# simonhmartin/genomics_general

Measured on NVIDIA H100. Metric: sites/sec popgenWindows (pi+Fst+Dxy), higher is better.
Workload: dtype u8

## Files before the change

genomics_general_b200/_lib.py:

```python
from __future__ import annotations

import ctypes as C
import os
import subprocess

import numpy as np

_HERE = os.path.dirname(os.path.abspath(__file__))
LIB_PATH = os.path.join(_HERE, "libpgwin.so")
CSRC = os.path.join(_HERE, "csrc")

_lib = None


class PgError(RuntimeError):
    pass


def build(force: bool = False, verbose: bool = False) -> str:
    srcs = [os.path.join(CSRC, f) for f in os.listdir(CSRC) if f.endswith((".cu", ".h", ".cpp"))]
    srcs.append(os.path.join(_HERE, "..", "include", "pgwin.h"))
    if not force and os.path.exists(LIB_PATH):
        newest = max(os.path.getmtime(s) for s in srcs)
        if os.path.getmtime(LIB_PATH) >= newest:
            return LIB_PATH
    cmd = ["make", "-C", CSRC, "-j4"]
    r = subprocess.run(cmd, stdout=subprocess.PIPE, stderr=subprocess.STDOUT, text=True)
    if verbose or r.returncode != 0:
        print(r.stdout)
    if r.returncode != 0:
        raise PgError("building libpgwin.so failed (nvcc for sm_90a)")
    return LIB_PATH


_SIGS = {
    "pg_version": (C.c_int, []),
    "pg_last_error": (C.c_char_p, []),
    "pg_device_count": (C.c_int, [C.POINTER(C.c_int)]),
    "pg_ctx_create": (C.c_int, [C.c_int, C.POINTER(C.c_void_p)]),
    "pg_ctx_destroy": (C.c_int, [C.c_void_p]),
    "pg_host_alloc": (C.c_int, [C.POINTER(C.c_void_p), C.c_size_t]),
    "pg_host_free": (C.c_int, [C.c_void_p]),
    "pg_upload": (C.c_int, [C.c_void_p, C.c_void_p, C.c_int64, C.c_int32, C.c_void_p]),
    "pg_alloc_sites": (C.c_int, [C.c_void_p, C.c_int64, C.c_int32]),
    "pg_upload_range": (C.c_int, [C.c_void_p, C.c_int64, C.c_int64, C.c_void_p, C.c_void_p]),
    "pg_append_sites": (C.c_int, [C.c_void_p, C.c_int64, C.c_void_p, C.c_void_p]),
    "pg_synth_fill": (C.c_int, [C.c_void_p, C.c_int64, C.c_int32, C.c_int32, C.c_int32, C.c_uint64, C.c_uint64,
                                C.c_uint64, C.c_uint64, C.c_uint64, C.c_int32]),
    "pg_download": (C.c_int, [C.c_void_p, C.c_int64, C.c_int64, C.c_void_p, C.c_void_p]),
    "pg_set_pops": (C.c_int, [C.c_void_p, C.c_int32, C.c_void_p]),
    "pg_set_windows": (C.c_int, [C.c_void_p, C.c_int64, C.c_void_p, C.c_void_p]),
    "pg_popgen": (C.c_int, [C.c_void_p, C.c_int32, C.c_double, C.c_int32, C.c_void_p, C.c_void_p, C.c_void_p,
                            C.c_void_p, C.c_void_p, C.c_void_p]),
    "pg_popgen_device": (C.c_int, [C.c_void_p, C.c_int32, C.c_double, C.c_int32, C.c_void_p, C.POINTER(C.c_int64)]),
    "pg_popgen_freqstats": (C.c_int, [C.c_void_p] * 6),
    "pg_set_freqstats": (C.c_int, [C.c_void_p, C.c_int32]),
    "pg_abbababa": (C.c_int, [C.c_void_p, C.c_int32, C.c_int32, C.c_int32, C.c_int32, C.c_double, C.c_void_p,
                              C.c_void_p, C.c_void_p, C.c_void_p]),
    "pg_fourpop": (C.c_int, [C.c_void_p, C.c_int32, C.c_int32, C.c_int32, C.c_int32, C.c_double, C.c_int32, C.c_void_p,
                             C.c_void_p, C.c_void_p, C.c_void_p]),
    "pg_site_counts": (C.c_int, [C.c_void_p, C.c_int64, C.c_int64, C.c_void_p]),
    "pg_site_target_freqs": (C.c_int, [C.c_void_p, C.c_int64, C.c_int64, C.c_int32, C.c_double, C.c_int32, C.c_void_p,
                                       C.c_void_p]),
    "pg_sfs": (C.c_int, [C.c_void_p, C.c_int32, C.c_int32, C.c_int32, C.c_void_p, C.c_void_p, C.c_void_p, C.c_void_p,
                         C.c_void_p, C.POINTER(C.c_int64)]),
    "pg_sfs_tables": (C.c_int, [C.c_void_p, C.c_int32, C.c_void_p, C.c_int64, C.c_int32, C.c_void_p, C.c_int32, C.c_int32,
                                C.c_int32, C.c_void_p, C.c_void_p, C.c_void_p, C.c_void_p, C.c_void_p, C.POINTER(C.c_int64)]),
    "pg_sfs_sparse": (C.c_int, [C.c_void_p, C.c_int32, C.c_int32, C.c_int32, C.c_void_p, C.c_void_p, C.c_void_p, C.c_void_p,
                                C.POINTER(C.c_int64)]),
    "pg_sfs_tables_sparse": (C.c_int, [C.c_void_p, C.c_int32, C.c_void_p, C.c_int64, C.c_int32, C.c_void_p, C.c_int32,
                                       C.c_int32, C.c_int32, C.c_void_p, C.c_void_p, C.c_void_p, C.c_void_p,
                                       C.POINTER(C.c_int64)]),
    "pg_sfs_sparse_fetch": (C.c_int, [C.c_void_p, C.c_int64, C.c_void_p, C.c_void_p, C.c_void_p]),
    "pg_pairdist": (C.c_int, [C.c_void_p, C.c_int32, C.c_void_p, C.c_int32, C.c_int32, C.c_void_p, C.c_void_p,
                              C.c_void_p]),
    "pg_distpaint": (C.c_int, [C.c_void_p, C.c_int32, C.c_void_p, C.c_int32, C.c_void_p, C.c_void_p, C.c_int32, C.c_int32,
                               C.c_double, C.c_int32, C.c_void_p, C.c_void_p, C.c_void_p]),
    "pg_pairdist_cat": (C.c_int, [C.c_void_p, C.c_int32, C.c_void_p, C.c_int32, C.c_void_p, C.POINTER(C.c_int64)]),
    "pg_seq_nonnan": (C.c_int, [C.c_void_p, C.c_void_p]),
    "pg_ind_het": (C.c_int, [C.c_void_p, C.c_int32, C.c_void_p, C.c_int32, C.c_void_p]),
    "pg_hapstats": (C.c_int, [C.c_void_p, C.c_double, C.c_int32, C.c_int32, C.c_void_p]),
    "pg_pair_counts": (C.c_int, [C.c_void_p, C.c_int64, C.c_void_p, C.c_void_p]),
    "pg_last_timings": (C.c_int, [C.c_void_p, C.c_int32, C.c_void_p, C.c_void_p, C.c_void_p, C.POINTER(C.c_int32)]),
    "pg_launch_count": (C.c_int, [C.c_void_p, C.POINTER(C.c_int64)]),
    "pg_debug_k1_plan": (C.c_int, [C.c_int64, C.c_int32] + [C.POINTER(C.c_int32)] * 5),
    "pg_debug_k1_plan_ex": (C.c_int, [C.c_int64, C.c_int32, C.c_int32, C.c_int32, C.c_int32, C.POINTER(C.c_int32)]),
    "pg_debug_packed": (C.c_int, [C.c_void_p, C.c_int64, C.c_int64, C.POINTER(C.c_int32), C.c_void_p]),
    "pg_debug_site_cls": (C.c_int, [C.c_void_p, C.c_int64, C.c_int64, C.POINTER(C.c_int32), C.c_void_p]),
    "pg_debug_uniform": (C.c_int, [C.c_void_p, C.POINTER(C.c_int32), C.POINTER(C.c_int64)]),
    "pg_debug_uniform_tile": (C.c_int, [C.c_void_p, C.POINTER(C.c_int32)]),
    "pg_debug_uniform_rows": (C.c_int, [C.c_void_p, C.POINTER(C.c_int64), C.POINTER(C.c_int64)]),
    "pg_debug_uniform_ring": (C.c_int, [C.c_void_p, C.POINTER(C.c_int32)]),
    "pg_debug_uniform_launch": (C.c_int, [C.c_void_p, C.POINTER(C.c_int32)]),
    "pg_debug_uniform_tiles": (C.c_int, [C.c_void_p, C.c_int64, C.c_void_p, C.c_void_p, C.POINTER(C.c_int64),
                                         C.POINTER(C.c_int32)]),
    "pg_nccl_unique_id": (C.c_int, [C.c_void_p]),
    "pg_nccl_init": (C.c_int, [C.c_void_p, C.c_int32, C.c_int32, C.c_void_p]),
    "pg_nccl_finalize": (C.c_int, [C.c_void_p]),
    "pg_popgen_gather_begin": (C.c_int, [C.c_void_p, C.c_int32, C.c_double, C.c_int64, C.c_int32]),
    "pg_popgen_gather_end": (C.c_int, [C.c_void_p, C.c_int32, C.POINTER(C.c_void_p), C.POINTER(C.c_int64)]),
    "pg_popgen_allgather": (C.c_int, [C.c_void_p, C.c_int32, C.c_double, C.c_int32, C.c_int64, C.c_void_p,
                                      C.POINTER(C.c_int64)]),
    "pg_ingest_file": (C.c_int, [C.c_void_p, C.c_char_p, C.c_int64, C.c_int32, C.c_int32, C.c_void_p, C.c_void_p, C.c_int32,
                                 C.POINTER(C.c_int64)]),
    "pg_ingest_file_range": (C.c_int, [C.c_void_p, C.c_char_p, C.c_int64, C.c_int64, C.c_int32, C.c_int32, C.c_void_p, C.c_void_p,
                                       C.c_int32, C.POINTER(C.c_int64)]),
    "pg_ingest_text": (C.c_int, [C.c_void_p, C.c_void_p, C.c_size_t, C.c_int32, C.c_int32, C.c_void_p, C.c_void_p, C.c_int32,
                                 C.POINTER(C.c_int64)]),
    "pg_ingest_meta": (C.c_int, [C.c_void_p, C.c_void_p, C.c_void_p, C.c_void_p]),
    "pg_ingest_release": (C.c_int, [C.c_void_p]),
    "pg_ingest_set_strict": (C.c_int, [C.c_void_p, C.c_int32]),
    "pg_debug_ingest": (C.c_int, [C.c_void_p, C.c_void_p]),
    "pg_filter": (C.c_int, [C.c_void_p, C.c_void_p, C.c_void_p, C.c_void_p, C.POINTER(C.c_int64), C.POINTER(C.c_uint8)]),
    "pg_filter_emit": (C.c_int, [C.c_void_p, C.c_int32, C.c_int32, C.c_int64, C.c_void_p, C.c_size_t, C.POINTER(C.c_int64),
                                 C.POINTER(C.c_size_t)]),
    "pg_filter_stats": (C.c_int, [C.c_void_p, C.c_int64, C.c_int64] + [C.c_void_p] * 8),
    "pg_format_freq_rows": (C.c_int, [C.c_int32, C.c_void_p, C.c_int64, C.c_int32, C.c_void_p, C.c_void_p, C.c_void_p,
                                      C.c_void_p, C.c_void_p, C.c_size_t, C.c_int32, C.c_void_p]),
    "pg_format_matrix_rows": (C.c_int, [C.c_void_p, C.c_int64, C.c_int32, C.c_int32, C.c_void_p, C.c_void_p, C.c_size_t,
                                        C.c_int32, C.c_void_p]),
    "pg_abbababa_allgather": (C.c_int, [C.c_void_p, C.c_int32, C.c_int32, C.c_int32, C.c_int32, C.c_double, C.c_int64,
                                        C.c_void_p]),
    "pg_fourpop_allgather": (C.c_int, [C.c_void_p, C.c_int32, C.c_int32, C.c_int32, C.c_int32, C.c_double, C.c_int32,
                                       C.c_int64, C.c_void_p]),
    "pg_vcf_set_spec": (C.c_int, [C.c_void_p, C.c_void_p]),
    "pg_vcf_load": (C.c_int, [C.c_void_p, C.c_char_p, C.c_size_t, C.c_char_p, C.c_int32, C.c_int32, C.POINTER(C.c_int64)]),
    "pg_vcf_lines": (C.c_int, [C.c_void_p, C.c_int64, C.c_int64, C.c_void_p]),
    "pg_vcf_genotypes": (C.c_int, [C.c_void_p, C.c_int64, C.c_void_p, C.c_void_p, C.POINTER(C.c_int64), C.POINTER(C.c_uint64)]),
    "pg_vcf_verdicts": (C.c_int, [C.c_void_p, C.c_void_p, C.c_void_p]),
    "pg_vcf_emit": (C.c_int, [C.c_void_p, C.c_int64, C.c_void_p, C.c_size_t, C.POINTER(C.c_int64), C.POINTER(C.c_size_t)]),
    "pg_seq_index": (C.c_int, [C.c_void_p, C.c_char_p, C.c_size_t, C.c_char_p, C.c_int64, C.c_int32, C.c_void_p, C.c_int32,
                               C.c_void_p, C.c_int32, C.POINTER(C.c_int64), C.c_void_p]),
    "pg_seq_meta": (C.c_int, [C.c_void_p, C.c_void_p, C.c_void_p, C.c_void_p]),
    "pg_seq_plan": (C.c_int, [C.c_void_p, C.c_int32, C.c_int32, C.c_int32, C.c_char_p, C.c_void_p, C.c_void_p, C.c_void_p,
                              C.c_void_p, C.c_int64, C.c_void_p, C.c_void_p, C.POINTER(C.c_int64), C.c_void_p]),
    "pg_seq_emit": (C.c_int, [C.c_void_p, C.c_int64, C.c_int64, C.c_void_p, C.c_size_t, C.POINTER(C.c_int64),
                              C.POINTER(C.c_int64), C.POINTER(C.c_size_t)]),
    "pg_g2v_ref_load": (C.c_int, [C.c_void_p, C.c_char_p, C.c_size_t, C.POINTER(C.c_int64)]),
    "pg_g2v_ref_starts": (C.c_int, [C.c_void_p, C.c_void_p]),
    "pg_g2v_ref_index": (C.c_int, [C.c_void_p, C.c_int64, C.c_void_p, C.c_void_p, C.c_void_p]),
    "pg_g2v_spec": (C.c_int, [C.c_void_p, C.c_int32, C.c_int32, C.c_void_p, C.c_void_p, C.c_int32, C.c_void_p, C.c_int32]),
    "pg_g2v_chunk": (C.c_int, [C.c_void_p, C.c_char_p, C.c_size_t, C.POINTER(C.c_int64), C.POINTER(C.c_int64)]),
    "pg_g2v_runs": (C.c_int, [C.c_void_p, C.c_void_p, C.c_void_p]),
    "pg_g2v_sites": (C.c_int, [C.c_void_p, C.c_void_p, C.POINTER(C.c_int64), C.POINTER(C.c_int64), C.c_void_p]),
    "pg_g2v_emit": (C.c_int, [C.c_void_p, C.c_int64, C.c_void_p, C.c_size_t, C.POINTER(C.c_size_t)]),
    "pg_s2g_fasta_load": (C.c_int, [C.c_void_p, C.c_char_p, C.c_size_t, C.POINTER(C.c_int64)]),
    "pg_s2g_fasta_starts": (C.c_int, [C.c_void_p, C.c_void_p]),
    "pg_s2g_fasta_index": (C.c_int, [C.c_void_p, C.c_int64, C.c_void_p, C.c_void_p, C.c_void_p]),
    "pg_s2g_phylip_load": (C.c_int, [C.c_void_p, C.c_char_p, C.c_size_t, C.POINTER(C.c_int64)]),
    "pg_s2g_phylip_lines": (C.c_int, [C.c_void_p, C.c_void_p]),
    "pg_s2g_phylip_pack": (C.c_int, [C.c_void_p, C.c_int64, C.c_void_p, C.c_int64, C.c_void_p]),
    "pg_s2g_plan": (C.c_int, [C.c_void_p, C.c_int64, C.c_void_p, C.c_char_p, C.c_int64, C.c_int64, C.c_void_p, C.c_void_p,
                              C.POINTER(C.c_int64)]),
    "pg_s2g_emit": (C.c_int, [C.c_void_p, C.c_int64, C.c_void_p, C.c_size_t, C.POINTER(C.c_size_t)]),
    "pg_ws_spec": (C.c_int, [C.c_void_p, C.c_int32, C.c_void_p, C.c_int32, C.c_int32]),
    "pg_ws_chunk": (C.c_int, [C.c_void_p, C.c_char_p, C.c_size_t, C.POINTER(C.c_int64), C.POINTER(C.c_int64),
                              C.POINTER(C.c_int64), C.c_void_p]),
    "pg_ws_chunk_info": (C.c_int, [C.c_void_p, C.c_void_p, C.c_void_p, C.c_void_p, C.c_void_p]),
    "pg_ws_set_values": (C.c_int, [C.c_void_p, C.c_int64, C.c_void_p, C.c_void_p, C.c_void_p]),
    "pg_ws_meta": (C.c_int, [C.c_void_p, C.POINTER(C.c_int64), C.c_void_p]),
    "pg_ws_stats": (C.c_int, [C.c_void_p, C.c_int64, C.c_void_p, C.c_void_p, C.c_int32, C.c_void_p, C.c_void_p, C.c_int64,
                              C.c_void_p, C.c_void_p]),
    "pg_geno_count_lines": (C.c_int, [C.c_char_p, C.c_size_t, C.POINTER(C.c_int64)]),
    "pg_geno_parse": (C.c_int, [C.c_char_p, C.c_size_t, C.c_int32, C.c_int32, C.c_void_p, C.c_void_p, C.c_int32,
                                C.c_int64, C.c_void_p, C.c_void_p, C.c_void_p, C.c_void_p, C.c_int32]),
}

EXPORTS = tuple(_SIGS)


class FilterSpec(C.Structure):
    _fields_ = [("n_samp", C.c_int32), ("samp_hap0", C.c_void_p), ("samp_ploidy", C.c_void_p), ("P", C.c_int32),
                ("pop_off", C.c_void_p), ("pop_members", C.c_void_p), ("min_calls", C.c_int32), ("min_alleles", C.c_int32), ("max_alleles", C.c_double),
                ("min_var_count", C.c_int32), ("has_max_het", C.c_int32), ("max_het", C.c_double),
                ("min_freq", C.c_double), ("max_freq", C.c_double), ("min_pop_calls", C.c_void_p),
                ("min_pop_alleles", C.c_void_p), ("max_pop_alleles", C.c_void_p), ("fixed_diffs", C.c_int32),
                ("has_nearly_fixed", C.c_int32), ("nearly_fixed_diff", C.c_double), ("partial_to_missing", C.c_int32),
                ("no_test", C.c_int32), ("thin_dist", C.c_int32), ("pod_size", C.c_int32)]
# ... 42 lines not shown
```

genomics_general_b200/csrc/ctx.cu:

```cuda
#include <stdarg.h>
#include <stdlib.h>

#include <algorithm>
#include <thread>

#include "pgwin_internal.h"

static thread_local char g_err[1024] = "";

void pg_set_error(const char* fmt, ...) {
    va_list ap;
    va_start(ap, fmt);
    vsnprintf(g_err, sizeof(g_err), fmt, ap);
    va_end(ap);
}

extern "C" const char* pg_last_error(void) { return g_err; }
extern "C" int pg_version(void) { return 110; }

extern "C" int pg_device_count(int* n) {
    PG_CHECK(n != nullptr, "pg_device_count: null argument");
    *n = 0;
    PG_CUDA(cudaGetDeviceCount(n));
    return PG_OK;
// ... 86 lines not shown
            cudaEventDestroy(ctx->h_text_free[k]);
        }
    cudaStreamDestroy(ctx->stream);
    delete ctx;
    return PG_OK;
}

extern "C" int pg_host_alloc(void** ptr, size_t bytes) {
    PG_CHECK(ptr != nullptr, "pg_host_alloc: null pointer");
    PG_CUDA(cudaHostAlloc(ptr, bytes, cudaHostAllocDefault));
    return PG_OK;
}
extern "C" int pg_host_free(void* ptr) {
    if (ptr) PG_CUDA(cudaFreeHost(ptr));
    return PG_OK;
}

int pg_pinned(pg_ctx* ctx, size_t bytes, void** out) {
    if (bytes > ctx->h_pinned_cap) {
        if (ctx->h_pinned) cudaFreeHost(ctx->h_pinned);
        ctx->h_pinned = nullptr;
        ctx->h_pinned_cap = 0;
        size_t want = bytes + bytes / 4 + 4096;
        PG_CUDA(cudaHostAlloc(&ctx->h_pinned, want, cudaHostAllocDefault));
        ctx->h_pinned_cap = want;
    }
    *out = ctx->h_pinned;
    return PG_OK;
}

int pg_d2h_staged(pg_ctx* ctx, void* dst, const void* src, size_t bytes) {
    if (bytes == 0) return PG_OK;
    const size_t slab = (size_t)64 << 20;
    bool pinned = false;
    {
        cudaPointerAttributes at;
        if (cudaPointerGetAttributes(&at, dst) == cudaSuccess) pinned = (at.type == cudaMemoryTypeHost);
        else cudaGetLastError();
    }
    if (pinned || bytes < ((size_t)8 << 20)) {
        PG_CUDA(cudaMemcpyAsync(dst, src, bytes, cudaMemcpyDeviceToHost, ctx->stream));
        PG_CUDA(cudaStreamSynchronize(ctx->stream));
        return PG_OK;
    }
    if (!ctx->h_text[0]) {
        for (int k = 0; k < 2; ++k) {
            PG_CUDA(cudaHostAlloc(&ctx->h_text[k], slab, cudaHostAllocDefault));
            PG_CUDA(cudaEventCreateWithFlags(&ctx->h_text_free[k], cudaEventDisableTiming));
        }
    }
    const int n_threads = std::max(1, std::min(16, (int)std::thread::hardware_concurrency() / 2));
    auto drain = [&](int b, size_t off, size_t n) {
        std::vector<std::thread> th;
        auto work = [&](int t) {
            const size_t a = n * (size_t)t / (size_t)n_threads, e = n * (size_t)(t + 1) / (size_t)n_threads;
            memcpy((char*)dst + off + a, (const char*)ctx->h_text[b] + a, e - a);
        };
        for (int t = 1; t < n_threads; ++t) th.emplace_back(work, t);
        work(0);
        for (auto& x : th) x.join();
    };
    size_t prev_off = 0, prev_n = 0;
    int k = 0;
    for (size_t off = 0; off < bytes; off += slab, ++k) {
        const size_t n = std::min(slab, bytes - off);
        const int b = k & 1;
        PG_CUDA(cudaMemcpyAsync(ctx->h_text[b], (const char*)src + off, n, cudaMemcpyDeviceToHost, ctx->stream));
        PG_CUDA(cudaEventRecord(ctx->h_text_free[b], ctx->stream));
        if (k > 0) {
            PG_CUDA(cudaEventSynchronize(ctx->h_text_free[b ^ 1]));
            drain(b ^ 1, prev_off, prev_n);
        }
        prev_off = off;
        prev_n = n;
    }
    PG_CUDA(cudaEventSynchronize(ctx->h_text_free[(k - 1) & 1]));
    drain((k - 1) & 1, prev_off, prev_n);
    return PG_OK;
}

void pg_timings_reset(pg_ctx* ctx) {
    ctx->timings.clear();
    ctx->events_used = 0;
}
static cudaEvent_t next_event(pg_ctx* ctx) {
    if (ctx->events_used == ctx->event_pool.size()) {
        cudaEvent_t ev;
        cudaEventCreate(&ev);
        ctx->event_pool.push_back(ev);
    }
    return ctx->event_pool[ctx->events_used++];
}
int pg_time_begin(pg_ctx* ctx, const char* name) {
    PgTiming t;
    memset(&t, 0, sizeof(t));
    strncpy(t.name, name, sizeof(t.name) - 1);
    t.start = next_event(ctx);
    t.stop = next_event(ctx);
    t.launches = 1;
    cudaEventRecord(t.start, ctx->stream);
    ctx->timings.push_back(t);
    ctx->launches += 1;
    return (int)ctx->timings.size() - 1;
}
void pg_time_end(pg_ctx* ctx, int idx) { cudaEventRecord(ctx->timings[idx].stop, ctx->stream); }

extern "C" int pg_last_timings(pg_ctx* ctx, int32_t cap, char (*names)[32], float* ms, int32_t* launches,
                               int32_t* count) {
    PG_CHECK(ctx && count, "pg_last_timings: null argument");
    PG_CUDA(cudaSetDevice(ctx->device));
    PG_CUDA(cudaStreamSynchronize(ctx->stream));
    std::vector<std::string> order;
    std::vector<float> tot;
    std::vector<int> cnt;
    for (const PgTiming& t : ctx->timings) {
        float m = 0.f;
        PG_CUDA(cudaEventElapsedTime(&m, t.start, t.stop));
        size_t k = 0;
        for (; k < order.size(); ++k)
            if (order[k] == t.name) break;
        if (k == order.size()) {
            order.push_back(t.name);
            tot.push_back(0.f);
            cnt.push_back(0);
        }
        tot[k] += m;
        cnt[k] += t.launches;
    }
    int n = (int)std::min<size_t>(order.size(), (size_t)std::max(cap, 0));
    for (int k = 0; k < n; ++k) {
        if (names) {
            memset(names[k], 0, 32);
            strncpy(names[k], order[k].c_str(), 31);
        }
        if (ms) ms[k] = tot[k];
        if (launches) launches[k] = cnt[k];
    }
    *count = n;
    return PG_OK;
}

extern "C" int pg_launch_count(pg_ctx* ctx, int64_t* n) {
    PG_CHECK(ctx && n, "pg_launch_count: null argument");
    *n = ctx->launches;
    return PG_OK;
}

int pg_pitch_for(int H) {
    int chunks = (H + 15) / 16;
    if (chunks < 1) chunks = 1;
    if ((chunks & 1) == 0) chunks += 1;
    return chunks * 16;
}

static int env_int(const char* name, int dflt) {
    const char* e = getenv(name);
    return (e && *e) ? atoi(e) : dflt;
}

K1Plan pg_make_k1_plan(int64_t S, int H, int sm_count, int table_bytes, int nw, int force_G) {
    return pg_make_k1_plan_rows(S, pg_pitch_for(H), sm_count, table_bytes, nw, force_G);
}

int pg_k1_ring_stages(int tile_bytes, int table_bytes) {
    const int smem_cap = 227 * 1024 - 2048 - table_bytes;
    int stages = smem_cap / tile_bytes;
// ... 573 lines not shown
```

genomics_general_b200/csrc/k1.cu:

```cuda
#include <stdlib.h>

#include <algorithm>
#include <climits>
#include <cmath>
#include <type_traits>
#include <cub/cub.cuh>

#include "pgwin_internal.h"

namespace {

constexpr int K1_MAX_WARPS = 12;

enum { MODE_POPGEN = 0, MODE_ABBA = 1, MODE_COUNTS = 2, MODE_POPGEN_FREQ = 3, MODE_FOURPOP = 4 };

struct K1Params {
    const uint8_t* geno;
    const int32_t* pos;
    int64_t site_begin, site_end;
    int64_t num_tiles;
    int pitch, G, I, T, wpt, stages, tile_bytes, nw;
    const int32_t* ent_chunk;
    const uint4* ent_mask;
    int n_ent;
// ... 1262 lines not shown
                            gseg = next_seg(prm.brk, prm.nseg, gseg + 1, first);
                            gseg_end = __ldg(prm.brk + gseg + 1);
                        }
                        const uint32_t in = pending & __ballot_sync(0xffffffffu, site < gseg_end);
                        gram_add(k0, k1, in);
                        pending &= ~in;
                    }
                }
            } else if constexpr (P < 8) {
                for (int r = ((lw - rot + wpt) % wpt) * 32; r < n1; r += wpt * 32) {
                    const int rw = r + mma_row(lane);
                    BitCounts<P> ct;
                    ct.N = prm.popN;
                    varied_mma<P>(s_bf, reinterpret_cast<const uint32_t*>(tile), n1, prm.wd, r, lane, ct);
                    add_row(tile_site0 + (rw < n1 ? s_slot[rw] : 0), rw < n1, ct, false);
                }
            }

            const uint32_t* rows3 = reinterpret_cast<const uint32_t*>(tile) + ((n1 * prm.wd + 3) & ~3);
            for (int r = ((lw - rot - nb1 % wpt + 2 * wpt) % wpt) * spv; r < n3; r += wpt * spv) {
                const int rw = r + sl;
                const bool valid = rw < n3;
                const bool owner = valid && (gsub == 0);
                const uint32_t* row = rows3 + (valid ? rw : r);
                std::conditional_t<P == 8, ArrCounts<P>, PkCounts<P>> ct;
                if (P < 8 && Gv == 1) varied_counts<P, true>(prm, s_ent, row, n3, 1, 0, 32, ct);
                else varied_counts<P, false>(prm, s_ent, row, n3, Gv, gsub, spv, ct);
                add_row(tile_site0 + (valid ? s_slot[n1 + rw] : 0), owner, ct, true);
            }

            __syncwarp();
            if (lane == 0) mbar_arrive(&empty[stage]);
        }
        if constexpr (GRAM) gram_flush();
    }
    warp_flush<QI, QU, 0>(acc, cur_seg, prm.part, slot_base, seg_first, warp, lane, NW);
}

struct FinParams {
    const unsigned long long* part;
    const int32_t* seg_cta_lo;
    const int32_t* seg_cta_hi;
    const int32_t* cta_seg_first;
    const int64_t* cta_slot_off;
    const int32_t* win_seg_lo;
    const int32_t* win_seg_hi;
    const int64_t* win_lo;
    const int64_t* win_hi;
    int64_t W;
    int Q, QI, nw;
    int P;
    int Ppad;
    int popN[PG_MAX_K1_POPS];
    double harm_a[PG_MAX_K1_POPS], harm_a2[PG_MAX_K1_POPS];
    int min_sites;
    double min_data;
    int force_path;
    int with_freq;
    int bookkeeping_only;
    const int64_t* pre_pos;
    const int64_t* pre_uni;
    int64_t S;
    unsigned long long* rec;
    int RC;
    int32_t* path;
    int* n_pairwise;
};

__device__ __forceinline__ unsigned long long d2u(double x) { return (unsigned long long)__double_as_longlong(x); }

__device__ __forceinline__ double nan_d() { return __longlong_as_double(0x7ff8000000000000ll); }

__device__ __forceinline__ double cf_pi(long long N, long long Lp, long long sumsq, bool all_nan, double min_data) {
    if (N <= 0) return nan_d();
    const double size = (double)(N * N);
    const double nan_cnt = all_nan ? size : (double)N;
    if (1.0 - (1.0 * nan_cnt / size) < min_data) return nan_d();
    if (all_nan) return nan_d();
    const double num = (double)(N * N * Lp - sumsq);
    const double den = (double)((N * N - N) * Lp);
    return num / den;
}

template <int MODE>
__global__ void __launch_bounds__(64) k1_finalize(const __grid_constant__ FinParams fp) {
    __shared__ unsigned long long sums[64];
    const int q = threadIdx.x;
    for (int64_t w = blockIdx.x; w < fp.W; w += gridDim.x) {
        __syncthreads();
        if (q < fp.Q) {
            long long si = 0;
            double sd = 0.0;
            for (int g = fp.win_seg_lo[w]; g < fp.win_seg_hi[w]; ++g) {
                for (int b = fp.seg_cta_lo[g]; b <= fp.seg_cta_hi[g]; ++b) {
                    const unsigned long long* src =
                        fp.part + fp.cta_slot_off[b] + (int64_t)(g - fp.cta_seg_first[b]) * fp.nw * fp.Q;
                    for (int wp = 0; wp < fp.nw; ++wp) {
                        const unsigned long long v = src[wp * fp.Q + q];
                        if (q < fp.QI) si += (long long)v; else sd += __longlong_as_double((long long)v);
                    }
                }
            }
            if (MODE == MODE_POPGEN && fp.pre_uni) {
                const int64_t lo = min(max(fp.win_lo[w], (int64_t)0), fp.S), hi = min(max(fp.win_hi[w], lo), fp.S);
                const long long u = fp.pre_uni[hi] - fp.pre_uni[lo];
                const int Pp = fp.Ppad;
                if (q == 0) si += u;
                else if (q == 2) si += fp.pre_pos[hi] - fp.pre_pos[lo];
                else if (q >= 3 && q < 3 + Pp + Pp * (Pp - 1) / 2) {
                    int X = q - 3, Y = X;
                    if (X >= Pp) {
                        int k = X - Pp, left = Pp - 1;
                        for (X = 0; k >= left; ++X, --left) k -= left;
                        Y = X + 1 + k;
                    }
                    si += u * (long long)fp.popN[X] * (long long)fp.popN[Y];
                }
            }
            sums[q] = (q < fp.QI) ? (unsigned long long)si : (unsigned long long)__double_as_longlong(sd);
        }
        __syncthreads();
        if (q != 0) continue;
        const long long sites = fp.win_hi[w] - fp.win_lo[w];
        unsigned long long* rec = fp.rec + (size_t)w * fp.RC;
        rec[0] = (unsigned long long)sites;
        rec[1] = sums[2];
        if (MODE == MODE_POPGEN) {
            const int P = fp.P, Pp = fp.Ppad;
            const int npairs = P * (P - 1) / 2;
            double* pi_o = reinterpret_cast<double*>(rec + 3);
            double* dxy_o = pi_o + P;
            double* fst_o = dxy_o + npairs;
            const long long Lp = (long long)sums[0];
            const bool ragged = (long long)sums[1] > 0;
            if (fp.bookkeeping_only) {
                const int path = sites < fp.min_sites ? 0 : 2;
                fp.path[w] = path;
                rec[2] = (unsigned long long)path;
                if (path == 2) atomicAdd(fp.n_pairwise, 1);
                for (int k = 3; k < fp.RC; ++k) rec[k] = d2u(nan_d());
                continue;
            }
            {
                double* fq = fst_o + npairs;
                fq[0] = fp.with_freq ? (double)Lp : nan_d();
                const int npp = Pp * (Pp - 1) / 2;
                for (int x = 0; x < P; ++x) {
                    double Sx = nan_d(), tpi = nan_d(), tw = nan_d(), tD = nan_d();
                    if (Lp >= 1 && fp.with_freq) {
                        const long long N = fp.popN[x];
                        const long long seg = N == 1 ? (long long)Lp : (long long)sums[3 + Pp + npp + x];
                        const long long pairs = (N * N * Lp - (long long)sums[3 + x]) / 2;
                        Sx = (double)seg;
                        tpi = (double)pairs / (.5 * (double)N * (double)(N - 1));
                        const double a = fp.harm_a[x], a2 = fp.harm_a2[x];
                        tw = (double)seg / a;
                        const double n_ = (double)N;
                        const double b1 = (n_ + 1.) / (3 * (n_ - 1));
                        const double b2 = (2. * (n_ * n_ + n_ + 3)) / (9 * n_ * (n_ - 1));
                        const double c1 = b1 - (1. / a);
                        const double c2 = b2 - ((n_ + 2) / (a * n_)) + a2 / (a * a);
                        const double e1 = c1 / a;
                        const double e2 = c2 / (a * a + a2);
                        const double d = tpi - tw;
                        tD = d / sqrt(e1 * Sx + e2 * Sx * (Sx - 1));
                    }
                    fq[1 + x] = Sx;
                    fq[1 + P + x] = tpi;
                    fq[1 + 2 * P + x] = tw;
                    fq[1 + 3 * P + x] = tD;
                }
            }
            int path = 1;
            if (sites < fp.min_sites) path = 0;
            else if (ragged || fp.force_path == 2) path = 2;
            fp.path[w] = path;
            rec[2] = (unsigned long long)path;
            if (path == 2) atomicAdd(fp.n_pairwise, 1);
            if (path != 1) {
                for (int x = 0; x < P; ++x) pi_o[x] = nan_d();
                for (int k = 0; k < npairs; ++k) dxy_o[k] = fst_o[k] = nan_d();
                continue;
            }
            const bool all_nan = (Lp == 0) || (fp.min_sites > 0 && Lp < fp.min_sites);
            double piv[PG_MAX_K1_POPS];
            for (int x = 0; x < P; ++x) {
                piv[x] = cf_pi(fp.popN[x], Lp, (long long)sums[3 + x], all_nan, fp.min_data);
                pi_o[x] = piv[x];
            }
            int k = 0;
            for (int x = 0; x < P; ++x)
                for (int y = x + 1; y < P; ++y) {
                    int kp = 0;
                    for (int xx = 0; xx < x; ++xx) kp += Pp - 1 - xx;
                    kp += y - x - 1;
                    const long long cross = (long long)sums[3 + Pp + kp];
                    const long long Nx = fp.popN[x], Ny = fp.popN[y];
                    double dxy = nan_d();
                    {
                        const double size = (double)(Nx * Ny);
                        const double nan_cnt = all_nan ? size : 0.0;
                        const bool frac_bad = (1.0 - (1.0 * nan_cnt / size) < fp.min_data);
                        if (!frac_bad && !all_nan) dxy = (double)(Nx * Ny * Lp - cross) / (double)(Nx * Ny * Lp);
                    }
// ... 456 lines not shown
    p.pitch = pl.pitch;
    p.G = pl.G;
    p.I = pl.I;
    p.T = pl.T;
    p.wpt = pl.wpt;
    p.nw = pl.nw;
    p.stages = pl.stages;
    p.tile_bytes = pl.tile_bytes;
    p.ent_chunk = dt.ent_chunk;
    p.ent_mask = dt.ent_mask;
    p.word_ent = dt.word_ent;
    p.bit_frag = dt.bit_frag;
    p.wd = (ctx->H + 31) / 32;
    p.n_ent = packed ? (int)pt.word_ent.size() / 2 : (int)pt.ent_chunk.size();
    for (int X = 0; X < PG_MAX_K1_POPS; ++X) {
        p.ent_lo[X] = pt.ent_lo[X];
        p.ent_hi[X] = pt.ent_hi[X];
        p.full_lo[X] = pt.full_lo[X];
        p.full_hi[X] = pt.full_hi[X];
        p.popN[X] = pt.popN[X];
    }
}

int prepare_windowed(pg_ctx* ctx, K1Cache& c, const std::vector<int32_t>& hap_pop_local, int Ppad, int Q, int nw, int force_G,
                     bool packed) {
    K1Launch& L = c.L;
    DevTables& dt = c.dt;
    PopTables& pt = c.pt;
    PG_TRY(pg_build_segments(ctx));
    if (packed) {
        build_word_tables(hap_pop_local, ctx->H, Ppad, pt);
        const int table_bytes = table_bytes_of(pt);
        PG_CHECK(table_bytes <= 48 * 1024, "population layout needs %d bytes of mask tables (limit 48 KiB)", table_bytes);
        L.plan = pg_make_k1_plan_rows(ctx->S, ctx->packed_pitch, ctx->sm_count, table_bytes, nw, force_G);
        PG_CHECK(L.plan.stages >= 2, "rows of %d haplotypes are too long for the packed site pass (%d bytes)", ctx->H,
                 L.plan.pitch);
        PG_TRY(check_plan(L.plan));
    } else {
        PG_TRY(byte_plan(ctx, hap_pop_local, Ppad, nw, force_G, pt, L.plan));
    }
    for (int X = 0; X < Ppad; ++X) PG_CHECK(pt.popN[X] <= 65535, "a population has more than 65535 haplotypes");
    const K1Plan& pl = L.plan;
    const int B = pl.ctas;
    std::vector<int64_t> bound(B + 1);
    for (int b = 0; b <= B; ++b) bound[b] = std::min<int64_t>((int64_t)b * pl.num_tiles / B * pl.T, ctx->S);
    HostSlots hs;
    slot_tables(ctx->brk, bound, nw, Q, hs);
    size_t bytes = 4096 + pt.ent_mask.size() * 4 + pt.ent_chunk.size() * 4 + pt.word_ent.size() * 4 + pt.bit_frag.size() * 4 +
                   ctx->brk.size() * 8 + hs.bytes() + (size_t)ctx->W * 24 + 14 * 16;
    PG_TRY(c.tables.ensure(bytes));
    uint8_t* base = (uint8_t*)c.tables.p;
    size_t o = 0;
    uint32_t* d_mask_words = nullptr;
    PG_TRY(push(ctx, base, o, pt.ent_mask.data(), pt.ent_mask.size(), &d_mask_words));
    dt.ent_mask = reinterpret_cast<uint4*>(d_mask_words);
    PG_TRY(push(ctx, base, o, pt.ent_chunk.data(), pt.ent_chunk.size(), &dt.ent_chunk));
    uint32_t* d_word_ent = nullptr;
    PG_TRY(push(ctx, base, o, pt.word_ent.data(), pt.word_ent.size(), &d_word_ent));
    dt.word_ent = reinterpret_cast<uint2*>(d_word_ent);
    uint32_t* d_bit_frag = nullptr;
    PG_TRY(push(ctx, base, o, pt.bit_frag.data(), pt.bit_frag.size(), &d_bit_frag));
    dt.bit_frag = reinterpret_cast<uint2*>(d_bit_frag);
    PG_TRY(push(ctx, base, o, ctx->brk.data(), ctx->brk.size(), &dt.brk));
    PG_TRY(push_slots(ctx, base, o, hs, L.slots));
    PG_TRY(push(ctx, base, o, ctx->win_seg_lo.data(), ctx->win_seg_lo.size(), &dt.win_seg_lo));
    PG_TRY(push(ctx, base, o, ctx->win_seg_hi.data(), ctx->win_seg_hi.size(), &dt.win_seg_hi));
    PG_TRY(push(ctx, base, o, ctx->win_lo.data(), ctx->win_lo.size(), &dt.win_lo));
    PG_TRY(push(ctx, base, o, ctx->win_hi.data(), ctx->win_hi.size(), &dt.win_hi));
    PG_CHECK(o <= c.tables.cap, "internal: table buffer overflow");
    PG_CUDA(cudaStreamSynchronize(ctx->stream));

    K1Params& p = L.prm;
    fill_params(p, ctx, pl, pt, dt, packed);
    p.site_begin = 0;
    p.site_end = ctx->S;
    p.brk = dt.brk;
    p.nseg = (int)ctx->brk.size() - 1;
    p.cta_seg_first = L.slots.cta_seg_first;
    p.cta_slot_off = L.slots.cta_slot_off;
    return PG_OK;
}

int arm_slots(pg_ctx* ctx, K1Launch& L, const void* rows) {
    const size_t bytes = (size_t)std::max<int64_t>(L.slots.words, 1) * 8;
    PG_TRY(ctx->part.ensure(bytes));
    PG_CUDA(cudaMemsetAsync(ctx->part.p, 0, bytes, ctx->stream));
    L.prm.part = (unsigned long long*)ctx->part.p;
    L.prm.geno = (const uint8_t*)rows;
    L.prm.pos = ctx->d_pos;
    return PG_OK;
}

template <auto Kern, int NW>
int launch_kernel(pg_ctx* ctx, const K1Launch& L, const char* name) {
    PG_TRY(pg_smem_limit<Kern>(ctx, 227 * 1024));
    const int ti = pg_time_begin(ctx, name);
    Kern<<<L.plan.ctas, (NW + 1) * 32, L.plan.smem_bytes, ctx->stream>>>(L.prm);
    pg_time_end(ctx, ti);
    PG_CUDA(cudaGetLastError());
    return PG_OK;
}

template <int MODE, int P>
int launch_site_pass(pg_ctx* ctx, const K1Launch& L, const char* name) {
    constexpr bool POPGEN_MODE = (MODE == MODE_POPGEN || MODE == MODE_POPGEN_FREQ);
    const bool w12 = L.prm.nw == 12;
    if constexpr ((POPGEN_MODE || MODE == MODE_COUNTS) && (P == 4 || P == 8)) {
        if (L.prm.lanepop)
            return w12 ? launch_kernel<k1_site_pass_lp<MODE, P, 12>, 12>(ctx, L, name)
                       : launch_kernel<k1_site_pass_lp<MODE, P, 8>, 8>(ctx, L, name);
    }
    if constexpr (POPGEN_MODE) {
        if (L.prm.bytes)
            return w12 ? launch_kernel<k1_site_pass<MODE, P, 12, true>, 12>(ctx, L, name)
                       : launch_kernel<k1_site_pass<MODE, P, 8, true>, 8>(ctx, L, name);
    }
    return w12 ? launch_kernel<k1_site_pass<MODE, P, 12, false>, 12>(ctx, L, name)
               : launch_kernel<k1_site_pass<MODE, P, 8, false>, 8>(ctx, L, name);
}

template <int MODE, int P, bool UNI>
int launch_site_pass_packed(pg_ctx* ctx, const K1Launch& L, const char* name, int32_t* launched = nullptr) {
    if (launched) {
        launched[0] = L.plan.ctas;
        launched[1] = L.prm.nw;
        launched[2] = UNI && P < 8 && L.prm.bytes ? 1 : 0;
    }
    if constexpr (UNI && P < 8) {
        if (L.prm.bytes)
            return L.prm.nw == 12 ? launch_kernel<k1_site_pass_packed<MODE, P, 12, true, true>, 12>(ctx, L, name)
                                  : launch_kernel<k1_site_pass_packed<MODE, P, 8, true, true>, 8>(ctx, L, name);
    }
    return L.prm.nw == 12 ? launch_kernel<k1_site_pass_packed<MODE, P, 12, UNI>, 12>(ctx, L, name)
                          : launch_kernel<k1_site_pass_packed<MODE, P, 8, UNI>, 8>(ctx, L, name);
}

template <typename F>
int with_pops(int Pp, F&& f) {
    if (Pp == 2) return f(std::integral_constant<int, 2>());
    if (Pp == 4) return f(std::integral_constant<int, 4>());
    return f(std::integral_constant<int, 8>());
}

template <typename F>
int with_popgen_mode(bool with_freq, int Pp, F&& f) {
    return with_pops(Pp, [&](auto P) {
        return with_freq ? f(std::integral_constant<int, MODE_POPGEN_FREQ>(), P) : f(std::integral_constant<int, MODE_POPGEN>(), P);
    });
}

constexpr double UNI_MIN_FRACTION = 0.125;

int uni_word_rows(int R, int pitch, int wd) { return (R * (pitch / 4) - 3) / wd; }

int uni_stage_bytes(int row_cap, int cap_rows, int pitch) {
    return (int)align_up((size_t)row_cap * pitch + align_up((size_t)cap_rows * 2, 16), 128);
}

void uni_geometry(UniformPass& u) {
    const K1Plan& pl = u.plan;
    const char* eb = getenv("PG_K1_UNI_BITS");
    u.bits = u.one_plane && !(eb && *eb && atoi(eb) == 0);
    const char* er = getenv("PG_K1_UNI_R");
    u.words = u.bits && !(er && *er);
    int Tmax = u.words ? 2048 : 512;
    if (const char* e = getenv("PG_K1_UNI_TMAX")) Tmax = std::max(8, std::min(32768, (atoi(e) + 7) / 8 * 8));
    const int lanes = 32 / std::max(1, pl.G);
    int R = lanes * pl.wpt;
    auto stage = [&](int r) {
        const bool w = u.words && r >= 2;
        u.row_cap = w ? r + 1 : r;
        u.cap_rows = w ? uni_word_rows(r, pl.pitch, u.wd) : r;
        return uni_stage_bytes(u.row_cap, u.cap_rows, pl.pitch);
// ... 135 lines not shown
    PG_CUDA(cudaStreamSynchronize(ctx->stream));
    us.nt = info[0];
    const int B = (int)std::max<int64_t>(1, std::min<int64_t>(ctas, us.nt));
    us.bound.assign(info.begin() + 1, info.begin() + 2 + B);
    us.in_use = true;
    return PG_OK;
}

int uniform_slots(pg_ctx* ctx, UniformPass& u, const K1Launch& L, int Q) {
    if (u.slots_epoch == ctx->epoch && u.slots_serial == u.us.serial && u.slots_Q == Q && u.L.plan.stages == u.stages)
        return PG_OK;
    HostSlots hs;
    slot_tables(ctx->brk, u.us.bound, L.prm.nw, Q, hs);
    PG_TRY(u.slot_buf.ensure(hs.bytes()));
    size_t o = 0;
    PG_TRY(push_slots(ctx, (uint8_t*)u.slot_buf.p, o, hs, u.L.slots));
    PG_CHECK(o <= u.slot_buf.cap, "internal: slot table buffer overflow");
    PG_CUDA(cudaStreamSynchronize(ctx->stream));
    K1Plan& pl = u.L.plan;
    pl = u.plan;
    pl.T = u.Tmax;
    pl.num_tiles = u.us.nt;
    pl.ctas = (int)u.us.bound.size() - 1;
    pl.tile_bytes = u.stage_bytes;
    pl.stages = u.stages;
    pl.smem_bytes = pl.stages * pl.tile_bytes + 256 + u.table_bytes;
    K1Params& p = u.L.prm;
    p = L.prm;
    p.T = pl.T;
    p.num_tiles = pl.num_tiles;
    p.stages = pl.stages;
    p.tile_bytes = pl.tile_bytes;
    p.row_cap = u.row_cap;
    p.cta_seg_first = u.L.slots.cta_seg_first;
    p.cta_slot_off = u.L.slots.cta_slot_off;
    p.row0 = (const int64_t*)u.us.row0.p;
    p.site_lo = (const int64_t*)u.us.site_lo.p;
    p.woff = u.us.woff;
    p.n1 = (const int32_t*)u.us.n1.p;
    p.slots = (const uint16_t*)u.us.slots.p;
    u.slots_epoch = ctx->epoch;
    u.slots_serial = u.us.serial;
    u.slots_Q = Q;
    return PG_OK;
}

int pad_pops(int P) { return P <= 2 ? 2 : (P <= 4 ? 4 : 8); }

K1Cache* cache_of(pg_ctx* ctx, int slot) {
    if (!ctx->k1_cache[slot]) ctx->k1_cache[slot] = new K1Cache();
    return static_cast<K1Cache*>(ctx->k1_cache[slot]);
}

void fill_fin(FinParams& fp, pg_ctx* ctx, const K1Cache& c, const SlotTables& slots, int Q, int QI) {
    memset(&fp, 0, sizeof(fp));
    fp.part = (const unsigned long long*)ctx->part.p;
    fp.seg_cta_lo = slots.seg_cta_lo;
    fp.seg_cta_hi = slots.seg_cta_hi;
    fp.cta_seg_first = slots.cta_seg_first;
    fp.cta_slot_off = slots.cta_slot_off;
    fp.win_seg_lo = c.dt.win_seg_lo;
    fp.win_seg_hi = c.dt.win_seg_hi;
    fp.win_lo = c.dt.win_lo;
    fp.win_hi = c.dt.win_hi;
    fp.W = ctx->W;
    fp.Q = Q;
    fp.QI = QI;
    fp.nw = c.L.prm.nw;
    for (int X = 0; X < PG_MAX_K1_POPS; ++X) {
        fp.popN[X] = c.pt.popN[X];
        double a = 0.0, a2 = 0.0;
        for (int i = 1; i < c.pt.popN[X]; ++i) {
            a += 1. / (double)i;
            a2 += 1. / ((double)i * (double)i);
        }
        fp.harm_a[X] = a;
        fp.harm_a2[X] = a2;
    }
}

template <int MODE>
int launch_finalize(pg_ctx* ctx, const FinParams& fp) {
    const int ti = pg_time_begin(ctx, "k1_finalize");
    k1_finalize<MODE><<<(unsigned)std::min<int64_t>(fp.W, 65535), 64, 0, ctx->stream>>>(fp);
    pg_time_end(ctx, ti);
    PG_CUDA(cudaGetLastError());
    return PG_OK;
}

unsigned long long nan_bits() {
    const double qn = NAN;
    unsigned long long u;
    memcpy(&u, &qn, 8);
    return u;
}

int put_empty_records(pg_ctx* ctx, const std::vector<unsigned long long>& one, void* d_rec) {
    std::vector<unsigned long long> h;
    h.reserve((size_t)ctx->W * one.size());
    for (int64_t w = 0; w < ctx->W; ++w) h.insert(h.end(), one.begin(), one.end());
    PG_CUDA(cudaMemcpyAsync(d_rec, h.data(), h.size() * 8, cudaMemcpyHostToDevice, ctx->stream));
    PG_CUDA(cudaStreamSynchronize(ctx->stream));
    return PG_OK;
}

int min_count(int N, double min_data) {
    for (int n = 0; n <= N; ++n)
        if ((double)n * 1.0 / (double)N >= min_data) return n;
    return N + 1;
}

template <int FIN_MODE, typename Launch>
int fourpop_enqueue(pg_ctx* ctx, const char* who, int slot, int Q, int RC, int nan_end, const int* sel, double min_data,
                    int variant, void* d_rec, Launch launch) {
    PG_CHECK(ctx->P >= 1, "%s: call pg_set_pops first", who);
    for (int k = 0; k < 4; ++k) {
        PG_CHECK(sel[k] >= 0 && sel[k] < ctx->P, "%s: population index %d out of range", who, sel[k]);
        for (int j = 0; j < k; ++j) PG_CHECK(sel[j] != sel[k], "%s: populations must be distinct", who);
    }
    PG_CUDA(cudaSetDevice(ctx->device));
    pg_timings_reset(ctx);
    if (ctx->W == 0) return PG_OK;
    if (ctx->S == 0) {
        std::vector<unsigned long long> one(RC, 0ull);
        std::fill(one.begin() + 2, one.begin() + nan_end, nan_bits());
        return put_empty_records(ctx, one, d_rec);
    }
    K1Cache& c = *cache_of(ctx, slot);
    if (!c.valid || c.epoch != ctx->epoch || memcmp(c.sel, sel, 4 * sizeof(int)) != 0) {
        c.valid = false;
        std::vector<int32_t> local(ctx->H, -1);
        for (int h = 0; h < ctx->H; ++h)
            for (int k = 0; k < 4; ++k)
                if (ctx->hap_pop[h] == sel[k]) local[h] = k;
        PG_TRY(prepare_windowed(ctx, c, local, 4, Q, k1_nw_for(ctx->pitch, false), 0, false));
        for (int k = 0; k < 4; ++k) PG_CHECK(c.pt.popN[k] >= 1, "%s: population %d has no haplotypes", who, sel[k]);
        memcpy(c.sel, sel, 4 * sizeof(int));
        c.epoch = ctx->epoch;
        c.valid = true;
    }
    for (int k = 0; k < 4; ++k) c.L.prm.thr[k] = min_count(c.pt.popN[k], min_data);
    c.L.prm.variant = variant;
    PG_TRY(arm_slots(ctx, c.L, ctx->d_geno));
    PG_TRY(launch(c.L));
    FinParams fp;
    fill_fin(fp, ctx, c, c.L.slots, Q, 3);
    fp.P = 4;
    fp.Ppad = 4;
    fp.rec = (unsigned long long*)d_rec;
    fp.RC = RC;
    return launch_finalize<FIN_MODE>(ctx, fp);
}

template <typename Enqueue>
int fourpop_read(pg_ctx* ctx, int RC, Enqueue enqueue, double* out, double* sites_used, int64_t* n_sites, int64_t* pos_sum) {
    const int64_t W = ctx->W;
    PG_CUDA(cudaSetDevice(ctx->device));
    PG_TRY(ctx->out_d.ensure((size_t)std::max<int64_t>(W, 1) * RC * 8 + 64));
    PG_TRY(enqueue(ctx->out_d.p));
    if (W == 0) return PG_OK;
    void* hp = nullptr;
    PG_TRY(pg_pinned(ctx, (size_t)W * RC * 8 + 64, &hp));
    const unsigned long long* hrec = (const unsigned long long*)hp;
    PG_CUDA(cudaMemcpyAsync(hp, ctx->out_d.p, (size_t)W * RC * 8, cudaMemcpyDeviceToHost, ctx->stream));
    PG_CUDA(cudaStreamSynchronize(ctx->stream));
    const int n = RC - 3;
    for (int64_t w = 0; w < W; ++w) {
// ... 29 lines not shown
    pg_timings_reset(ctx);
    const int P = ctx->P;
    const bool many = P > PG_MAX_K1_POPS;
    const int npairs = P * (P - 1) / 2;
    const int RC = 3 + P + 2 * npairs + 1 + 4 * P;
    const int64_t W = ctx->W;
    if (W == 0) return PG_OK;
    if (ctx->S == 0) {
        std::vector<unsigned long long> one(RC, nan_bits());
        one[0] = one[1] = 0;
        one[2] = (0 < min_sites) ? 0 : 1;
        return put_empty_records(ctx, one, d_rec);
    }
    const int Pp = many ? 2 : pad_pops(P);
    const bool wf = ctx->want_freq && !many;
    const int Q = 3 + Pp + Pp * (Pp - 1) / 2 + (wf ? Pp : 0);
    const bool packed = ctx->d_packed != nullptr && !getenv("PG_K1_BYTE_PASS");
    K1Cache& c = *cache_of(ctx, 0);
    UniformPass& u = c.up;
    if (!c.valid || c.epoch != ctx->epoch || c.packed != packed) {
        c.valid = false;
        int maxN = 0;
        for (int x = 0; x < P; ++x) {
            int N = 0;
            for (int h = 0; h < ctx->H; ++h) N += ctx->hap_pop[h] == x;
            PG_CHECK(N >= 1, "pg_popgen: population %d has no haplotypes", x);
            maxN = std::max(maxN, N);
        }
        std::vector<int32_t> collapsed;
        if (many) {
            collapsed.assign(ctx->hap_pop.begin(), ctx->hap_pop.end());
            for (int32_t& v : collapsed) v = v >= 0 ? 0 : -1;
        }
        const std::vector<int32_t>& pop_map = many ? collapsed : ctx->hap_pop;
        PopTables pt;
        if (packed) {
            K1Plan bp;
            PG_TRY(byte_plan(ctx, pop_map, Pp, k1_nw_for(ctx->pitch, false), 0, pt, bp));
            c.lanepop = false;
            const int nw = k1_nw_for(ctx->packed_pitch, false);
            PG_TRY(prepare_windowed(ctx, c, pop_map, Pp, Q, nw, 0, true));
            u.one_plane = Pp < 8;
            u.table_bytes = table_bytes_of(c.pt) + (u.one_plane ? (int)c.pt.bit_frag.size() * 4 : 0);
            u.plan = c.L.plan;
            u.wd = (ctx->H + 31) / 32;
            u.slots_epoch = 0;
        } else {
            build_tables(pop_map, ctx->H, ctx->pitch / 16, Pp, pt);
            const WarpChoice wc = choose_warps(ctx, ctx->S, Pp, Pp == P, table_bytes_of(pt), byte_counts(maxN));
            c.lanepop = wc.lanepop;
            PG_TRY(prepare_windowed(ctx, c, pop_map, Pp, Q, wc.nw, wc.lanepop ? Pp : 0, false));
        }
        c.packed = packed;
        c.epoch = ctx->epoch;
        c.valid = true;
    }
    const bool uni = c.packed && ctx->d_site_cls && !getenv("PG_K1_NO_UNIFORM");
    if (c.packed) uni_geometry(u);
    if (uni) PG_TRY(uniform_prepare(ctx, u));
    u.last = uni && u.us.in_use;
    if (u.last) PG_TRY(uniform_slots(ctx, u, c.L, Q));
    K1Launch& L = u.last ? u.L : c.L;
    {
        long long maxN = 1;
        for (int X = 0; X < Pp; ++X) maxN = std::max<long long>(maxN, c.pt.popN[X]);
        L.prm.acc_limit = (int)std::max<long long>(1, std::min<long long>(0xffffffffll / (maxN * maxN), 1 << 30));
        if (const char* e = getenv("PG_K1_ACC_LIMIT")) L.prm.acc_limit = std::max(1, atoi(e));
        L.prm.bytes = byte_counts((int)maxN) ? 1 : 0;
        L.prm.lanepop = c.lanepop ? 1 : 0;
        const char* gv = getenv("PG_K1_UNI_GV");
        L.prm.uni_gv = u.last && gv && *gv ? atoi(gv) : 0;
        PG_CHECK(L.prm.uni_gv >= 0 && L.prm.uni_gv <= 32 && (L.prm.uni_gv & (L.prm.uni_gv - 1)) == 0,
                 "PG_K1_UNI_GV must be a power of two up to 32");
    }
    PG_TRY(arm_slots(ctx, L, u.last ? u.us.rows.p : c.packed ? (const void*)ctx->d_packed : ctx->d_geno));
    PG_TRY(with_popgen_mode(wf, Pp, [&](auto M, auto PP) {
        constexpr int MODE = decltype(M)::value, PT = decltype(PP)::value;
        if (u.last) return launch_site_pass_packed<MODE, PT, true>(ctx, L, "k1_popgen", u.launched);
        if (c.packed) return launch_site_pass_packed<MODE, PT, false>(ctx, L, "k1_popgen");
        return launch_site_pass<MODE, PT>(ctx, L, "k1_popgen");
    }));

    PG_TRY(ctx->out_i.ensure((size_t)W * 4 + 128));
    int* d_cnt = (int*)ctx->out_i.p;
    int32_t* d_path = (int32_t*)ctx->out_i.p + 16;
    PG_CUDA(cudaMemsetAsync(d_cnt, 0, 4, ctx->stream));
    FinParams fp;
    fill_fin(fp, ctx, c, L.slots, Q, Q);
    fp.P = P;
    fp.Ppad = Pp;
    fp.min_sites = min_sites;
    fp.min_data = min_data;
    fp.force_path = many ? 2 : force_path;
    fp.bookkeeping_only = many ? 1 : 0;
    fp.with_freq = wf ? 1 : 0;
    if (u.last) {
        fp.pre_uni = (const int64_t*)u.us.pre.p;
        fp.pre_pos = fp.pre_uni + ctx->S + 1;
        fp.S = ctx->S;
    }
    fp.rec = (unsigned long long*)d_rec;
    fp.RC = RC;
    fp.path = d_path;
    fp.n_pairwise = d_cnt;
    PG_TRY(launch_finalize<MODE_POPGEN>(ctx, fp));
    if (!h_count) return PG_OK;
    void* hp = nullptr;
    PG_TRY(pg_pinned(ctx, (size_t)W * 4 + 256, &hp));
    int* h_cnt = (int*)hp;
    *h_cnt = 0;
    PG_CUDA(cudaMemcpyAsync(h_cnt, d_cnt, 4, cudaMemcpyDeviceToHost, ctx->stream));
    *h_count = h_cnt;
    return PG_OK;
}

extern "C" int pg_debug_uniform(pg_ctx* ctx, int32_t* in_use, int64_t* varied_sites) {
    PG_CHECK(ctx && in_use && varied_sites, "pg_debug_uniform: null argument");
    const K1Cache* c = static_cast<const K1Cache*>(ctx->k1_cache[0]);
    const bool read = c && c->up.last;
    *in_use = read ? 1 : 0;
    *varied_sites = (c && c->up.us.gen == ctx->data_gen) ? c->up.us.varied : ctx->S;
    return PG_OK;
}

extern "C" int pg_debug_uniform_tile(pg_ctx* ctx, int32_t* out) {
    PG_CHECK(ctx && out, "pg_debug_uniform_tile: null argument");
    const K1Cache* c = static_cast<const K1Cache*>(ctx->k1_cache[0]);
    const bool planned = c && c->valid && c->packed;
    out[0] = planned ? c->up.Tmax : 0;
    out[1] = planned ? c->up.plan.wpt : 0;
    return PG_OK;
}

extern "C" int pg_debug_uniform_ring(pg_ctx* ctx, int32_t* out) {
    PG_CHECK(ctx && out, "pg_debug_uniform_ring: null argument");
    const K1Cache* c = static_cast<const K1Cache*>(ctx->k1_cache[0]);
    const bool read = c && c->up.last;
    out[0] = read ? c->up.cap_rows : 0;
    out[1] = read ? c->up.stages : 0;
    out[2] = read ? c->up.stage_bytes : 0;
    return PG_OK;
}

extern "C" int pg_debug_uniform_launch(pg_ctx* ctx, int32_t* out) {
    PG_CHECK(ctx && out, "pg_debug_uniform_launch: null argument");
    const K1Cache* c = static_cast<const K1Cache*>(ctx->k1_cache[0]);
    const bool read = c && c->up.last;
    for (int k = 0; k < 3; ++k) out[k] = read ? c->up.launched[k] : 0;
    return PG_OK;
}

extern "C" int pg_debug_uniform_tiles(pg_ctx* ctx, int64_t cap, int64_t* site_lo, int64_t* row0, int64_t* ntiles,
                                      int32_t* geometry) {
    PG_CHECK(ctx && ntiles && geometry, "pg_debug_uniform_tiles: null argument");
    const K1Cache* c = static_cast<const K1Cache*>(ctx->k1_cache[0]);
    const bool read = c && c->up.last;
    const UniformStream* us = read ? &c->up.us : nullptr;
    *ntiles = read ? us->nt : 0;
    geometry[0] = read ? c->up.cap_rows : 0;
    geometry[1] = read ? c->up.Tmax : 0;
    if (!read || cap < us->nt + 1) return PG_OK;
    PG_CHECK(site_lo && row0, "pg_debug_uniform_tiles: null table");
    PG_CUDA(cudaSetDevice(ctx->device));
    PG_CUDA(cudaStreamSynchronize(ctx->stream));
    PG_CUDA(cudaMemcpy(site_lo, us->site_lo.p, (size_t)(us->nt + 1) * 8, cudaMemcpyDeviceToHost));
    PG_CUDA(cudaMemcpy(row0, us->row0.p, (size_t)(us->nt + 1) * 8, cudaMemcpyDeviceToHost));
    return PG_OK;
}

// ... 908 lines not shown
```

genomics_general_b200/csrc/k2.cu:

```cuda
#include <stdlib.h>

#include <algorithm>
#include <cmath>

#include "pgwin_internal.h"

namespace {

constexpr int TS = 64;
constexpr int TSP = TS + 1;
constexpr int KW = 16;
constexpr int K4 = KW / 4;
constexpr int NST = 3;
enum { PAIR_DIFF = 0, PAIR_N = 1 };
template <int WHAT>
struct PairGeom {
    static constexpr int NP = (WHAT == PAIR_DIFF) ? 3 : 1;
    static constexpr int OPND_BYTES = NP * K4 * TSP * 16;
    static constexpr int STAGE_BYTES = 2 * OPND_BYTES;
    static constexpr int SMEM = NST * STAGE_BYTES;
};

__device__ __forceinline__ uint32_t smem_u32(const void* p) { return (uint32_t)__cvta_generic_to_shared(p); }
__device__ __forceinline__ void cp_async16(void* dst, const void* src, bool valid) {
// ... 320 lines not shown
    const int32_t* n;
    const int32_t* mid;
    int Hm;
    int Hk, P;
    const int32_t* pop_start;
    int min_sites;
    double min_data;
    unsigned long long* rec;
    int RC;
    const int64_t* win_idx;
    double* blk_s;
    long long* blk_c;
};

__device__ __forceinline__ double nanmean_min_dev(double sum, double nonnan, double size, double min_data) {
    if (size <= 0) return nan_d();
    const double nan_cnt = size - nonnan;
    if (1.0 - (1.0 * nan_cnt / size) < min_data) return nan_d();
    if (nonnan <= 0) return nan_d();
    return sum / nonnan;
}

__global__ void __launch_bounds__(256) k2_popgen_epi_blocks(const __grid_constant__ PopEpiParams ep) {
    __shared__ double sh_s[8];
    __shared__ long long sh_c[8];
    const int P = ep.P;
    const int wb = blockIdx.y;
    int bi = blockIdx.x, X = 0;
    while (bi >= P - X) {
        bi -= P - X;
        ++X;
    }
    const int Y = X + bi;
    const size_t HH = (size_t)ep.Hk * ep.Hk;
    const int32_t* D = ep.diff + (size_t)wb * HH;
    const int32_t* N = ep.n + (size_t)wb * ep.Hm * ep.Hm;
    const int r0 = ep.pop_start[X], r1 = ep.pop_start[X + 1];
    const int c0 = ep.pop_start[Y], c1 = ep.pop_start[Y + 1];
    const int nr = r1 - r0, nc = c1 - c0;
    double s = 0.0;
    long long c = 0;
    double s1 = 0.0;
    long long cnt1 = 0;
    for (int i = r0 + (threadIdx.x >> 5); i < r1; i += 8) {
        const int mi = ep.mid[i];
        const int32_t* Drow = D + (size_t)i * ep.Hk;
        for (int j = ((X == Y) ? i + 1 : c0) + (threadIdx.x & 31); j < c1; j += 64) {
            const int j2 = j + 32;
            const int nij = N[upper_idx(mi, ep.mid[j], ep.Hm)];
            const int nij2 = (j2 < c1) ? N[upper_idx(mi, ep.mid[j2], ep.Hm)] : 0;
            const bool ok = !(nij == 0 || (ep.min_sites > 0 && nij < ep.min_sites));
            const bool ok2 = !(nij2 == 0 || (ep.min_sites > 0 && nij2 < ep.min_sites));
            const double d0 = ok ? (double)Drow[j] / (double)nij : 0.0;
            const double d1 = ok2 ? (double)Drow[j2] / (double)nij2 : 0.0;
            if (ok) {
                s += d0;
                c += 1;
            }
            if (ok2) {
                s1 += d1;
                cnt1 += 1;
            }
        }
    }
    s += s1;
    c += cnt1;
    (void)nr;
    (void)nc;
    block_sum(s, c, sh_s, sh_c);
    if (threadIdx.x == 0) {
        const int nblk = P * (P + 1) / 2;
        ep.blk_s[(size_t)wb * nblk + blockIdx.x] = s;
        ep.blk_c[(size_t)wb * nblk + blockIdx.x] = c;
    }
}

__global__ void __launch_bounds__(128) k2_popgen_epi_pairs(const __grid_constant__ PopEpiParams ep) {
    extern __shared__ __align__(16) double epi_sh[];
    const int P = ep.P, nblk = P * (P + 1) / 2;
    double* sh_s = epi_sh;
    long long* sh_c = reinterpret_cast<long long*>(epi_sh + (size_t)nblk * 4);
    const int wb = blockIdx.x;
    const int lane = threadIdx.x & 31, warp = threadIdx.x >> 5;
    const int32_t* D = ep.diff + (size_t)wb * ep.Hk * ep.Hk;
    const int32_t* N = ep.n + (size_t)wb * ep.Hm * ep.Hm;
    int blk = 0;
    for (int X = 0; X < P; ++X) {
        const int a0 = ep.pop_start[X] >> 1, a1 = ep.pop_start[X + 1] >> 1;
        for (int Y = X; Y < P; ++Y, ++blk) {
            if (blk % (int)gridDim.y != (int)blockIdx.y) continue;
            const int b0 = ep.pop_start[Y] >> 1, b1 = ep.pop_start[Y + 1] >> 1;
            double s = 0.0;
            int c = 0;
            const int n = a1 - a0;
            const bool diag = (X == Y);
            const uint32_t width = diag ? (uint32_t)(n + 1) : (uint32_t)(b1 - b0);
            const uint32_t units = diag ? (uint32_t)((n + 1) / 2) * width : (uint32_t)n * width;
            const uint32_t magic = width > 1 ? (uint32_t)(((1ull << 32) + width - 1) / width) : 0u;
#pragma unroll 2
            for (uint32_t idx = threadIdx.x; idx < units; idx += 128) {
                uint32_t r = width > 1 ? __umulhi(idx, magic) : idx;
                int k = (int)(idx - r * width);
                if (k < 0) {
                    r -= 1;
                    k += (int)width;
                }
                int a = a0 + (int)r, b = b0 + k;
                bool use = true;
                if (diag) {
                    if (k < n - (int)r) b = a + k;
                    else {
                        const int a2 = n - 1 - (int)r;
                        use = (a2 != (int)r);
                        a = a0 + a2;
                        b = a + (k - (n - (int)r));
                    }
                }
                const int nab = N[(size_t)a * ep.Hm + b];
                const int2 u = *reinterpret_cast<const int2*>(D + (size_t)(2 * a) * ep.Hk + 2 * b);
                const int2 v = *reinterpret_cast<const int2*>(D + (size_t)(2 * a + 1) * ep.Hk + 2 * b);
                const bool ok = use && nab != 0 && !(ep.min_sites > 0 && nab < ep.min_sites);
                const int num = (a == b) ? u.y : (u.x + u.y + v.x + v.y);
                const double q = (double)num / (double)(ok ? nab : 1);
                if (ok) {
                    s += q;
                    c += (a == b) ? 1 : 4;
                }
            }
#pragma unroll
            for (int d = 16; d >= 1; d >>= 1) {
                s += __shfl_xor_sync(0xffffffffu, s, d);
                c += __shfl_xor_sync(0xffffffffu, c, d);
            }
            if (lane == 0) {
                sh_s[blk * 4 + warp] = s;
                sh_c[blk * 4 + warp] = c;
            }
        }
    }
    __syncthreads();
    for (int b = threadIdx.x; b < nblk; b += 128) {
        if (b % (int)gridDim.y != (int)blockIdx.y) continue;
        ep.blk_s[(size_t)wb * nblk + b] = ((sh_s[b * 4] + sh_s[b * 4 + 1]) + sh_s[b * 4 + 2]) + sh_s[b * 4 + 3];
        ep.blk_c[(size_t)wb * nblk + b] = sh_c[b * 4] + sh_c[b * 4 + 1] + sh_c[b * 4 + 2] + sh_c[b * 4 + 3];
    }
}

__global__ void __launch_bounds__(128) k2_popgen_epi_final(const __grid_constant__ PopEpiParams ep, int nb) {
    const int wb = blockIdx.x * 128 + threadIdx.x;
    if (wb >= nb) return;
    const int P = ep.P;
    const int nblk = P * (P + 1) / 2;
    const double* blk_s = ep.blk_s + (size_t)wb * nblk;
    const long long* blk_c = ep.blk_c + (size_t)wb * nblk;
    const int npairs = P * (P - 1) / 2;
    double* pi_o = reinterpret_cast<double*>(ep.rec + (size_t)ep.win_idx[wb] * ep.RC + 3);
    double* dxy_o = pi_o + P;
    double* fst_o = dxy_o + npairs;
    auto bidx = [&](int X, int Y) { return X * P - X * (X - 1) / 2 + (Y - X); };
    for (int X = 0; X < P; ++X) {
        const double Nx = ep.pop_start[X + 1] - ep.pop_start[X];
        const int b = bidx(X, X);
        pi_o[X] = nanmean_min_dev(2.0 * blk_s[b], 2.0 * (double)blk_c[b], Nx * Nx, ep.min_data);
    }
    int k = 0;
    for (int X = 0; X < P; ++X)
        for (int Y = X + 1; Y < P; ++Y, ++k) {
            const double Nx = ep.pop_start[X + 1] - ep.pop_start[X], Ny = ep.pop_start[Y + 1] - ep.pop_start[Y];
            const int bxx = bidx(X, X), byy = bidx(Y, Y), bxy = bidx(X, Y);
            const double dxy = nanmean_min_dev(blk_s[bxy], (double)blk_c[bxy], Nx * Ny, ep.min_data);
            const double st = blk_s[bxx] + blk_s[byy] + blk_s[bxy];
            const double ct = (double)(blk_c[bxx] + blk_c[byy] + blk_c[bxy]);
            const double pi_t = nanmean_min_dev(2.0 * st, 2.0 * ct, (Nx + Ny) * (Nx + Ny), ep.min_data);
            const double w = 1.0 * Nx / (Nx + Ny);
            const double pi_s = w * pi_o[X] + (1 - w) * pi_o[Y];
            dxy_o[k] = dxy;
            fst_o[k] = 1 - pi_s / pi_t;
        }
}

struct IndEpiParams {
    const int32_t* diff;
    const int32_t* n;
    const int32_t* mid;
    int Hm;
    int Hk, n_ind;
    const int32_t* ind_start;
    int include_same;
    int min_sites;
    double* out;
};

__global__ void __launch_bounds__(256) k2_ind_epi(const __grid_constant__ IndEpiParams ep) {
    const int wb = blockIdx.y;
    const size_t HH = (size_t)ep.Hk * ep.Hk;
    const int32_t* D = ep.diff + (size_t)wb * HH;
    const int32_t* N = ep.n + (size_t)wb * ep.Hm * ep.Hm;
    const int64_t total = (int64_t)ep.n_ind * ep.n_ind;
    double* o = ep.out + (size_t)wb * total;
    const int lane = threadIdx.x & 31;
    for (int a = blockIdx.x * 8 + (threadIdx.x >> 5); a < ep.n_ind; a += gridDim.x * 8) {
        const int i0 = ep.ind_start[a], i1 = ep.ind_start[a + 1];
        for (int b = lane; b < ep.n_ind; b += 32) {
            const int j0 = ep.ind_start[b], j1 = ep.ind_start[b + 1];
            double s = 0.0;
// ... 454 lines not shown
    std::vector<int32_t> c2r(ctx->pitch, -1);
    for (int r = 0; r < Hk; ++r) c2r[order[r]] = r;
    PG_TRY(ctx->misc2.ensure((size_t)ctx->pitch * 4 + 64));
    PG_CUDA(cudaMemcpyAsync(ctx->misc2.p, c2r.data(), (size_t)ctx->pitch * 4, cudaMemcpyHostToDevice, ctx->stream));
    PG_TRY(pg_smem_limit<k2_build_planes>(ctx, BP_SMEM));
    const int colblocks = (ctx->pitch + BP_COLS - 1) / BP_COLS;
    for (int64_t y0 = 0; y0 < nblk; y0 += 65535) {
        const int64_t ny = std::min<int64_t>(65535, nblk - y0);
        PG_TRY(pg_timed(ctx, "k2_planes", [&] {
            k2_build_planes<<<dim3((unsigned)colblocks, (unsigned)ny), 256, BP_SMEM, ctx->stream>>>(
                (const uint8_t*)ctx->d_geno, ctx->pitch, ctx->S, sb + y0 * BP_SITES, (const int32_t*)ctx->misc2.p,
                (uint32_t*)ctx->planes.p + y0 * 8, Hk, NWp);
        }));
    }
    ps.Hk = Hk;
    ps.site_base = sb;
    ps.NWp = NWp;
    ps.planes = (uint32_t*)ctx->planes.p;
    int32_t* d_mid = (int32_t*)(ps.planes + bytes / 4);
    int32_t* d_rowmap = d_mid + Hk;
    PG_TRY(ctx->misc4.ensure((size_t)Hk * 12 + 256));
    unsigned long long* d_hash = (unsigned long long*)ctx->misc4.p;
    int32_t* d_rep = (int32_t*)(d_hash + Hk);
    int* d_flag = (int*)(d_rep + Hk);
    const uint32_t* mplane = ps.planes + (size_t)2 * Hk * NWp;
    PG_TRY(pg_timed(ctx, "k2_mask_groups", [&] { k2_hash_rows<<<Hk, 256, 0, ctx->stream>>>(mplane, NWp, d_hash); }));
    std::vector<unsigned long long> hh(Hk);
    PG_CUDA(cudaMemcpyAsync(hh.data(), d_hash, (size_t)Hk * 8, cudaMemcpyDeviceToHost, ctx->stream));
    PG_CUDA(cudaStreamSynchronize(ctx->stream));
    std::vector<int32_t> rep(Hk), mid(Hk), rowmap;
    {
        std::vector<std::pair<unsigned long long, int>> first;
        for (int r = 0; r < Hk; ++r) {
            int q = -1;
            for (size_t k = 0; k < first.size(); ++k)
                if (first[k].first == hh[r]) {
                    q = (int)k;
                    break;
                }
            if (q < 0) {
                first.push_back({hh[r], r});
                q = (int)first.size() - 1;
                rowmap.push_back(r);
            }
            mid[r] = q;
            rep[r] = first[q].second;
        }
    }
    PG_CUDA(cudaMemcpyAsync(d_rep, rep.data(), (size_t)Hk * 4, cudaMemcpyHostToDevice, ctx->stream));
    PG_CUDA(cudaMemsetAsync(d_flag, 0, 4, ctx->stream));
    PG_TRY(pg_timed(ctx, "k2_mask_groups", [&] { k2_verify_rows<<<Hk, 256, 0, ctx->stream>>>(mplane, NWp, d_rep, d_flag); }));
    int flag = 0;
    PG_CUDA(cudaMemcpyAsync(&flag, d_flag, 4, cudaMemcpyDeviceToHost, ctx->stream));
    PG_CUDA(cudaStreamSynchronize(ctx->stream));
    if (flag || getenv("PG_K2_NO_MASK_SHARING")) {
        rowmap.resize(Hk);
        for (int r = 0; r < Hk; ++r) mid[r] = rowmap[r] = r;
    }
    ps.Hm = (int)rowmap.size();
    ps.mid = mid;
    PG_CUDA(cudaMemcpyAsync(d_mid, mid.data(), (size_t)Hk * 4, cudaMemcpyHostToDevice, ctx->stream));
    PG_CUDA(cudaMemcpyAsync(d_rowmap, rowmap.data(), (size_t)ps.Hm * 4, cudaMemcpyHostToDevice, ctx->stream));
    PG_CUDA(cudaStreamSynchronize(ctx->stream));
    ps.d_mid = d_mid;
    ps.d_rowmap = d_rowmap;
    return PG_OK;
}

int build_planes(pg_ctx* ctx, const std::vector<int32_t>& order, int64_t lo, int64_t hi, PlaneSet& ps) {
    const int Hk = (int)order.size();
    PG_CHECK(Hk >= 1, "pairwise path: no haplotypes selected");
    ps.tensor = pg_k2_use_tensor() && pg_k2t_fits(ctx->pitch, Hk);
    if (!ps.tensor) return build_popc_planes(ctx, order, lo, hi, ps);
    PG_TRY(pg_k2t_build(ctx, order, lo, hi, ps.t));
    ps.Hk = Hk;
    ps.Hm = ps.t.Hm;
    ps.mid.resize(Hk);
    for (int r = 0; r < Hk; ++r) ps.mid[r] = (ps.t.Hm == Hk) ? r : r / 2;
    ps.d_mid = ps.t.d_mid;
    return PG_OK;
}

int run_pair_batch(pg_ctx* ctx, const PlaneSet& ps, const int64_t* d_lo, const int64_t* d_hi, int nb, int32_t** d_diff,
                   int32_t** d_n) {
    const size_t HH = (size_t)ps.Hk * ps.Hk, MM = (size_t)ps.Hm * ps.Hm;
    PG_TRY(ctx->pairs.ensure((size_t)nb * (HH + MM) * 4 + 64));
    *d_diff = (int32_t*)ctx->pairs.p;
    *d_n = *d_diff + (size_t)nb * HH;
    if (ps.tensor) return pg_k2t_pairs(ctx, ps.t, d_lo, d_hi, nb, *d_diff, *d_n);
    PG_TRY(pg_smem_limit<k2_pair<PAIR_DIFF>>(ctx, PairGeom<PAIR_DIFF>::SMEM));
    PG_TRY(pg_smem_limit<k2_pair<PAIR_N>>(ctx, PairGeom<PAIR_N>::SMEM));
    PairParams pp;
    pp.planes = ps.planes;
    pp.Hk = ps.Hk;
    pp.NWp = ps.NWp;
    pp.site_base = ps.site_base;
    pp.win_lo = d_lo;
    pp.win_hi = d_hi;
    pp.n_rows = ps.Hk;
    pp.row_map = nullptr;
    pp.ntile = (ps.Hk + TS - 1) / TS;
    pp.out = *d_diff;
    PG_TRY(pg_timed(ctx, "k2_pair_diff", [&] {
        k2_pair<PAIR_DIFF><<<dim3((unsigned)(pp.ntile * (pp.ntile + 1) / 2), (unsigned)nb), 256, PairGeom<PAIR_DIFF>::SMEM,
                             ctx->stream>>>(pp);
    }));
    pp.n_rows = ps.Hm;
    pp.row_map = ps.d_rowmap;
    pp.ntile = (ps.Hm + TS - 1) / TS;
    pp.out = *d_n;
    return pg_timed(ctx, "k2_pair_n", [&] {
        k2_pair<PAIR_N><<<dim3((unsigned)(pp.ntile * (pp.ntile + 1) / 2), (unsigned)nb), 256, PairGeom<PAIR_N>::SMEM,
                          ctx->stream>>>(pp);
    });
}

int run_het(pg_ctx* ctx, const PlaneSet& ps, const int64_t* d_lo, const int64_t* d_hi, int nb, const int32_t* d_ind_start,
            int n_ind, int min_sites, double* d_out) {
    if (ps.tensor) return pg_k2t_het(ctx, ps.t, d_lo, d_hi, nb, d_ind_start, n_ind, min_sites, d_out);
    HetParams hp;
    hp.planes = ps.planes;
    hp.Hk = ps.Hk;
    hp.NWp = ps.NWp;
    hp.site_base = ps.site_base;
    hp.win_lo = d_lo;
    hp.win_hi = d_hi;
    hp.ind_start = d_ind_start;
    hp.n_ind = n_ind;
    hp.min_sites = min_sites;
    hp.out = d_out;
    return pg_timed(ctx, "k2_het", [&] { k2_het<<<dim3((unsigned)n_ind, (unsigned)nb), 128, 0, ctx->stream>>>(hp); });
}

int run_seq_nonnan(pg_ctx* ctx, const PlaneSet& ps, const int64_t* d_lo, const int64_t* d_hi, int nb, long long* d_out) {
    if (ps.tensor) return pg_k2t_seq_nonnan(ctx, ps.t, d_lo, d_hi, nb, d_out);
    return pg_timed(ctx, "k2_seq_nonnan", [&] {
        k2_seq_nonnan<<<dim3((unsigned)ps.Hk, (unsigned)nb), 128, 0, ctx->stream>>>(ps.planes + (size_t)2 * ps.Hk * ps.NWp,
                                                                                   ps.NWp, ps.site_base, d_lo, d_hi, ps.Hk,
                                                                                   d_out);
    });
}

int group_rows(const pg_ctx* ctx, const int32_t* group, int G, const char* what, std::vector<int32_t>& order,
               std::vector<int32_t>& start) {
    for (int h = 0; what && h < ctx->H; ++h)
        PG_CHECK(group[h] >= -1 && group[h] < G, "%s[%d]=%d out of range", what, h, group[h]);
    start.assign(G + 1, 0);
    for (int g = 0; g < G; ++g) {
        start[g] = (int32_t)order.size();
        for (int h = 0; h < ctx->H; ++h)
            if (group[h] == g) order.push_back(h);
    }
    start[G] = (int32_t)order.size();
    return PG_OK;
}

std::vector<int32_t> all_rows(int H) {
    std::vector<int32_t> order(H);
    for (int h = 0; h < H; ++h) order[h] = h;
    return order;
}

void nonempty_windows(const pg_ctx* ctx, std::vector<int64_t>& idx, int64_t& lo, int64_t& hi) {
    lo = ctx->S;
    hi = 0;
    for (int64_t w = 0; w < ctx->W; ++w)
        if (ctx->win_hi[w] > ctx->win_lo[w]) {
            idx.push_back(w);
            lo = std::min(lo, ctx->win_lo[w]);
            hi = std::max(hi, ctx->win_hi[w]);
        }
}

size_t pair_batch_size(int Hk, size_t extra) {
    const char* e = getenv("PG_PAIR_SCRATCH_MB");
    size_t mb = e ? (size_t)atoll(e) : 3072;
    if (mb < 1) mb = 1;
    return std::max<size_t>(1, std::min<size_t>((mb << 20) / ((size_t)Hk * Hk * 8 + extra), 65535));
}

template <class Body>
int for_each_batch(pg_ctx* ctx, const std::vector<int64_t>& wins, const int64_t* lo, const int64_t* hi, size_t per_batch,
                   Body&& body) {
    for (size_t b0 = 0; b0 < wins.size(); b0 += per_batch) {
        const size_t nb = std::min(per_batch, wins.size() - b0);
        std::vector<int64_t> blo(nb), bhi(nb);
        for (size_t k = 0; k < nb; ++k) {
            blo[k] = lo[wins[b0 + k]];
            bhi[k] = hi[wins[b0 + k]];
        }
        PG_TRY(ctx->misc3.ensure(nb * 16 + 64));
        int64_t* d_lo = (int64_t*)ctx->misc3.p;
        int64_t* d_hi = d_lo + nb;
        PG_CUDA(cudaMemcpyAsync(d_lo, blo.data(), nb * 8, cudaMemcpyHostToDevice, ctx->stream));
        PG_CUDA(cudaMemcpyAsync(d_hi, bhi.data(), nb * 8, cudaMemcpyHostToDevice, ctx->stream));
        PG_TRY(body(b0, nb, (const int64_t*)d_lo, (const int64_t*)d_hi));
    }
    return PG_OK;
}

int copy_rows_back(pg_ctx* ctx, const std::vector<int64_t>& wins, size_t b0, size_t nb, const void* d_src, void* h_dst,
                   size_t row_bytes, bool staged = false) {
    size_t k = 0;
    while (k < nb) {
        size_t e = k + 1;
        while (e < nb && wins[b0 + e] == wins[b0 + e - 1] + 1) ++e;
        uint8_t* dst = (uint8_t*)h_dst + (size_t)wins[b0 + k] * row_bytes;
        const uint8_t* src = (const uint8_t*)d_src + k * row_bytes;
        if (staged) PG_TRY(pg_d2h_staged(ctx, dst, src, (e - k) * row_bytes));
        else PG_CUDA(cudaMemcpyAsync(dst, src, (e - k) * row_bytes, cudaMemcpyDeviceToHost, ctx->stream));
        k = e;
    }
    PG_CUDA(cudaStreamSynchronize(ctx->stream));
    return PG_OK;
}

}

int pg_k2_popgen_windows(pg_ctx* ctx, const std::vector<int64_t>& wins, const int64_t* win_lo, const int64_t* win_hi,
                         int32_t min_sites, double min_data, void* d_rec, int RC) {
    const int P = ctx->P;
    std::vector<int32_t> order, pop_start;
    PG_TRY(group_rows(ctx, ctx->hap_pop.data(), P, nullptr, order, pop_start));
    int64_t lo = ctx->S, hi = 0;
    for (int64_t w : wins) {
        lo = std::min(lo, win_lo[w]);
        hi = std::max(hi, win_hi[w]);
    }
    PlaneSet ps;
    PG_TRY(build_planes(ctx, order, lo, hi, ps));
    const size_t per_batch = pair_batch_size(ps.Hk, 0);
    PG_TRY(ctx->misc.ensure((size_t)(P + 1) * 4 + per_batch * 8 + 128));
    PG_CUDA(cudaMemcpyAsync(ctx->misc.p, pop_start.data(), (size_t)(P + 1) * 4, cudaMemcpyHostToDevice, ctx->stream));
    int64_t* d_widx = reinterpret_cast<int64_t*>((uint8_t*)ctx->misc.p + (((size_t)(P + 1) * 4 + 63) / 64) * 64);
    return for_each_batch(ctx, wins, win_lo, win_hi, per_batch, [&](size_t b0, size_t nb, const int64_t* d_lo, const int64_t* d_hi) {
        int32_t *d_diff = nullptr, *d_n = nullptr;
        PG_TRY(run_pair_batch(ctx, ps, d_lo, d_hi, (int)nb, &d_diff, &d_n));
        PG_CUDA(cudaMemcpyAsync(d_widx, wins.data() + b0, nb * 8, cudaMemcpyHostToDevice, ctx->stream));
        PopEpiParams ep;
        ep.diff = d_diff;
        ep.n = d_n;
        ep.mid = ps.d_mid;
        ep.Hm = ps.Hm;
        ep.Hk = ps.Hk;
        ep.P = P;
        ep.pop_start = (const int32_t*)ctx->misc.p;
        ep.min_sites = min_sites;
        ep.min_data = min_data;
        ep.rec = (unsigned long long*)d_rec;
        ep.RC = RC;
        ep.win_idx = d_widx;
        const int nblk = P * (P + 1) / 2;
        PG_TRY(ctx->misc5.ensure(nb * (size_t)nblk * 16 + 64));
        ep.blk_s = (double*)ctx->misc5.p;
        ep.blk_c = (long long*)(ep.blk_s + nb * (size_t)nblk);
        bool by_pairs = ps.tensor && ps.Hm * 2 == ps.Hk && (size_t)nblk * 64 <= 48 * 1024;
        for (int X = 0; X <= P; ++X) by_pairs = by_pairs && (pop_start[X] % 2 == 0);
        const unsigned nsplit = (unsigned)std::max<int64_t>(1, std::min<int64_t>(nblk, (8 * (int64_t)ctx->sm_count + (int64_t)nb - 1) / (int64_t)nb));
        PG_TRY(pg_timed(ctx, by_pairs ? "k2_popgen_epi_pairs" : "k2_popgen_epi_blocks", [&] {
            if (by_pairs) k2_popgen_epi_pairs<<<dim3((unsigned)nb, nsplit), 128, (size_t)nblk * 64, ctx->stream>>>(ep);
            else k2_popgen_epi_blocks<<<dim3((unsigned)nblk, (unsigned)nb), 256, 0, ctx->stream>>>(ep);
            k2_popgen_epi_final<<<(unsigned)((nb + 127) / 128), 128, 0, ctx->stream>>>(ep, (int)nb);
        }));
        ctx->launches += 1;
        PG_CUDA(cudaStreamSynchronize(ctx->stream));
        return PG_OK;
    });
}

extern "C" int pg_pairdist(pg_ctx* ctx, int32_t n_ind, const int32_t* hap_ind, int32_t include_same_with_same,
                           int32_t min_sites, double* dist, int64_t* n_sites, int64_t* pos_sum) {
    PG_CHECK(ctx && hap_ind && dist, "pg_pairdist: null argument");
    PG_CHECK(n_ind >= 1, "pg_pairdist: n_ind must be >= 1");
    PG_CHECK(ctx->H > 0, "pg_pairdist: upload genotypes first");
    PG_CUDA(cudaSetDevice(ctx->device));
    pg_timings_reset(ctx);
    const int64_t W = ctx->W;
    if (W == 0) return PG_OK;
    std::vector<int32_t> order, ind_start;
    PG_TRY(group_rows(ctx, hap_ind, n_ind, "pg_pairdist: hap_ind", order, ind_start));
    const size_t nn = (size_t)n_ind * n_ind;
    std::vector<int64_t> wins;
    int64_t lo, hi;
    nonempty_windows(ctx, wins, lo, hi);
    for (int64_t w = 0; w < W; ++w) {
        if (n_sites) n_sites[w] = ctx->win_hi[w] - ctx->win_lo[w];
        if (ctx->win_hi[w] <= ctx->win_lo[w])
            for (size_t k = 0; k < nn; ++k) dist[(size_t)w * nn + k] = NAN;
    }
    if (pos_sum) {
        std::vector<int32_t> hp((size_t)std::max<int64_t>(ctx->S, 1));
        if (ctx->S > 0)
            PG_CUDA(cudaMemcpy(hp.data(), ctx->d_pos, (size_t)ctx->S * 4, cudaMemcpyDeviceToHost));
        std::vector<int64_t> pre((size_t)ctx->S + 1, 0);
        for (int64_t s = 0; s < ctx->S; ++s) pre[s + 1] = pre[s] + hp[s];
        for (int64_t w = 0; w < W; ++w) pos_sum[w] = pre[ctx->win_hi[w]] - pre[ctx->win_lo[w]];
    }
    if (wins.empty()) return PG_OK;
    PlaneSet ps;
    PG_TRY(build_planes(ctx, order, lo, hi, ps));
    const size_t per_batch = pair_batch_size(ps.Hk, nn * 8);
    PG_TRY(ctx->misc.ensure((size_t)(n_ind + 1) * 4 + 64));
    PG_CUDA(cudaMemcpyAsync(ctx->misc.p, ind_start.data(), (size_t)(n_ind + 1) * 4, cudaMemcpyHostToDevice, ctx->stream));
    PG_TRY(ctx->out_d.ensure(per_batch * nn * 8 + 64));
    return for_each_batch(ctx, wins, ctx->win_lo.data(), ctx->win_hi.data(), per_batch,
                          [&](size_t b0, size_t nb, const int64_t* d_lo, const int64_t* d_hi) {
        int32_t *d_diff = nullptr, *d_n = nullptr;
        PG_TRY(run_pair_batch(ctx, ps, d_lo, d_hi, (int)nb, &d_diff, &d_n));
        IndEpiParams ep;
        ep.diff = d_diff;
        ep.n = d_n;
        ep.mid = ps.d_mid;
        ep.Hm = ps.Hm;
        ep.Hk = ps.Hk;
        ep.n_ind = n_ind;
        ep.ind_start = (const int32_t*)ctx->misc.p;
        ep.include_same = include_same_with_same ? 1 : 0;
        ep.min_sites = min_sites;
        ep.out = (double*)ctx->out_d.p;
        PG_TRY(pg_timed(ctx, "k2_ind_epi", [&] {
            k2_ind_epi<<<dim3((unsigned)std::min<int>((n_ind + 7) / 8, 64), (unsigned)nb), 256, 0, ctx->stream>>>(ep);
        }));
        return copy_rows_back(ctx, wins, b0, nb, ctx->out_d.p, dist, nn * 8, true);
    });
}

extern "C" int pg_distpaint(pg_ctx* ctx, int32_t n_query, const int32_t* query_hap, int32_t P, const int32_t* ref_off,
                            const int32_t* ref_hap, int32_t min_sites, int32_t mode, double threshold, int32_t noresult,
                            int32_t* out, double* means, double* pvals) {
    PG_CHECK(ctx && query_hap && ref_off && ref_hap && out, "pg_distpaint: null argument");
    PG_CHECK(ctx->H > 0, "pg_distpaint: upload genotypes first");
    PG_CHECK(n_query >= 1, "pg_distpaint: n_query must be >= 1");
    PG_CHECK(P >= 1 && P <= PAINT_MAX_POPS, "pg_distpaint: P=%d populations; the epilogue takes 1 to %d (one lane each)", P,
             PAINT_MAX_POPS);
    PG_CHECK(mode == 0 || mode == 1, "pg_distpaint: mode %d is neither 0 (rank-sum rule) nor 1 (delta rule)", mode);
    PG_CHECK(mode == 0 || P >= 2, "pg_distpaint: the delta rule compares the two lowest means and needs two populations");
    PG_CHECK(min_sites >= 1, "pg_distpaint: min_sites must be >= 1");
    PG_CHECK(ref_off[0] == 0, "pg_distpaint: ref_off[0] must be 0");
    for (int p = 0; p < P; ++p)
        PG_CHECK(ref_off[p + 1] > ref_off[p], "pg_distpaint: reference population %d has no member entries", p);
// ... 13 lines not shown
    nonempty_windows(ctx, wins, lo, hi);
    if (wins.empty()) return PG_OK;
    PlaneSet ps;
    PG_TRY(build_planes(ctx, all_rows(H), lo, hi, ps));
    PG_TRY(ctx->misc.ensure((size_t)(n_query + P + 1 + M) * 4 + 64));
    int32_t* d_query = (int32_t*)ctx->misc.p;
    int32_t* d_off = d_query + n_query;
    int32_t* d_ref = d_off + P + 1;
    PG_CUDA(cudaMemcpyAsync(d_query, query_hap, (size_t)n_query * 4, cudaMemcpyHostToDevice, ctx->stream));
    PG_CUDA(cudaMemcpyAsync(d_off, ref_off, (size_t)(P + 1) * 4, cudaMemcpyHostToDevice, ctx->stream));
    PG_CUDA(cudaMemcpyAsync(d_ref, ref_hap, (size_t)M * 4, cudaMemcpyHostToDevice, ctx->stream));
    const size_t qp = (size_t)n_query * P;
    const int n_dbl = (means ? 1 : 0) + (pvals ? 1 : 0);
    const size_t per_batch = pair_batch_size(ps.Hk, (size_t)n_query * 4 + qp * 8 * n_dbl);
    PG_TRY(ctx->out_i.ensure(per_batch * n_query * 4 + 64));
    PG_TRY(ctx->out_d.ensure(per_batch * qp * 8 * std::max(n_dbl, 1) + 64));
    const size_t smem = (size_t)PAINT_WARPS * M * 8;
    return for_each_batch(ctx, wins, ctx->win_lo.data(), ctx->win_hi.data(), per_batch,
                          [&](size_t b0, size_t nb, const int64_t* d_lo, const int64_t* d_hi) {
        int32_t *d_diff = nullptr, *d_n = nullptr;
        PG_TRY(run_pair_batch(ctx, ps, d_lo, d_hi, (int)nb, &d_diff, &d_n));
        PaintEpiParams ep;
        ep.diff = d_diff;
        ep.n = d_n;
        ep.mid = ps.d_mid;
        ep.Hm = ps.Hm;
        ep.Hk = ps.Hk;
        ep.n_query = n_query;
        ep.query_row = d_query;
        ep.P = P;
        ep.M = M;
        ep.ref_off = d_off;
        ep.ref_row = d_ref;
        ep.min_sites = min_sites;
        ep.mode = mode;
        ep.threshold = threshold;
        ep.noresult = noresult;
        ep.out = (int32_t*)ctx->out_i.p;
        ep.means = means ? (double*)ctx->out_d.p : nullptr;
        ep.pvals = pvals ? (double*)ctx->out_d.p + (means ? nb * qp : 0) : nullptr;
        PG_TRY(pg_timed(ctx, "k2_paint_epi", [&] {
            k2_paint_epi<<<dim3((unsigned)((n_query + PAINT_WARPS - 1) / PAINT_WARPS), (unsigned)nb), PAINT_WARPS * 32, smem,
                           ctx->stream>>>(ep);
        }));
        if (means) PG_TRY(copy_rows_back(ctx, wins, b0, nb, ep.means, means, qp * 8));
        if (pvals) PG_TRY(copy_rows_back(ctx, wins, b0, nb, ep.pvals, pvals, qp * 8));
        return copy_rows_back(ctx, wins, b0, nb, ep.out, out, (size_t)n_query * 4);
    });
}

extern "C" int pg_pair_counts(pg_ctx* ctx, int64_t window, int32_t* diff, int32_t* n) {
    PG_CHECK(ctx && diff && n, "pg_pair_counts: null argument");
    PG_CHECK(window >= 0 && window < ctx->W, "pg_pair_counts: window %lld out of range", (long long)window);
    PG_CUDA(cudaSetDevice(ctx->device));
    pg_timings_reset(ctx);
    const int H = ctx->H;
    const size_t HH = (size_t)H * H;
    const int64_t lo = ctx->win_lo[window], hi = ctx->win_hi[window];
    if (hi <= lo) {
        memset(diff, 0, HH * 4);
        memset(n, 0, HH * 4);
        return PG_OK;
    }
    PlaneSet ps;
    PG_TRY(build_planes(ctx, all_rows(H), lo, hi, ps));
    int32_t *d_diff = nullptr, *d_n = nullptr;
    PG_TRY(for_each_batch(ctx, std::vector<int64_t>(1, window), ctx->win_lo.data(), ctx->win_hi.data(), 1,
                          [&](size_t, size_t, const int64_t* d_lo, const int64_t* d_hi) {
        return run_pair_batch(ctx, ps, d_lo, d_hi, 1, &d_diff, &d_n);
    }));
    std::vector<int32_t> nu((size_t)ps.Hm * ps.Hm);
    PG_CUDA(cudaMemcpyAsync(diff, d_diff, HH * 4, cudaMemcpyDeviceToHost, ctx->stream));
    PG_CUDA(cudaMemcpyAsync(nu.data(), d_n, nu.size() * 4, cudaMemcpyDeviceToHost, ctx->stream));
    PG_CUDA(cudaStreamSynchronize(ctx->stream));
    for (int i = 0; i < H; ++i)
        for (int j = 0; j < H; ++j) {
            const int a = std::min(ps.mid[i], ps.mid[j]), b = std::max(ps.mid[i], ps.mid[j]);
            n[(size_t)i * H + j] = nu[(size_t)a * ps.Hm + b];
            if (j < i) diff[(size_t)i * H + j] = diff[(size_t)j * H + i];
        }
    return PG_OK;
}

extern "C" int pg_ind_het(pg_ctx* ctx, int32_t n_ind, const int32_t* hap_ind, int32_t min_sites, double* het) {
    PG_CHECK(ctx && hap_ind && het, "pg_ind_het: null argument");
    PG_CHECK(n_ind >= 1, "pg_ind_het: n_ind must be >= 1");
    PG_CHECK(ctx->H > 0, "pg_ind_het: upload genotypes first");
    PG_CUDA(cudaSetDevice(ctx->device));
    pg_timings_reset(ctx);
    const int64_t W = ctx->W;
    if (W == 0) return PG_OK;
    std::vector<int32_t> order, ind_start;
    PG_TRY(group_rows(ctx, hap_ind, n_ind, "pg_ind_het: hap_ind", order, ind_start));
    for (size_t k = 0; k < (size_t)W * n_ind; ++k) het[k] = NAN;
    std::vector<int64_t> wins;
    int64_t lo, hi;
    nonempty_windows(ctx, wins, lo, hi);
    if (wins.empty() || order.empty()) return PG_OK;
    PlaneSet ps;
    PG_TRY(build_planes(ctx, order, lo, hi, ps));
    PG_TRY(ctx->misc.ensure((size_t)(n_ind + 1) * 4 + 64));
    PG_CUDA(cudaMemcpyAsync(ctx->misc.p, ind_start.data(), (size_t)(n_ind + 1) * 4, cudaMemcpyHostToDevice, ctx->stream));
    return for_each_batch(ctx, wins, ctx->win_lo.data(), ctx->win_hi.data(), 65535,
                          [&](size_t b0, size_t nb, const int64_t* d_lo, const int64_t* d_hi) {
        PG_TRY(ctx->out_d.ensure(nb * (size_t)n_ind * 8 + 64));
        PG_TRY(run_het(ctx, ps, d_lo, d_hi, (int)nb, (const int32_t*)ctx->misc.p, n_ind, min_sites, (double*)ctx->out_d.p));
        return copy_rows_back(ctx, wins, b0, nb, ctx->out_d.p, het, (size_t)n_ind * 8);
    });
}

extern "C" int pg_hapstats(pg_ctx* ctx, double max_dist, int32_t min_sites, int32_t diag_nan, double* out) {
    PG_CHECK(ctx && out, "pg_hapstats: null argument");
    PG_CHECK(ctx->P >= 1, "pg_hapstats: call pg_set_pops first");
    PG_CHECK(ctx->P <= PG_MAX_POPS, "pg_hapstats: P=%d > %d populations", ctx->P, PG_MAX_POPS);
    PG_CUDA(cudaSetDevice(ctx->device));
    pg_timings_reset(ctx);
    const int64_t W = ctx->W;
    const int P = ctx->P;
    if (W == 0) return PG_OK;
    std::vector<int32_t> order, pop_start;
    PG_TRY(group_rows(ctx, ctx->hap_pop.data(), P, nullptr, order, pop_start));
    int maxN = 0;
    for (int X = 0; X < P; ++X) {
        PG_CHECK(pop_start[X + 1] > pop_start[X], "pg_hapstats: population %d has no haplotypes", X);
        maxN = std::max(maxN, pop_start[X + 1] - pop_start[X]);
    }
    const size_t smem = (size_t)maxN * ((maxN + 31) / 32) * 4 + (size_t)((maxN + 31) / 32) * 4 + (size_t)maxN * 4 + 64;
    PG_CHECK(smem <= 200 * 1024, "pg_hapstats: a population of %d haplotypes is too large for the clustering kernel", maxN);
    for (size_t k = 0; k < (size_t)W * P * 3; ++k) out[k] = NAN;
    std::vector<int64_t> wins;
    int64_t lo, hi;
    nonempty_windows(ctx, wins, lo, hi);
    if (wins.empty()) return PG_OK;
    PlaneSet ps;
    PG_TRY(build_planes(ctx, order, lo, hi, ps));
    PG_TRY(ctx->misc.ensure((size_t)(P + 1) * 4 + 64));
    PG_CUDA(cudaMemcpyAsync(ctx->misc.p, pop_start.data(), (size_t)(P + 1) * 4, cudaMemcpyHostToDevice, ctx->stream));
    PG_CUDA(cudaFuncSetAttribute(k2_hap_epi, cudaFuncAttributeMaxDynamicSharedMemorySize, (int)smem));
    return for_each_batch(ctx, wins, ctx->win_lo.data(), ctx->win_hi.data(), pair_batch_size(ps.Hk, 0),
                          [&](size_t b0, size_t nb, const int64_t* d_lo, const int64_t* d_hi) {
        int32_t *d_diff = nullptr, *d_n = nullptr;
        PG_TRY(run_pair_batch(ctx, ps, d_lo, d_hi, (int)nb, &d_diff, &d_n));
        PG_TRY(ctx->out_d.ensure(nb * (size_t)P * 24 + 64));
        HapEpiParams ep;
        ep.diff = d_diff;
        ep.n = d_n;
        ep.mid = ps.d_mid;
        ep.Hm = ps.Hm;
        ep.Hk = ps.Hk;
        ep.P = P;
        ep.pop_start = (const int32_t*)ctx->misc.p;
        ep.min_sites = min_sites;
        ep.diag_nan = diag_nan ? 1 : 0;
        ep.max_dist = max_dist;
        ep.out = (double*)ctx->out_d.p;
        PG_TRY(pg_timed(ctx, "k2_hap_epi", [&] {
            k2_hap_epi<<<dim3((unsigned)P, (unsigned)nb), 256, smem, ctx->stream>>>(ep);
        }));
        return copy_rows_back(ctx, wins, b0, nb, ctx->out_d.p, out, (size_t)P * 24);
    });
}

extern "C" int pg_pairdist_cat(pg_ctx* ctx, int32_t n_ind, const int32_t* hap_ind, int32_t include_same_with_same,
                               double* dist, int64_t* total_sites) {
    PG_CHECK(ctx && hap_ind && dist, "pg_pairdist_cat: null argument");
    PG_CHECK(n_ind >= 1, "pg_pairdist_cat: n_ind must be >= 1");
// ... 82 lines not shown
```

genomics_general_b200/csrc/k2t.cu:

```cuda
#include <stdlib.h>

#include <algorithm>

#include "pgwin_internal.h"

namespace {

__device__ __forceinline__ uint32_t smem_u32(const void* p) { return (uint32_t)__cvta_generic_to_shared(p); }
__device__ __forceinline__ void mbar_init(uint64_t* bar, uint32_t count) {
    asm volatile("mbarrier.init.shared::cta.b64 [%0], %1;" ::"r"(smem_u32(bar)), "r"(count) : "memory");
}
__device__ __forceinline__ void mbar_arrive(uint64_t* bar) {
    asm volatile("mbarrier.arrive.shared::cta.b64 _, [%0];" ::"r"(smem_u32(bar)) : "memory");
}
__device__ __forceinline__ void mbar_expect_tx(uint64_t* bar, uint32_t bytes) {
    asm volatile("mbarrier.arrive.expect_tx.shared::cta.b64 _, [%0], %1;" ::"r"(smem_u32(bar)), "r"(bytes) : "memory");
}
__device__ __forceinline__ void bulk_g2s(void* dst, const void* src, uint32_t bytes, uint64_t* bar) {
    asm volatile("cp.async.bulk.shared::cluster.global.mbarrier::complete_tx::bytes [%0], [%1], %2, [%3];" ::"r"(smem_u32(dst)),
                 "l"(src), "r"(bytes), "r"(smem_u32(bar))
                 : "memory");
}
__device__ __forceinline__ void mbar_wait(uint64_t* bar, uint32_t parity) {
    uint32_t ok;
// ... 272 lines not shown
#pragma unroll
            for (int k = 0; k < 8; ++k) {
#define PQ_WORD(C)                                         \
    {                                                      \
        op.C |= ((w[k].C >> psh[k]) & 0x01010101u) << k;   \
        uint32_t t = w[k].C & qm[k];                       \
        t |= t >> 4;                                       \
        t |= t >> 2;                                       \
        oq.C |= (t & 0x01010101u) << k;                    \
    }
                PQ_WORD(x)
                PQ_WORD(y)
                PQ_WORD(z)
                PQ_WORD(w)
#undef PQ_WORD
            }
            reinterpret_cast<uint4*>(pq_st + (0 * 8 + o) * p.pw)[q] = op;
            reinterpret_cast<uint4*>(pq_st + (1 * 8 + o) * p.pw)[q] = oq;
        }
        __syncthreads();
        for (int cw = tid; cw < p.pw; cw += 256) {
            uint32_t a[8], plo[4], phi[4], qlo[4], qhi[4];
#pragma unroll
            for (int q = 0; q < 8; ++q) a[q] = pq_st[q * p.pw + cw];
            octets_to_words(a, plo, phi);
#pragma unroll
            for (int q = 0; q < 8; ++q) a[q] = pq_st[(8 + q) * p.pw + cw];
            octets_to_words(a, qlo, qhi);
            const int4 r4 = *reinterpret_cast<const int4*>(p.c2r + 4 * cw);
            const int rr[4] = {r4.x, r4.y, r4.z, r4.w};
#pragma unroll
            for (int j = 0; j < 4; ++j) {
                if (rr[j] < 0) continue;
                p.pq[(chunk * 2 + 0) * p.R + rr[j]] = (uint64_t)plo[j] | ((uint64_t)phi[j] << 32);
                p.pq[(chunk * 2 + 1) * p.R + rr[j]] = (uint64_t)qlo[j] | ((uint64_t)qhi[j] << 32);
            }
        }
        for (int r = p.Hk + tid; r < p.R; r += 256) {
            p.pq[(chunk * 2 + 0) * p.R + r] = 0ull;
            p.pq[(chunk * 2 + 1) * p.R + r] = 0ull;
        }
        __syncthreads();
    }
}

struct GramGroup {
    int a_row0;
    int b_row0;
    int nb_rows;
    int pad;
};
struct GramParams {
    const uint64_t* plane;
    int R, Hk;
    int64_t site_base;
    const int64_t* win_lo;
    const int64_t* win_hi;
    const int32_t* cps;
    const GramGroup* groups;
    int ngroups;
    int nb;
    int brows;
    int a_sep;
    int nstages;
    int nraw;
    int64_t nchunks;
    int32_t* out;
};

constexpr int GRAM_CTHREADS = 256;
constexpr int GRAM_THREADS = GRAM_CTHREADS + 32;
constexpr int GRAM_MAX_RAW = 48;
constexpr int GRAM_BMAX = 256;
constexpr int GRAM_ACC = GRAM_BMAX / 2;

__device__ __forceinline__ uint4 expand16(uint32_t x) {
    uint4 r;
    r.x = ((x & 0xfu) * 0x00204081u) & 0x01010101u;
    r.y = (((x >> 4) & 0xfu) * 0x00204081u) & 0x01010101u;
    r.z = (((x >> 8) & 0xfu) * 0x00204081u) & 0x01010101u;
    r.w = (((x >> 12) & 0xfu) * 0x00204081u) & 0x01010101u;
    return r;
}

__device__ __forceinline__ uint64_t gmma_desc(uint32_t saddr) {
    return (uint64_t)((saddr & 0x3ffffu) >> 4) | ((uint64_t)(128u >> 4) << 16) | ((uint64_t)(256u >> 4) << 32);
}

template <int N>
__device__ __forceinline__ void wgmma_u8(uint32_t (&d)[GRAM_ACC], uint64_t a, uint64_t b);
template <>
__device__ __forceinline__ void wgmma_u8<64>(uint32_t (&d)[GRAM_ACC], uint64_t a, uint64_t b) {
    asm volatile(
        "{\n\t.reg .pred p;\n\tsetp.ne.b32 p, 1, 0;\n\twgmma.mma_async.sync.aligned.m64n64k32.s32.u8.u8 {"
        "%0,%1,%2,%3,%4,%5,%6,%7,%8,%9,%10,%11,%12,%13,%14,%15,"
        "%16,%17,%18,%19,%20,%21,%22,%23,%24,%25,%26,%27,%28,%29,%30,%31"
        "}, %32, %33, p;\n\t}"
        : "+r"(d[0]), "+r"(d[1]), "+r"(d[2]), "+r"(d[3]), "+r"(d[4]), "+r"(d[5]), "+r"(d[6]), "+r"(d[7]),
          "+r"(d[8]), "+r"(d[9]), "+r"(d[10]), "+r"(d[11]), "+r"(d[12]), "+r"(d[13]), "+r"(d[14]), "+r"(d[15]),
          "+r"(d[16]), "+r"(d[17]), "+r"(d[18]), "+r"(d[19]), "+r"(d[20]), "+r"(d[21]), "+r"(d[22]), "+r"(d[23]),
          "+r"(d[24]), "+r"(d[25]), "+r"(d[26]), "+r"(d[27]), "+r"(d[28]), "+r"(d[29]), "+r"(d[30]), "+r"(d[31])
        : "l"(a), "l"(b));
}
template <>
__device__ __forceinline__ void wgmma_u8<128>(uint32_t (&d)[GRAM_ACC], uint64_t a, uint64_t b) {
    asm volatile(
        "{\n\t.reg .pred p;\n\tsetp.ne.b32 p, 1, 0;\n\twgmma.mma_async.sync.aligned.m64n128k32.s32.u8.u8 {"
        "%0,%1,%2,%3,%4,%5,%6,%7,%8,%9,%10,%11,%12,%13,%14,%15,"
        "%16,%17,%18,%19,%20,%21,%22,%23,%24,%25,%26,%27,%28,%29,%30,%31,"
        "%32,%33,%34,%35,%36,%37,%38,%39,%40,%41,%42,%43,%44,%45,%46,%47,"
        "%48,%49,%50,%51,%52,%53,%54,%55,%56,%57,%58,%59,%60,%61,%62,%63"
        "}, %64, %65, p;\n\t}"
        : "+r"(d[0]), "+r"(d[1]), "+r"(d[2]), "+r"(d[3]), "+r"(d[4]), "+r"(d[5]), "+r"(d[6]), "+r"(d[7]),
          "+r"(d[8]), "+r"(d[9]), "+r"(d[10]), "+r"(d[11]), "+r"(d[12]), "+r"(d[13]), "+r"(d[14]), "+r"(d[15]),
          "+r"(d[16]), "+r"(d[17]), "+r"(d[18]), "+r"(d[19]), "+r"(d[20]), "+r"(d[21]), "+r"(d[22]), "+r"(d[23]),
          "+r"(d[24]), "+r"(d[25]), "+r"(d[26]), "+r"(d[27]), "+r"(d[28]), "+r"(d[29]), "+r"(d[30]), "+r"(d[31]),
          "+r"(d[32]), "+r"(d[33]), "+r"(d[34]), "+r"(d[35]), "+r"(d[36]), "+r"(d[37]), "+r"(d[38]), "+r"(d[39]),
          "+r"(d[40]), "+r"(d[41]), "+r"(d[42]), "+r"(d[43]), "+r"(d[44]), "+r"(d[45]), "+r"(d[46]), "+r"(d[47]),
          "+r"(d[48]), "+r"(d[49]), "+r"(d[50]), "+r"(d[51]), "+r"(d[52]), "+r"(d[53]), "+r"(d[54]), "+r"(d[55]),
          "+r"(d[56]), "+r"(d[57]), "+r"(d[58]), "+r"(d[59]), "+r"(d[60]), "+r"(d[61]), "+r"(d[62]), "+r"(d[63])
        : "l"(a), "l"(b));
}
template <>
__device__ __forceinline__ void wgmma_u8<192>(uint32_t (&d)[GRAM_ACC], uint64_t a, uint64_t b) {
    asm volatile(
        "{\n\t.reg .pred p;\n\tsetp.ne.b32 p, 1, 0;\n\twgmma.mma_async.sync.aligned.m64n192k32.s32.u8.u8 {"
        "%0,%1,%2,%3,%4,%5,%6,%7,%8,%9,%10,%11,%12,%13,%14,%15,"
        "%16,%17,%18,%19,%20,%21,%22,%23,%24,%25,%26,%27,%28,%29,%30,%31,"
        "%32,%33,%34,%35,%36,%37,%38,%39,%40,%41,%42,%43,%44,%45,%46,%47,"
        "%48,%49,%50,%51,%52,%53,%54,%55,%56,%57,%58,%59,%60,%61,%62,%63,"
        "%64,%65,%66,%67,%68,%69,%70,%71,%72,%73,%74,%75,%76,%77,%78,%79,"
        "%80,%81,%82,%83,%84,%85,%86,%87,%88,%89,%90,%91,%92,%93,%94,%95"
        "}, %96, %97, p;\n\t}"
        : "+r"(d[0]), "+r"(d[1]), "+r"(d[2]), "+r"(d[3]), "+r"(d[4]), "+r"(d[5]), "+r"(d[6]), "+r"(d[7]),
          "+r"(d[8]), "+r"(d[9]), "+r"(d[10]), "+r"(d[11]), "+r"(d[12]), "+r"(d[13]), "+r"(d[14]), "+r"(d[15]),
          "+r"(d[16]), "+r"(d[17]), "+r"(d[18]), "+r"(d[19]), "+r"(d[20]), "+r"(d[21]), "+r"(d[22]), "+r"(d[23]),
          "+r"(d[24]), "+r"(d[25]), "+r"(d[26]), "+r"(d[27]), "+r"(d[28]), "+r"(d[29]), "+r"(d[30]), "+r"(d[31]),
          "+r"(d[32]), "+r"(d[33]), "+r"(d[34]), "+r"(d[35]), "+r"(d[36]), "+r"(d[37]), "+r"(d[38]), "+r"(d[39]),
          "+r"(d[40]), "+r"(d[41]), "+r"(d[42]), "+r"(d[43]), "+r"(d[44]), "+r"(d[45]), "+r"(d[46]), "+r"(d[47]),
          "+r"(d[48]), "+r"(d[49]), "+r"(d[50]), "+r"(d[51]), "+r"(d[52]), "+r"(d[53]), "+r"(d[54]), "+r"(d[55]),
          "+r"(d[56]), "+r"(d[57]), "+r"(d[58]), "+r"(d[59]), "+r"(d[60]), "+r"(d[61]), "+r"(d[62]), "+r"(d[63]),
          "+r"(d[64]), "+r"(d[65]), "+r"(d[66]), "+r"(d[67]), "+r"(d[68]), "+r"(d[69]), "+r"(d[70]), "+r"(d[71]),
          "+r"(d[72]), "+r"(d[73]), "+r"(d[74]), "+r"(d[75]), "+r"(d[76]), "+r"(d[77]), "+r"(d[78]), "+r"(d[79]),
          "+r"(d[80]), "+r"(d[81]), "+r"(d[82]), "+r"(d[83]), "+r"(d[84]), "+r"(d[85]), "+r"(d[86]), "+r"(d[87]),
          "+r"(d[88]), "+r"(d[89]), "+r"(d[90]), "+r"(d[91]), "+r"(d[92]), "+r"(d[93]), "+r"(d[94]), "+r"(d[95])
        : "l"(a), "l"(b));
}
template <>
__device__ __forceinline__ void wgmma_u8<256>(uint32_t (&d)[GRAM_ACC], uint64_t a, uint64_t b) {
    asm volatile(
        "{\n\t.reg .pred p;\n\tsetp.ne.b32 p, 1, 0;\n\twgmma.mma_async.sync.aligned.m64n256k32.s32.u8.u8 {"
        "%0,%1,%2,%3,%4,%5,%6,%7,%8,%9,%10,%11,%12,%13,%14,%15,"
        "%16,%17,%18,%19,%20,%21,%22,%23,%24,%25,%26,%27,%28,%29,%30,%31,"
        "%32,%33,%34,%35,%36,%37,%38,%39,%40,%41,%42,%43,%44,%45,%46,%47,"
        "%48,%49,%50,%51,%52,%53,%54,%55,%56,%57,%58,%59,%60,%61,%62,%63,"
        "%64,%65,%66,%67,%68,%69,%70,%71,%72,%73,%74,%75,%76,%77,%78,%79,"
        "%80,%81,%82,%83,%84,%85,%86,%87,%88,%89,%90,%91,%92,%93,%94,%95,"
        "%96,%97,%98,%99,%100,%101,%102,%103,%104,%105,%106,%107,%108,%109,%110,%111,"
        "%112,%113,%114,%115,%116,%117,%118,%119,%120,%121,%122,%123,%124,%125,%126,%127"
        "}, %128, %129, p;\n\t}"
        : "+r"(d[0]), "+r"(d[1]), "+r"(d[2]), "+r"(d[3]), "+r"(d[4]), "+r"(d[5]), "+r"(d[6]), "+r"(d[7]),
          "+r"(d[8]), "+r"(d[9]), "+r"(d[10]), "+r"(d[11]), "+r"(d[12]), "+r"(d[13]), "+r"(d[14]), "+r"(d[15]),
          "+r"(d[16]), "+r"(d[17]), "+r"(d[18]), "+r"(d[19]), "+r"(d[20]), "+r"(d[21]), "+r"(d[22]), "+r"(d[23]),
          "+r"(d[24]), "+r"(d[25]), "+r"(d[26]), "+r"(d[27]), "+r"(d[28]), "+r"(d[29]), "+r"(d[30]), "+r"(d[31]),
          "+r"(d[32]), "+r"(d[33]), "+r"(d[34]), "+r"(d[35]), "+r"(d[36]), "+r"(d[37]), "+r"(d[38]), "+r"(d[39]),
          "+r"(d[40]), "+r"(d[41]), "+r"(d[42]), "+r"(d[43]), "+r"(d[44]), "+r"(d[45]), "+r"(d[46]), "+r"(d[47]),
          "+r"(d[48]), "+r"(d[49]), "+r"(d[50]), "+r"(d[51]), "+r"(d[52]), "+r"(d[53]), "+r"(d[54]), "+r"(d[55]),
          "+r"(d[56]), "+r"(d[57]), "+r"(d[58]), "+r"(d[59]), "+r"(d[60]), "+r"(d[61]), "+r"(d[62]), "+r"(d[63]),
          "+r"(d[64]), "+r"(d[65]), "+r"(d[66]), "+r"(d[67]), "+r"(d[68]), "+r"(d[69]), "+r"(d[70]), "+r"(d[71]),
          "+r"(d[72]), "+r"(d[73]), "+r"(d[74]), "+r"(d[75]), "+r"(d[76]), "+r"(d[77]), "+r"(d[78]), "+r"(d[79]),
          "+r"(d[80]), "+r"(d[81]), "+r"(d[82]), "+r"(d[83]), "+r"(d[84]), "+r"(d[85]), "+r"(d[86]), "+r"(d[87]),
          "+r"(d[88]), "+r"(d[89]), "+r"(d[90]), "+r"(d[91]), "+r"(d[92]), "+r"(d[93]), "+r"(d[94]), "+r"(d[95]),
          "+r"(d[96]), "+r"(d[97]), "+r"(d[98]), "+r"(d[99]), "+r"(d[100]), "+r"(d[101]), "+r"(d[102]), "+r"(d[103]),
          "+r"(d[104]), "+r"(d[105]), "+r"(d[106]), "+r"(d[107]), "+r"(d[108]), "+r"(d[109]), "+r"(d[110]), "+r"(d[111]),
          "+r"(d[112]), "+r"(d[113]), "+r"(d[114]), "+r"(d[115]), "+r"(d[116]), "+r"(d[117]), "+r"(d[118]), "+r"(d[119]),
          "+r"(d[120]), "+r"(d[121]), "+r"(d[122]), "+r"(d[123]), "+r"(d[124]), "+r"(d[125]), "+r"(d[126]), "+r"(d[127])
        : "l"(a), "l"(b));
}
__device__ __forceinline__ void wgmma_fence() { asm volatile("wgmma.fence.sync.aligned;" ::: "memory"); }
__device__ __forceinline__ void wgmma_commit() { asm volatile("wgmma.commit_group.sync.aligned;" ::: "memory"); }
__device__ __forceinline__ void wgmma_wait_all() { asm volatile("wgmma.wait_group.sync.aligned 0;" ::: "memory"); }
__device__ __forceinline__ void consumers_sync() { asm volatile("bar.sync 1, %0;" ::"n"(GRAM_CTHREADS) : "memory"); }

__device__ __forceinline__ bool elect_one() {
    uint32_t pred;
    asm volatile("{\n\t.reg .pred p;\n\telect.sync _|p, 0xffffffff;\n\tselp.u32 %0, 1, 0, p;\n\t}" : "=r"(pred));
    return pred != 0;
}

struct GramItem {
    GramGroup g;
    int wb;
    int64_t lo, hi, c_first;
    int nst;
};
template <int NPL, int CH>
__device__ __forceinline__ GramItem gram_item(const GramParams& gp, int64_t j) {
    constexpr int SH = 6 + (CH == 4 ? 2 : (CH == 2 ? 1 : 0));
    GramItem it;
    it.wb = (int)(j / gp.ngroups);
    it.g = gp.groups[j - (int64_t)it.wb * gp.ngroups];
    it.lo = gp.win_lo[it.wb] - gp.site_base;
    it.hi = gp.win_hi[it.wb] - gp.site_base;
    if (NPL == 2) {
        it.lo = gp.cps[it.lo];
        it.hi = gp.cps[it.hi];
    }
    it.c_first = it.lo >> SH;
    it.nst = (it.hi > it.lo) ? (int)(((it.hi - 1) >> SH) - it.c_first + 1) : 0;
    return it;
}

template <int NPL, int CH, int N>
__device__ __forceinline__ void gram_stage_mma(uint32_t (&acc)[GRAM_ACC], uint32_t st, uint32_t a_off, uint32_t b_off,
                                               uint32_t blk) {
#pragma unroll
    for (int ks = 0; ks < 2 * CH; ++ks) {
        if (NPL == 1) {
            const uint32_t bk = st + ks * blk;
            wgmma_u8<N>(acc, gmma_desc(bk + a_off), gmma_desc(bk + b_off));
        } else {
            const uint32_t bp = st + (ks * 2) * blk, bq = bp + blk;
            wgmma_u8<N>(acc, gmma_desc(bp + a_off), gmma_desc(bq + b_off));
            wgmma_u8<N>(acc, gmma_desc(bq + a_off), gmma_desc(bp + b_off));
        }
    }
}

template <int NPL, int CH>
__global__ void __launch_bounds__(GRAM_THREADS, 1) k2t_gram(const __grid_constant__ GramParams gp) {
    static_assert(CH == 1 || CH == 2 || CH == 4, "chunks per stage");
    constexpr int GRAM_MAX_ITEMS = ((128 + GRAM_BMAX) * NPL + GRAM_CTHREADS - 1) / GRAM_CTHREADS;
    extern __shared__ __align__(128) uint8_t gsm[];
    __shared__ __align__(8) uint64_t raw_full[GRAM_MAX_RAW], raw_empty[GRAM_MAX_RAW];
    const int tid = threadIdx.x, warp = tid >> 5;
    const int NS = gp.nstages, RD = gp.nraw;
    const int AOFF = gp.a_sep ? 128 : 0;
    const int RROWS = AOFF + gp.brows;
    const int RAW1 = NPL * RROWS * 8;
    const int RAW = CH * RAW1;
    const int BLK = RROWS * 32;
    const int STAGE = CH * 2 * NPL * BLK;
    uint8_t* const raw_base = gsm;
    uint8_t* const op_base = gsm + (size_t)RD * RAW;

    const int64_t n_items = (int64_t)gp.nb * gp.ngroups;
    const int64_t j0 = n_items * blockIdx.x / gridDim.x, j1 = n_items * (blockIdx.x + 1) / gridDim.x;

    if (tid == 0) {
        for (int s = 0; s < RD; ++s) {
            mbar_init(&raw_full[s], 1);
            mbar_init(&raw_empty[s], 1);
        }
        asm volatile("fence.mbarrier_init.release.cluster;" ::: "memory");
    }
    __syncthreads();

    if (__shfl_sync(0xffffffffu, warp, 0) == GRAM_CTHREADS / 32) {
        int n_done = 0, rs = 0;
        uint32_t rph = 0;
        for (int64_t j = j0; j < j1; ++j) {
            const GramItem im = gram_item<NPL, CH>(gp, j);
            const bool a_in_b = (im.g.a_row0 == im.g.b_row0);
            const int a_rows = a_in_b ? 0 : min(128, gp.R - im.g.a_row0);
            const uint32_t bytes_a = (uint32_t)a_rows * 8u, bytes_b = (uint32_t)im.g.nb_rows * 8u;
            for (int it = 0; it < im.nst; ++it) {
                if (n_done >= RD) mbar_wait(&raw_empty[rs], rph ^ 1u);
                if (elect_one()) {
                    mbar_expect_tx(&raw_full[rs], CH * NPL * (bytes_a + bytes_b));
#pragma unroll
                    for (int h = 0; h < CH; ++h) {
                        const int64_t chunk = min((im.c_first + it) * CH + h, gp.nchunks - 1);
#pragma unroll
                        for (int pl = 0; pl < NPL; ++pl) {
                            const uint64_t* src = gp.plane + (chunk * NPL + pl) * gp.R;
                            uint8_t* dst = raw_base + (size_t)rs * RAW + (size_t)h * RAW1 + (size_t)pl * RROWS * 8;
                            if (bytes_a) bulk_g2s(dst, src + im.g.a_row0, bytes_a, &raw_full[rs]);
                            bulk_g2s(dst + AOFF * 8, src + im.g.b_row0, bytes_b, &raw_full[rs]);
                        }
                    }
                }
                __syncwarp();
                ++n_done;
                if (++rs == RD) {
                    rs = 0;
                    rph ^= 1u;
                }
            }
        }
        return;
    }

    const int wg = warp >> 2, lane = tid & 31, wq = warp & 3;
    const uint32_t op16 = smem_u32(op_base);
    int rs = 0, os = 0;
    uint32_t rph = 0;
    uint32_t acc[GRAM_ACC];
    for (int64_t j = j0; j < j1; ++j) {
        const GramItem im = gram_item<NPL, CH>(gp, j);
        const bool a_in_b = (im.g.a_row0 == im.g.b_row0);
        const int skip_a = a_in_b ? 128 : 0;
        const int rows_tot = 128 + im.g.nb_rows - skip_a;
        const int nitems = rows_tot * NPL;
        int r_idx[GRAM_MAX_ITEMS], d_off[GRAM_MAX_ITEMS];
#pragma unroll
        for (int q = 0; q < GRAM_MAX_ITEMS; ++q) {
            const int item = tid + q * GRAM_CTHREADS;
            r_idx[q] = -1;
            d_off[q] = 0;
            if (item < nitems) {
                const int pl = (NPL == 2 && item >= rows_tot) ? 1 : 0;
                const int rr = item - pl * rows_tot + skip_a;
                const int x = (rr < 128) ? rr : rr - 128;
                const int row = (rr < 128) ? x : AOFF + x;
                r_idx[q] = (rr < 128 && im.g.a_row0 + x >= gp.R) ? -2 : pl * RROWS + row;
                d_off[q] = pl * BLK + (row >> 3) * 256 + (row & 7) * 16;
            }
        }
        const uint32_t a_off = (uint32_t)((a_in_b ? AOFF : 0) + 64 * wg) * 32u, b_off = (uint32_t)AOFF * 32u;
        const int nsel = __shfl_sync(0xffffffffu, (min(im.g.nb_rows, GRAM_BMAX) + 63) / 64, 0);
#pragma unroll
        for (int e = 0; e < GRAM_ACC; ++e) acc[e] = 0u;
        for (int it = 0; it < im.nst; ++it) {
            uint64_t mask[CH];
#pragma unroll
            for (int h = 0; h < CH; ++h) {
                const int64_t b0 = ((im.c_first + it) * CH + h) << 6;
                uint64_t m = 0ull;
                if (b0 < im.hi && b0 + 64 > im.lo) {
                    m = ~0ull;
                    if (im.lo > b0) m &= ~0ull << (int)(im.lo - b0);
                    if (im.hi < b0 + 64) m &= ~0ull >> (int)(b0 + 64 - im.hi);
                }
                mask[h] = m;
            }
            mbar_wait(&raw_full[rs], rph);
            const uint64_t* rw = reinterpret_cast<const uint64_t*>(raw_base + (size_t)rs * RAW);
            uint64_t v[GRAM_MAX_ITEMS][CH];
#pragma unroll
            for (int q = 0; q < GRAM_MAX_ITEMS; ++q)
#pragma unroll
                for (int h = 0; h < CH; ++h) v[q][h] = (r_idx[q] >= 0) ? (rw[h * (RAW1 / 8) + r_idx[q]] & mask[h]) : 0ull;
            if (NS == 1) {
                wgmma_wait_all();
                consumers_sync();
            }
            uint8_t* sb = op_base + (size_t)os * STAGE;
#pragma unroll
            for (int q = 0; q < GRAM_MAX_ITEMS; ++q) {
                if (q * GRAM_CTHREADS < nitems && r_idx[q] != -1) {
#pragma unroll
                    for (int h = 0; h < CH; ++h) {
                        const uint32_t wlo = (uint32_t)v[q][h], whi = (uint32_t)(v[q][h] >> 32);
                        uint8_t* d0 = sb + (size_t)h * 2 * NPL * BLK + d_off[q];
                        uint8_t* d1 = d0 + NPL * BLK;
                        *reinterpret_cast<uint4*>(d0) = expand16(wlo & 0xffffu);
                        *reinterpret_cast<uint4*>(d0 + 128) = expand16(wlo >> 16);
                        *reinterpret_cast<uint4*>(d1) = expand16(whi & 0xffffu);
                        *reinterpret_cast<uint4*>(d1 + 128) = expand16(whi >> 16);
                    }
                }
            }
            asm volatile("fence.proxy.async.shared::cta;" ::: "memory");
            wgmma_wait_all();
            consumers_sync();
            if (tid == 0) mbar_arrive(&raw_empty[rs]);
            wgmma_fence();
            const uint32_t st = op16 + (uint32_t)os * (uint32_t)STAGE;
            switch (nsel) {
                case 1: gram_stage_mma<NPL, CH, 64>(acc, st, a_off, b_off, (uint32_t)BLK); break;
                case 2: gram_stage_mma<NPL, CH, 128>(acc, st, a_off, b_off, (uint32_t)BLK); break;
                case 3: gram_stage_mma<NPL, CH, 192>(acc, st, a_off, b_off, (uint32_t)BLK); break;
                default: gram_stage_mma<NPL, CH, 256>(acc, st, a_off, b_off, (uint32_t)BLK); break;
            }
            wgmma_commit();
            if (++rs == RD) {
                rs = 0;
                rph ^= 1u;
            }
            if (++os == NS) os = 0;
        }
        wgmma_wait_all();
        const int i0 = im.g.a_row0 + 64 * wg + 16 * wq + (lane >> 2);
        const bool pair_ok = (gp.Hk & 1) == 0;
#pragma unroll
        for (int e = 0; e < GRAM_ACC; e += 2) {
            const int c = 8 * (e >> 2) + 2 * (lane & 3);
            const int i = i0 + 8 * ((e >> 1) & 1), jc = im.g.b_row0 + c;
            if (c < im.g.nb_rows && i < gp.Hk && jc < gp.Hk) {
                int32_t* o = gp.out + (size_t)im.wb * gp.Hk * gp.Hk + (size_t)i * gp.Hk + jc;
                if (pair_ok) {
                    *reinterpret_cast<int2*>(o) = make_int2((int32_t)acc[e], (int32_t)acc[e + 1]);
                } else {
                    o[0] = (int32_t)acc[e];
                    if (jc + 1 < gp.Hk) o[1] = (int32_t)acc[e + 1];
                }
            }
        }
    }
}

__device__ __forceinline__ uint64_t chunk_mask(int64_t chunk, int64_t lo, int64_t hi) {
    uint64_t m = ~0ull;
    const int64_t b0 = chunk << 6;
    if (lo > b0) m &= ~0ull << (int)(lo - b0);
    if (hi < b0 + 64) m &= ~0ull >> (int)(b0 + 64 - hi);
    return m;
}

__global__ void __launch_bounds__(128) k2t_seq_nonnan(const uint64_t* __restrict__ vplane, int R, int Hk, int64_t site_base,
                                                      const int64_t* __restrict__ win_lo, const int64_t* __restrict__ win_hi,
                                                      long long* __restrict__ out) {
    const int r = blockIdx.x * 128 + threadIdx.x, wb = blockIdx.y;
    if (r >= Hk) return;
    const int64_t lo = win_lo[wb] - site_base, hi = win_hi[wb] - site_base;
    long long n = 0;
    if (hi > lo)
        for (int64_t c = lo >> 6; c <= (hi - 1) >> 6; ++c) n += __popcll(vplane[c * R + r] & chunk_mask(c, lo, hi));
    out[(size_t)wb * Hk + r] = n;
}

__global__ void __launch_bounds__(128) k2t_het(const uint64_t* __restrict__ vplane, const uint64_t* __restrict__ pq,
                                               const int32_t* __restrict__ cps, int R, int64_t site_base,
                                               const int64_t* __restrict__ win_lo, const int64_t* __restrict__ win_hi,
                                               const int32_t* __restrict__ ind_start, int n_ind, int min_sites,
                                               double* __restrict__ out) {
    const int a = blockIdx.x * 128 + threadIdx.x, wb = blockIdx.y;
    if (a >= n_ind) return;
    const double nan = __longlong_as_double(0x7ff8000000000000ll);
    const int r0 = ind_start[a], r1 = ind_start[a + 1];
    double v = nan;
    if (r1 - r0 == 2) {
        const int64_t lo = win_lo[wb] - site_base, hi = win_hi[wb] - site_base;
        long long n = 0, diff = 0;
        if (hi > lo) {
            for (int64_t c = lo >> 6; c <= (hi - 1) >> 6; ++c)
                n += __popcll(vplane[c * R + r0] & vplane[c * R + r0 + 1] & chunk_mask(c, lo, hi));
            const int64_t plo = cps[lo], phi = cps[hi];
            if (phi > plo)
                for (int64_t c = plo >> 6; c <= (phi - 1) >> 6; ++c) {
                    const uint64_t p0 = pq[(c * 2) * R + r0], p1 = pq[(c * 2) * R + r0 + 1];
                    const uint64_t q0 = pq[(c * 2 + 1) * R + r0], q1 = pq[(c * 2 + 1) * R + r0 + 1];
// ... 78 lines not shown
    vp.pair_flag = d_off + nchunk + 1;
    PG_CUDA(cudaMemsetAsync(vp.pair_flag, 0, 4, ctx->stream));
    const int grid1 = (int)std::min<int64_t>(nchunk, (int64_t)ctx->sm_count * 8);
    bool all_used = true;
    for (int c = 0; c < ctx->H; ++c) all_used = all_used && c2r[c] >= 0;
    PG_TRY(pg_timed(ctx, "k2t_valid_class", [&] {
        if (all_used) k2t_valid_class<true><<<grid1, 256, (size_t)8 * pw * 4 + (size_t)R * 8, ctx->stream>>>(vp);
        else k2t_valid_class<false><<<grid1, 256, (size_t)8 * pw * 4 + (size_t)R * 8, ctx->stream>>>(vp);
    }));
    PG_TRY(pg_timed(ctx, "k2t_scan", [&] { k2t_scan<<<1, 1024, 0, ctx->stream>>>(vp.chunk_tot, d_off, nchunk); }));
    int32_t tf[2] = {0, 0};
    PG_CUDA(cudaMemcpyAsync(tf, d_off + nchunk, 8, cudaMemcpyDeviceToHost, ctx->stream));
    PG_CUDA(cudaStreamSynchronize(ctx->stream));
    const int32_t total = tf[0];
    const bool pairs_ok = want_pairs && tf[1] == 0;
    const int64_t nchunk_d = ((int64_t)total + 63) / 64;
    off = 0;
    const size_t o_inv = carve((size_t)std::max<int64_t>(total, 1) * 8), o_pq = carve((size_t)std::max<int64_t>(nchunk_d, 1) * 2 * R * 8);
    PG_TRY(ctx->planes2.ensure(off));
    uint8_t* base2 = (uint8_t*)ctx->planes2.p;
    const int gridi = (int)std::min<int64_t>((nchunk + 7) / 8, (int64_t)ctx->sm_count * 16);
    PG_TRY(pg_timed(ctx, "k2t_inv", [&] {
        k2t_inv<<<gridi, 256, 0, ctx->stream>>>(vp.cls, d_off, nchunk, d_cps, (uint2*)(base2 + o_inv));
    }));
    if (nchunk_d > 0) {
        PqParams pp;
        pp.geno32 = vp.geno32;
        pp.pw = pw;
        pp.pitch = pitch;
        pp.site_base = sb;
        pp.total = total;
        pp.nchunk = nchunk_d;
        pp.inv = (const uint2*)(base2 + o_inv);
        pp.c2r = d_c2r;
        pp.pq = (uint64_t*)(base2 + o_pq);
        pp.R = R;
        pp.Hk = Hk;
        const size_t smem = (size_t)16 * pw * 4;
        const int grid2 = (int)std::min<int64_t>(nchunk_d, (int64_t)ctx->sm_count * 8);
        PG_TRY(pg_timed(ctx, "k2t_build_pq", [&] { k2t_build_pq<<<grid2, 256, smem, ctx->stream>>>(pp); }));
    }
    ps.Hk = Hk;
    ps.R = R;
    ps.site_base = sb;
    ps.nchunk_v = nchunk;
    ps.vplane = vp.vplane;
    ps.cps = d_cps;
    ps.npseudo = total;
    ps.pq = (uint64_t*)(base2 + o_pq);
    ps.Hm = pairs_ok ? Hk / 2 : Hk;
    ps.R2 = R2;
    ps.vpair = pairs_ok ? vp.vpair : nullptr;
    if (pairs_ok) {
        int32_t* d_mid = (int32_t*)(base + o_mid);
        k2t_half<<<(Hk + 255) / 256, 256, 0, ctx->stream>>>(d_mid, Hk);
        ps.d_mid = d_mid;
    } else {
        ps.d_mid = d_iota;
    }
    return PG_OK;
}

namespace {
void gram_groups(int R, std::vector<GramGroup>& groups, int& brows, int& a_sep) {
    groups.clear();
    int nbmax = 16;
    a_sep = 0;
    for (int a0 = 0; a0 < R; a0 += 128)
        for (int c = a0; c < R; c += GRAM_BMAX) {
            GramGroup g;
            g.a_row0 = a0;
            g.b_row0 = c;
            g.nb_rows = std::min(GRAM_BMAX, R - c);
            g.pad = 0;
            nbmax = std::max(nbmax, g.nb_rows);
            if (c != a0) a_sep = 1;
            groups.push_back(g);
        }
    brows = std::max(128, (nbmax + 63) / 64 * 64);
}
}

int pg_k2t_pairs(pg_ctx* ctx, const K2TPlanes& ps, const int64_t* d_lo, const int64_t* d_hi, int nb, int32_t* d_diff,
                 int32_t* d_n) {
    const int budget = 227 * 1024 - 1024;
    PG_TRY((pg_smem_limit<k2t_gram<1, 1>>(ctx, budget)));
    PG_TRY((pg_smem_limit<k2t_gram<1, 2>>(ctx, budget)));
    PG_TRY((pg_smem_limit<k2t_gram<1, 4>>(ctx, budget)));
    PG_TRY((pg_smem_limit<k2t_gram<2, 1>>(ctx, budget)));
    const int Rn = ps.vpair ? ps.R2 : ps.R;
    std::vector<GramGroup> gn, gd;
    int brows_n, asep_n, brows_d, asep_d;
    gram_groups(Rn, gn, brows_n, asep_n);
    gram_groups(ps.R, gd, brows_d, asep_d);
    PG_TRY(ctx->misc4.ensure((gn.size() + gd.size()) * sizeof(GramGroup) + 64));
    GramGroup* d_gn = (GramGroup*)ctx->misc4.p;
    GramGroup* d_gd = d_gn + gn.size();
    PG_CUDA(cudaMemcpyAsync(d_gn, gn.data(), gn.size() * sizeof(GramGroup), cudaMemcpyHostToDevice, ctx->stream));
    PG_CUDA(cudaMemcpyAsync(d_gd, gd.data(), gd.size() * sizeof(GramGroup), cudaMemcpyHostToDevice, ctx->stream));
    GramParams gp;
    gp.site_base = ps.site_base;
    gp.win_lo = d_lo;
    gp.win_hi = d_hi;
    gp.nb = nb;
    auto geometry = [&](int npl, int brows, int a_sep, int ch, int& nstages, int& nraw) {
        const int rrows = (a_sep ? 128 : 0) + brows;
        const int stage = ch * 2 * npl * rrows * 32, raw = ch * npl * rrows * 8;
        nstages = 2;
        if (const char* e = getenv("PG_K2T_NSTAGES")) nstages = std::max(1, std::min(nstages, atoi(e)));
        nraw = std::min(GRAM_MAX_RAW, (budget - nstages * stage) / raw);
        if (const char* e = getenv("PG_K2T_NRAW")) nraw = std::min(nraw, atoi(e));
        nraw = std::max(1, nraw);
        return (size_t)nstages * stage + (size_t)nraw * raw;
    };
    {
        gp.R = Rn;
        gp.Hk = ps.Hm;
        gp.groups = d_gn;
        gp.ngroups = (int)gn.size();
        gp.brows = brows_n;
        gp.a_sep = asep_n;
        int ch_n = 4;
        if (const char* e = getenv("PG_K2T_CH")) ch_n = std::min(ch_n, std::max(1, atoi(e)));
        size_t smem = geometry(1, brows_n, asep_n, ch_n, gp.nstages, gp.nraw);
        while (ch_n > 1 && (smem > (size_t)budget || gp.nraw < 2)) {
            ch_n /= 2;
            smem = geometry(1, brows_n, asep_n, ch_n, gp.nstages, gp.nraw);
        }
        PG_CHECK(smem <= (size_t)budget, "pairwise path: %d mask rows do not fit the Gram kernel's shared memory", Rn);
        gp.plane = ps.vpair ? ps.vpair : ps.vplane;
        gp.nchunks = ps.nchunk_v;
        gp.cps = nullptr;
        gp.out = d_n;
        const unsigned grid = (unsigned)std::min<int64_t>((int64_t)nb * gp.ngroups, ctx->sm_count);
        PG_TRY(pg_timed(ctx, "k2t_gram_n", [&] {
            if (ch_n == 4) k2t_gram<1, 4><<<grid, GRAM_THREADS, smem, ctx->stream>>>(gp);
            else if (ch_n == 2) k2t_gram<1, 2><<<grid, GRAM_THREADS, smem, ctx->stream>>>(gp);
            else k2t_gram<1, 1><<<grid, GRAM_THREADS, smem, ctx->stream>>>(gp);
        }));
    }
    {
        gp.R = ps.R;
        gp.Hk = ps.Hk;
        gp.groups = d_gd;
        gp.ngroups = (int)gd.size();
        gp.brows = brows_d;
        gp.a_sep = asep_d;
        const size_t smem = geometry(2, brows_d, asep_d, 1, gp.nstages, gp.nraw);
        PG_CHECK(smem <= (size_t)budget, "pairwise path: %d haplotype rows do not fit the Gram kernel's shared memory", ps.R);
        gp.plane = ps.pq;
        gp.nchunks = (ps.npseudo + 63) / 64;
        gp.cps = ps.cps;
        gp.out = d_diff;
        const unsigned grid = (unsigned)std::min<int64_t>((int64_t)nb * gp.ngroups, ctx->sm_count);
        PG_TRY(pg_timed(ctx, "k2t_gram_diff", [&] { k2t_gram<2, 1><<<grid, GRAM_THREADS, smem, ctx->stream>>>(gp); }));
    }
    return PG_OK;
}

int pg_k2t_seq_nonnan(pg_ctx* ctx, const K2TPlanes& ps, const int64_t* d_lo, const int64_t* d_hi, int nb, long long* d_out) {
    return pg_timed(ctx, "k2_seq_nonnan", [&] {
        k2t_seq_nonnan<<<dim3((unsigned)((ps.Hk + 127) / 128), (unsigned)nb), 128, 0, ctx->stream>>>(ps.vplane, ps.R, ps.Hk,
                                                                                                    ps.site_base, d_lo, d_hi, d_out);
    });
}

int pg_k2t_het(pg_ctx* ctx, const K2TPlanes& ps, const int64_t* d_lo, const int64_t* d_hi, int nb, const int32_t* d_ind_start,
               int n_ind, int min_sites, double* d_out) {
    return pg_timed(ctx, "k2_het", [&] {
        k2t_het<<<dim3((unsigned)((n_ind + 127) / 128), (unsigned)nb), 128, 0, ctx->stream>>>(
            ps.vplane, ps.pq, ps.cps, ps.R, ps.site_base, d_lo, d_hi, d_ind_start, n_ind, min_sites, d_out);
    });
}
```

genomics_general_b200/csrc/pgwin_internal.h:

```cpp
#pragma once

#include <cuda_runtime.h>
#include <stdint.h>
#include <stdio.h>
#include <string.h>

#include <string>
#include <vector>

#include "../../include/pgwin.h"

#define PG_OK 0
#define PG_ERR 1

void pg_set_error(const char* fmt, ...);

#define PG_CUDA(call)                                                                                  \
    do {                                                                                               \
        cudaError_t _e = (call);                                                                       \
        if (_e != cudaSuccess) {                                                                       \
            pg_set_error("%s:%d: %s failed: %s", __FILE__, __LINE__, #call, cudaGetErrorString(_e));  \
            return PG_ERR;                                                                             \
        }                                                                                              \
    } while (0)

#define PG_CHECK(cond, ...)                 \
    do {                                    \
        if (!(cond)) {                      \
            pg_set_error(__VA_ARGS__);      \
            return PG_ERR;                  \
        }                                   \
    } while (0)

#define PG_TRY(expr)                 \
    do {                             \
        int _r = (expr);             \
        if (_r != PG_OK) return _r;  \
    } while (0)

struct PgTiming {
    char name[32];
    cudaEvent_t start, stop;
    int launches;
};

struct PgBuf {
    void* p = nullptr;
    size_t cap = 0;
    int ensure(size_t bytes);
    void release();
};

static constexpr int PG_MAX_K1_POPS = 8;
static constexpr int PG_MAX_POPS = 64;

struct K1Plan {
    int pitch;
    int chunks;
    int G;
    int I;
    int wpt;
    int nw;
    int T;
    int stages;
    int tile_bytes;
    int smem_bytes;
    int64_t num_tiles;
    int ctas;
};
K1Plan pg_make_k1_plan(int64_t S, int H, int sm_count, int table_bytes, int nw = 8, int force_G = 0);
K1Plan pg_make_k1_plan_rows(int64_t S, int pitch, int sm_count, int table_bytes, int nw, int force_G);
int pg_k1_ring_stages(int tile_bytes, int table_bytes);
int pg_k1_plan_ok(const K1Plan& p);
int pg_pitch_for(int H);
int pg_packed_pitch_for(int H);

enum { PG_CLS_VARIED = 0, PG_CLS_A = 1, PG_CLS_C = 2, PG_CLS_G = 3, PG_CLS_T = 4, PG_CLS_MISSING = 5, PG_CLS_VARIED2 = 6,
       PG_CLS_VARIED2_B1 = 7 };
__host__ __device__ inline bool pg_cls_varied(unsigned c) { return c == PG_CLS_VARIED || c >= PG_CLS_VARIED2; }
__host__ __device__ inline bool pg_cls_biallelic(unsigned c) { return c >= PG_CLS_VARIED2; }

struct pg_ctx {
    int device = 0;
    int sm_count = 132;
    cudaStream_t stream = nullptr;
    int8_t* d_geno = nullptr;
    int32_t* d_pos = nullptr;
    int64_t S = 0;
    int32_t H = 0;
    int32_t pitch = 0;
    size_t geno_cap = 0, pos_cap = 0;
    uint32_t* d_packed = nullptr;
    int32_t packed_pitch = 0;
    size_t packed_cap = 0;
    uint8_t* d_site_cls = nullptr;
    size_t cls_cap = 0;
    int32_t P = 0;
    std::vector<int32_t> hap_pop;
    int64_t W = 0;
    std::vector<int64_t> win_lo, win_hi;
    std::vector<int64_t> brk;
    std::vector<int32_t> win_seg_lo, win_seg_hi;
    std::vector<PgTiming> timings;
    std::vector<cudaEvent_t> event_pool;
    size_t events_used = 0;
    int64_t launches = 0;
    PgBuf tables, part, segmeta, winmeta, out_d, out_i, planes, planes2, pairs, misc, misc2, misc3, misc4, misc5;
    PgBuf text, starts, meta;
    int64_t ingest_sites = -1;
    int32_t ingest_fmt = 0;
    int32_t ingest_strict = 0;
    int64_t ingest_geom[5] = {0, 0, 0, 0, 0};
    uint64_t text_gen = 0;
    PgBuf flt_aux, flt_tab, flt_stats, flt_rows, flt_off, flt_out, flt_cub;
    void* flt_state = nullptr;
    void* vcf_state = nullptr;
    void* seq_state = nullptr;
    void* g2v_state = nullptr;
    void* s2g_state = nullptr;
    void* ws_state = nullptr;
    void* h_text[2] = {nullptr, nullptr};
    cudaEvent_t h_text_free[2] = {nullptr, nullptr};
    cudaStream_t copy_stream = nullptr;
    PgBuf stage[2];
    cudaEvent_t stage_full[2] = {nullptr, nullptr}, stage_free[2] = {nullptr, nullptr};
    bool want_freq = false;
    uint64_t epoch = 1;
    uint64_t data_gen = 1;
    void* k1_cache[3] = {nullptr, nullptr, nullptr};
    std::vector<unsigned long long> h_rec;
    void* nccl_comm = nullptr;
    int nccl_ranks = 1, nccl_rank = 0;
    PgBuf gather;
    PgBuf gather_flag;
    cudaStream_t gather_stream = nullptr;
    cudaEvent_t g_rec[2] = {nullptr, nullptr}, g_done[2] = {nullptr, nullptr};
    PgBuf gslot[2];
    void* gslot_host[2] = {nullptr, nullptr};
    size_t gslot_host_cap[2] = {0, 0}, gslot_words[2] = {0, 0};
    int64_t gslot_wmax[2] = {0, 0};
    int32_t gslot_min_sites[2] = {0, 0};
    double gslot_min_data[2] = {0, 0};
    int64_t gslot_W[2] = {0, 0};
    int32_t gslot_RC[2] = {0, 0};
    std::vector<int64_t> gslot_lo[2], gslot_hi[2];
    uint64_t gslot_gen[2] = {0, 0};
    void* h_pinned = nullptr;
    size_t h_pinned_cap = 0;
    PgBuf sfs_acc_k[2], sfs_acc_r[2], sfs_slab, sfs_merge, sfs_cub;
    int sfs_cur = 0;
    int64_t sfs_total = -1;
};

void pg_timings_reset(pg_ctx* ctx);
int pg_time_begin(pg_ctx* ctx, const char* name);
void pg_time_end(pg_ctx* ctx, int idx);
int pg_pinned(pg_ctx* ctx, size_t bytes, void** out);
int pg_d2h_staged(pg_ctx* ctx, void* dst, const void* src, size_t bytes);
int pg_build_segments(pg_ctx* ctx);
int pg_pack_rows(pg_ctx* ctx, int64_t s0, int64_t n);

template <class Launch>
int pg_timed(pg_ctx* ctx, const char* name, Launch&& launch) {
    const int ti = pg_time_begin(ctx, name);
    launch();
    pg_time_end(ctx, ti);
    PG_CUDA(cudaGetLastError());
    return PG_OK;
}

template <auto Kern>
int pg_smem_limit(const pg_ctx* ctx, int bytes) {
    static bool set[64] = {};
    if (!set[ctx->device & 63]) {
        PG_CUDA(cudaFuncSetAttribute(Kern, cudaFuncAttributeMaxDynamicSharedMemorySize, bytes));
        set[ctx->device & 63] = true;
    }
    return PG_OK;
}

struct K2TPlanes {
    int Hk = 0, R = 0;
    int64_t site_base = 0;
    int64_t nchunk_v = 0;
    const uint64_t* vplane = nullptr;
    const int32_t* cps = nullptr;
    int64_t npseudo = 0;
    const uint64_t* pq = nullptr;
    int Hm = 0, R2 = 0;
    const uint64_t* vpair = nullptr;
    const int32_t* d_mid = nullptr;
};
bool pg_k2_use_tensor();
inline bool pg_k2t_fits(int pitch, int Hk) { return (size_t)16 * pitch + (size_t)((Hk + 15) / 16 * 16) * 8 <= 96 * 1024; }
int pg_k2t_build(pg_ctx* ctx, const std::vector<int32_t>& order, int64_t lo, int64_t hi, K2TPlanes& ps);
int pg_k2t_pairs(pg_ctx* ctx, const K2TPlanes& ps, const int64_t* d_lo, const int64_t* d_hi, int nb, int32_t* d_diff,
                 int32_t* d_n);
int pg_k2t_seq_nonnan(pg_ctx* ctx, const K2TPlanes& ps, const int64_t* d_lo, const int64_t* d_hi, int nb, long long* d_out);
int pg_k2t_het(pg_ctx* ctx, const K2TPlanes& ps, const int64_t* d_lo, const int64_t* d_hi, int nb, const int32_t* d_ind_start,
               int n_ind, int min_sites, double* d_out);

__device__ __forceinline__ int pg_freq_order(const int c[4], int rank[4]) {
    int nr = 0;
    for (int a = 0; a < 4; ++a) {
        rank[a] = 4;
        if (c[a] <= 0) continue;
        int before = 0;
        for (int b = 0; b < 4; ++b)
            if (c[b] > 0 && (c[b] > c[a] || (c[b] == c[a] && b > a))) ++before;
        rank[a] = before;
        ++nr;
    }
    return nr;
}

__device__ __forceinline__ bool pg_sblank(unsigned c) {
    return c == ' ' || c == '\t' || c == '\r' || c == '\v' || c == '\f' || (c >= 0x1c && c <= 0x1f);
}

__device__ __forceinline__ unsigned pg_byte_at(const uint8_t* buf, size_t len, size_t i) { return i < len ? buf[i] : (unsigned)'\n'; }

template <class OnField>
__device__ __forceinline__ unsigned pg_warp_fields(const uint8_t* buf, size_t len, size_t l0, bool* hi, bool* lone_cr,
                                                   OnField&& on_field) {
    const int lane = threadIdx.x & 31;
    const size_t a0 = l0 & ~(size_t)3;
    unsigned fields_before = 0;
    bool prev_ws = true, any_hi = false, any_cr = false, done = false;
    for (size_t step = 0; !done; ++step) {
        const size_t wbase = a0 + step * 128 + (size_t)lane * 4;
        uint32_t w = 0x0a0a0a0au;
        if (wbase + 4 <= len) w = *reinterpret_cast<const uint32_t*>(buf + wbase);
        else if (wbase < len) {
            for (int k = 0; k < 4; ++k)
                if (wbase + k < len) w = (w & ~(0xffu << (8 * k))) | ((uint32_t)buf[wbase + k] << (8 * k));
        }
        unsigned ws = 0, nl = 0, hb = 0, cr = 0;
#pragma unroll
        for (int k = 0; k < 4; ++k) {
            const unsigned c = (w >> (8 * k)) & 0xffu;
            const bool before = (wbase + k) < l0;
            if (before || pg_sblank(c)) ws |= 1u << k;
            else if (c == '\n') nl |= 1u << k;
            if (!before && c >= 0x80u) hb |= 1u << k;
            if (!before && c == '\r') cr |= 1u << k;
        }
        const unsigned nl_lanes = __ballot_sync(0xffffffffu, nl != 0);
        if (nl_lanes) {
            const int first = __ffs(nl_lanes) - 1;
            if (lane > first) ws = 0xfu, nl = 0, hb = 0, cr = 0;
            else if (lane == first) {
                const unsigned from = nl & (0u - nl);
                ws |= ~(from - 1u) & 0xfu;
                hb &= from - 1u;
                cr &= from - 1u;
            }
            done = true;
        }
        any_hi |= hb != 0;
        for (unsigned m = cr; m; m &= m - 1)
            if (pg_byte_at(buf, len, wbase + __ffs(m)) != '\n') any_cr = true;
        const unsigned last_ws = (ws >> 3) & 1u;
        unsigned pw = __shfl_up_sync(0xffffffffu, last_ws, 1);
        if (lane == 0) pw = prev_ws ? 1u : 0u;
        const unsigned prevbits = ((ws << 1) | pw) & 0xfu;
        const unsigned st = ~ws & prevbits & 0xfu;
        unsigned cnt = __popc(st), incl = cnt;
#pragma unroll
        for (int d = 1; d < 32; d <<= 1) {
            const unsigned v = __shfl_up_sync(0xffffffffu, incl, d);
            if (lane >= d) incl += v;
        }
        unsigned fidx = fields_before + incl - cnt;
        fields_before += __shfl_sync(0xffffffffu, incl, 31);
        prev_ws = (__shfl_sync(0xffffffffu, last_ws, 31) != 0);
        for (unsigned m = st; m; m &= m - 1, ++fidx) on_field(fidx, wbase + (__ffs(m) - 1));
    }
    *hi = __any_sync(0xffffffffu, any_hi);
    *lone_cr = __any_sync(0xffffffffu, any_cr);
    return fields_before;
// ... 30 lines not shown
```

genomics_general_b200/engine.py:

```python
from __future__ import annotations

import ctypes as C
import itertools

import numpy as np

from . import _lib
from ._lib import PgError, check


def _ptr(a):
    return a.ctypes.data_as(C.c_void_p) if a is not None else None


class PinnedArray:

    def __init__(self, shape, dtype):
        self._lib = _lib.lib()
        self.shape = tuple(int(s) for s in shape)
        self.dtype = np.dtype(dtype)
        nbytes = int(np.prod(self.shape)) * self.dtype.itemsize
        p = C.c_void_p()
        check(self._lib.pg_host_alloc(C.byref(p), max(nbytes, 1)), "pg_host_alloc")
        self._p = p
# ... 780 lines not shown
        assert hap_ind.shape == (self.H,)
        het = np.empty((self.W, n_ind), dtype=np.float64)
        check(self._lib.pg_ind_het(self._ctx, int(n_ind), _ptr(hap_ind), int(min_sites or 0), _ptr(het)), "pg_ind_het")
        return het

    def hapstats(self, max_dist: float = 0.0, min_sites: int = 0, diag_nan: bool = False):
        out = np.empty((self.W, self.P, 3), dtype=np.float64)
        check(self._lib.pg_hapstats(self._ctx, float(max_dist), int(min_sites or 0), 1 if diag_nan else 0, _ptr(out)),
              "pg_hapstats")
        return out

    def pair_counts(self, window: int):
        diff = np.empty((self.H, self.H), dtype=np.int32)
        n = np.empty((self.H, self.H), dtype=np.int32)
        check(self._lib.pg_pair_counts(self._ctx, int(window), _ptr(diff), _ptr(n)), "pg_pair_counts")
        return diff, n

    def last_timings(self):
        cap = 32
        names = (C.c_char * 32 * cap)()
        ms = (C.c_float * cap)()
        launches = (C.c_int32 * cap)()
        cnt = C.c_int32(0)
        check(self._lib.pg_last_timings(self._ctx, cap, names, ms, launches, C.byref(cnt)), "pg_last_timings")
        return {names[k].value.decode(): dict(ms=float(ms[k]), launches=int(launches[k])) for k in range(cnt.value)}

    def launch_count(self) -> int:
        n = C.c_int64(0)
        check(self._lib.pg_launch_count(self._ctx, C.byref(n)), "pg_launch_count")
        return int(n.value)

    def packed_rows(self, site0: int, n: int):
        words = C.c_int32(0)
        check(self._lib.pg_debug_packed(self._ctx, int(site0), int(n), C.byref(words), None), "pg_debug_packed")
        if words.value == 0:
            return None
        out = np.empty((n, words.value), dtype=np.uint32)
        check(self._lib.pg_debug_packed(self._ctx, int(site0), int(n), C.byref(words), _ptr(out)), "pg_debug_packed")
        wd = (self.H + 31) // 32
        return out[:, :3 * wd].reshape(n, 3, wd)

    def site_classes(self, site0: int, n: int):
        avail = C.c_int32(0)
        out = np.empty(int(n), dtype=np.uint8)
        check(self._lib.pg_debug_site_cls(self._ctx, int(site0), int(n), C.byref(avail), _ptr(out)), "pg_debug_site_cls")
        return out if avail.value else None

    def uniform_stream(self):
        in_use, varied = C.c_int32(0), C.c_int64(0)
        check(self._lib.pg_debug_uniform(self._ctx, C.byref(in_use), C.byref(varied)), "pg_debug_uniform")
        return bool(in_use.value), int(varied.value)

    def uniform_rows(self):
        n1, words = C.c_int64(0), C.c_int64(0)
        check(self._lib.pg_debug_uniform_rows(self._ctx, C.byref(n1), C.byref(words)), "pg_debug_uniform_rows")
        return int(n1.value), int(words.value)

    def uniform_tile(self):
        v = (C.c_int32 * 2)()
        check(self._lib.pg_debug_uniform_tile(self._ctx, v), "pg_debug_uniform_tile")
        return int(v[0]), int(v[1])

    def uniform_ring(self):
        v = (C.c_int32 * 3)()
        check(self._lib.pg_debug_uniform_ring(self._ctx, v), "pg_debug_uniform_ring")
        return int(v[0]), int(v[1]), int(v[2])

    def uniform_launch(self):
        v = (C.c_int32 * 3)()
        check(self._lib.pg_debug_uniform_launch(self._ctx, v), "pg_debug_uniform_launch")
        return int(v[0]), int(v[1]), int(v[2])

    def uniform_tiles(self):
        nt, geo = C.c_int64(0), (C.c_int32 * 2)()
        check(self._lib.pg_debug_uniform_tiles(self._ctx, 0, None, None, C.byref(nt), geo), "pg_debug_uniform_tiles")
        if nt.value == 0:
            return None
        site_lo = np.empty(nt.value + 1, np.int64)
        row0 = np.empty(nt.value + 1, np.int64)
        check(self._lib.pg_debug_uniform_tiles(self._ctx, nt.value + 1, _ptr(site_lo), _ptr(row0), C.byref(nt), geo),
              "pg_debug_uniform_tiles")
        return int(geo[0]), int(geo[1]), site_lo, row0


def k1_plan(S: int, H: int, nw: int = 8, lanes: int = 0, table_bytes: int = 4096):
    v = (C.c_int32 * 9)()
    check(_lib.lib().pg_debug_k1_plan_ex(int(S), int(H), int(nw), int(lanes), int(table_bytes), v), "pg_debug_k1_plan_ex")
    return dict(pitch=v[0], lanes_per_site=v[1], warps_per_tile=v[2], sites_per_lane=v[3], tile_sites=v[4], stages=v[5],
                smem_bytes=v[6], ctas=v[7], ok=bool(v[8]))
```

include/pgwin.h:

```cpp
#ifndef PGWIN_H
#define PGWIN_H

#include <stddef.h>
#include <stdint.h>

#ifdef __cplusplus
extern "C" {
#endif

typedef struct pg_ctx pg_ctx;

int         pg_version(void);
const char* pg_last_error(void);
int         pg_device_count(int* n);
int         pg_ctx_create(int device, pg_ctx** out);
int         pg_ctx_destroy(pg_ctx* ctx);
int         pg_host_alloc(void** ptr, size_t bytes);
int         pg_host_free(void* ptr);

int pg_upload(pg_ctx* ctx, const int8_t* geno, int64_t S, int32_t H, const int32_t* pos);
int pg_alloc_sites(pg_ctx* ctx, int64_t S, int32_t H);
int pg_upload_range(pg_ctx* ctx, int64_t site0, int64_t n, const int8_t* geno, const int32_t* pos);
int pg_append_sites(pg_ctx* ctx, int64_t n, const int8_t* geno, const int32_t* pos);
int pg_synth_fill(pg_ctx* ctx, int64_t S, int32_t n_pops, int32_t samples_per_pop, int32_t ploidy,
// ... 113 lines not shown
    int32_t has_nearly_fixed;
    double nearly_fixed_diff;
    int32_t partial_to_missing;
    int32_t no_test;
    int32_t thin_dist;
    int32_t pod_size;
} pg_filter_spec;

int pg_filter(pg_ctx* ctx, const pg_filter_spec* spec, const uint8_t* contig_mask, const int32_t* scaf_id, int64_t* n_kept,
              uint8_t* flags_or);
int pg_filter_emit(pg_ctx* ctx, int32_t fmt, int32_t freq_order, int64_t row0, char* out, size_t cap, int64_t* rows,
                   size_t* bytes);
int pg_filter_stats(pg_ctx* ctx, int64_t site0, int64_t n, int32_t* called, int32_t* het, int32_t* counts,
                    int32_t* pop_called, uint8_t* pop_mask, uint8_t* flags, uint8_t* keep, uint8_t* final_);

typedef struct {
    int64_t start;
    int64_t end;
    int64_t pos;
    uint32_t chrom_off, chrom_len, pos_off, pos_len, ref_off, ref_len, alt_off, alt_len, qual_off, qual_len, fmt_off, fmt_len;
    int32_t n_fields;
    int32_t n_alt;
    uint32_t flags;
    uint32_t reserved;
} pg_vcf_line;
#define PG_VCF_NONASCII 1u
#define PG_VCF_POS_UNRESOLVED 2u
#define PG_VCF_QUAL_DROP 4u
#define PG_VCF_QUAL_UNRESOLVED 8u
#define PG_VCF_SAME_LEN 16u
#define PG_VCF_DUPLICATE 32u
#define PG_VCF_FORMAT_WIDE 64u

typedef struct {
    int32_t n_cols;
    const int32_t* col_slot;
    const int32_t* col_prev;
    int32_t n_keys;
    const int32_t* key_off;
    const char* key_chars;
    int32_t n_samp;
    const int32_t* samp_col;
    const int32_t* samp_ploidy;
    int32_t field_key;
    int32_t field_phase;
    int32_t n_filt;
    const int32_t* filt_key;
    const double* filt_min;
    const double* filt_max;
    const uint8_t* filt_site;
    const uint8_t* filt_gt;
    const uint8_t* filt_samp;
    int32_t has_min_qual;
    double min_qual;
    const char* missing;
    int32_t missing_len;
    const char* sep;
    int32_t sep_len;
    int32_t skip_indels, keep_partial, ploidy_mismatch_to_missing, add_ref_track;
} pg_vcf_spec;

int pg_vcf_set_spec(pg_ctx* ctx, const pg_vcf_spec* spec);
int pg_vcf_load(pg_ctx* ctx, const char* text, size_t len, const char* prev, int32_t prev_chrom, int32_t prev_pos,
                int64_t* n_lines);
int pg_vcf_lines(pg_ctx* ctx, int64_t line0, int64_t n, pg_vcf_line* out);
int pg_vcf_genotypes(pg_ctx* ctx, int64_t n_rows, const int64_t* rows, const int64_t* pos, int64_t* n_unresolved,
                     uint64_t* error);
int pg_vcf_verdicts(pg_ctx* ctx, uint8_t* get, const uint8_t* put);
int pg_vcf_emit(pg_ctx* ctx, int64_t row0, char* out, size_t cap, int64_t* rows, size_t* bytes);

int pg_last_timings(pg_ctx* ctx, int32_t cap, char (*names)[32], float* ms, int32_t* launches, int32_t* count);
int pg_launch_count(pg_ctx* ctx, int64_t* n);
int pg_debug_k1_plan(int64_t S, int32_t H, int32_t* pitch, int32_t* lanes_per_site, int32_t* tile_sites,
                     int32_t* stages, int32_t* smem_bytes);
int pg_debug_k1_plan_ex(int64_t S, int32_t H, int32_t nw, int32_t force_G, int32_t table_bytes, int32_t* out);
int pg_debug_packed(pg_ctx* ctx, int64_t site0, int64_t n, int32_t* row_words, uint32_t* out);
int pg_debug_site_cls(pg_ctx* ctx, int64_t site0, int64_t n, int32_t* avail, uint8_t* out);
int pg_debug_uniform(pg_ctx* ctx, int32_t* in_use, int64_t* varied_sites);
int pg_debug_uniform_tile(pg_ctx* ctx, int32_t* out);
int pg_debug_uniform_ring(pg_ctx* ctx, int32_t* out);
int pg_debug_uniform_launch(pg_ctx* ctx, int32_t* out);
int pg_debug_uniform_tiles(pg_ctx* ctx, int64_t cap, int64_t* site_lo, int64_t* row0, int64_t* ntiles, int32_t* geometry);
int pg_debug_uniform_rows(pg_ctx* ctx, int64_t* one_plane_rows, int64_t* words);


int pg_seq_index(pg_ctx* ctx, const char* text, size_t len, const char* path, int64_t body_offset, int32_t n_cols,
                 const int32_t* col_slot, int32_t n_slots, const int32_t* slot_width, int32_t exact_cols, int64_t* n_sites,
                 int64_t* error);
int pg_seq_meta(pg_ctx* ctx, int32_t* pos, int8_t* new_scaffold, int64_t* line_off);
int pg_seq_plan(pg_ctx* ctx, int32_t fmt, int32_t nto_gap, int32_t n_seq, const char* names, const int64_t* name_off,
                const int32_t* seq_slot, const int32_t* seq_byte, const int32_t* seq_width, int64_t n_win, const int64_t* lo,
                const int64_t* hi, int64_t* n_rows, int64_t* win_bytes);
int pg_seq_emit(pg_ctx* ctx, int64_t row0, int64_t part0, char* out, size_t cap, int64_t* row1, int64_t* part1, size_t* bytes);


int pg_g2v_ref_load(pg_ctx* ctx, const char* text, size_t len, int64_t* n_rec);
int pg_g2v_ref_starts(pg_ctx* ctx, int64_t* starts);
int pg_g2v_ref_index(pg_ctx* ctx, int64_t n_rec, const int64_t* lo, const int64_t* hi, int64_t* rec_len);
int pg_g2v_spec(pg_ctx* ctx, int32_t fmt, int32_t n_cols, const int32_t* col_slot, const int32_t* col_prev, int32_t n_sel,
                const int32_t* sel_col, int32_t use_ref);
int pg_g2v_chunk(pg_ctx* ctx, const char* text, size_t len, int64_t* n_lines, int64_t* n_runs);
int pg_g2v_runs(pg_ctx* ctx, int64_t* run_line, int64_t* run_off);
int pg_g2v_sites(pg_ctx* ctx, const int32_t* run_rec, int64_t* n_rows, int64_t* n_bytes, int64_t* error);
int pg_g2v_emit(pg_ctx* ctx, int64_t byte0, char* out, size_t cap, size_t* bytes);


int pg_s2g_fasta_load(pg_ctx* ctx, const char* text, size_t len, int64_t* n_rec);
int pg_s2g_fasta_starts(pg_ctx* ctx, int64_t* starts);
int pg_s2g_fasta_index(pg_ctx* ctx, int64_t n_rec, const int64_t* lo, const int64_t* hi, int64_t* rec_len);
int pg_s2g_phylip_load(pg_ctx* ctx, const char* text, size_t len, int64_t* n_lines);
int pg_s2g_phylip_lines(pg_ctx* ctx, int64_t* lines);
int pg_s2g_phylip_pack(pg_ctx* ctx, int64_t n_seq, const int64_t* seq_len, int64_t n_span, const int64_t* span);
int pg_s2g_plan(pg_ctx* ctx, int64_t n_blk, const int64_t* blk, const char* names, int64_t names_len, int64_t n_mem,
                const int64_t* mem_rec, const uint8_t* mem_sep, int64_t* n_bytes);
int pg_s2g_emit(pg_ctx* ctx, int64_t byte0, char* out, size_t cap, size_t* bytes);

int pg_ws_spec(pg_ctx* ctx, int32_t n_cols, const int32_t* col_slot, int32_t n_slots, int32_t n_fields);
int pg_ws_chunk(pg_ctx* ctx, const char* text, size_t len, int64_t* n_lines, int64_t* n_runs, int64_t* n_flag, int64_t* error);
int pg_ws_chunk_info(pg_ctx* ctx, int64_t* run_line, int64_t* run_off, int64_t* flag_idx, uint64_t* flag_tok);
int pg_ws_set_values(pg_ctx* ctx, int64_t n, const int64_t* line, const int32_t* slot, const double* v);
int pg_ws_meta(pg_ctx* ctx, int64_t* n_lines, int64_t* pos);
int pg_ws_stats(pg_ctx* ctx, int64_t W, const int64_t* lo, const int64_t* hi, int32_t K, const int32_t* code, const double* q,
                int64_t sort_budget, double* out, int64_t* n_out);

#ifdef __cplusplus
}
#endif
#endif
```

Measured before the change: 69.38 billion.

## Compute diff Gram over diploid sample rows and widen finalize blocks

When both haplotypes of each sample sit in adjacent rows, the diff Gram kernel now adds the two haplotype rows of a sample before the tensor-core Gram. This produces a sample-by-sample matrix (Hm x Hm) instead of a haplotype-by-haplotype one (Hk x Hk), and the pairs epilogue reads that smaller matrix. The finalize kernel now handles four windows per block using named-barrier groups, and the slot counter shares the already-cleared partials buffer so one memset is dropped. The risk is correctness in the halved-diagonal and row-bound handling, plus more register use in the Gram loader.

```diff
diff --git a/genomics_general_b200/_lib.py b/genomics_general_b200/_lib.py
--- a/genomics_general_b200/_lib.py
+++ b/genomics_general_b200/_lib.py
@@ -94,6 +94,7 @@
     "pg_debug_uniform_launch": (C.c_int, [C.c_void_p, C.POINTER(C.c_int32)]),
     "pg_debug_uniform_tiles": (C.c_int, [C.c_void_p, C.c_int64, C.c_void_p, C.c_void_p, C.POINTER(C.c_int64),
                                          C.POINTER(C.c_int32)]),
+    "pg_debug_sample_gram": (C.c_int, [C.c_void_p, C.c_int64, C.c_int64, C.c_void_p, C.c_void_p, C.POINTER(C.c_int32)]),
     "pg_nccl_unique_id": (C.c_int, [C.c_void_p]),
     "pg_nccl_init": (C.c_int, [C.c_void_p, C.c_int32, C.c_int32, C.c_void_p]),
     "pg_nccl_finalize": (C.c_int, [C.c_void_p]),
diff --git a/genomics_general_b200/csrc/ctx.cu b/genomics_general_b200/csrc/ctx.cu
--- a/genomics_general_b200/csrc/ctx.cu
+++ b/genomics_general_b200/csrc/ctx.cu
@@ -192,6 +192,7 @@
 void pg_timings_reset(pg_ctx* ctx) {
     ctx->timings.clear();
     ctx->events_used = 0;
+    ctx->k2_diff_rows = 0;
 }
 static cudaEvent_t next_event(pg_ctx* ctx) {
     if (ctx->events_used == ctx->event_pool.size()) {
diff --git a/genomics_general_b200/csrc/k1.cu b/genomics_general_b200/csrc/k1.cu
--- a/genomics_general_b200/csrc/k1.cu
+++ b/genomics_general_b200/csrc/k1.cu
@@ -1368,12 +1368,17 @@
     return num / den;
 }
 
+constexpr int FIN_WPB = 4;
+
+__device__ __forceinline__ void fin_group_sync(int grp) { asm volatile("bar.sync %0, 64;" ::"r"(1 + grp) : "memory"); }
+
 template <int MODE>
-__global__ void __launch_bounds__(64) k1_finalize(const __grid_constant__ FinParams fp) {
-    __shared__ unsigned long long sums[64];
-    const int q = threadIdx.x;
-    for (int64_t w = blockIdx.x; w < fp.W; w += gridDim.x) {
-        __syncthreads();
+__global__ void __launch_bounds__(64 * FIN_WPB) k1_finalize(const __grid_constant__ FinParams fp) {
+    __shared__ unsigned long long sums_of[FIN_WPB][64];
+    const int grp = threadIdx.x >> 6, q = threadIdx.x & 63;
+    unsigned long long* sums = sums_of[grp];
+    for (int64_t w = (int64_t)blockIdx.x * FIN_WPB + grp; w < fp.W; w += (int64_t)gridDim.x * FIN_WPB) {
+        fin_group_sync(grp);
         if (q < fp.Q) {
             long long si = 0;
             double sd = 0.0;
@@ -1405,7 +1410,7 @@
             }
             sums[q] = (q < fp.QI) ? (unsigned long long)si : (unsigned long long)__double_as_longlong(sd);
         }
-        __syncthreads();
+        fin_group_sync(grp);
         if (q != 0) continue;
         const long long sites = fp.win_hi[w] - fp.win_lo[w];
         unsigned long long* rec = fp.rec + (size_t)w * fp.RC;
@@ -2028,13 +2033,17 @@
 }
 
 int arm_slots(pg_ctx* ctx, K1Launch& L, const void* rows) {
-    const size_t bytes = (size_t)std::max<int64_t>(L.slots.words, 1) * 8;
+    const size_t bytes = (size_t)std::max<int64_t>(L.slots.words, 1) * 8 + 16;
     PG_TRY(ctx->part.ensure(bytes));
     PG_CUDA(cudaMemsetAsync(ctx->part.p, 0, bytes, ctx->stream));
     L.prm.part = (unsigned long long*)ctx->part.p;
     L.prm.geno = (const uint8_t*)rows;
     L.prm.pos = ctx->d_pos;
     return PG_OK;
+}
+
+int* slot_counter(pg_ctx* ctx, const K1Launch& L) {
+    return (int*)((uint8_t*)ctx->part.p + (size_t)std::max<int64_t>(L.slots.words, 1) * 8);
 }
 
 template <auto Kern, int NW>
@@ -2336,7 +2345,7 @@
 template <int MODE>
 int launch_finalize(pg_ctx* ctx, const FinParams& fp) {
     const int ti = pg_time_begin(ctx, "k1_finalize");
-    k1_finalize<MODE><<<(unsigned)std::min<int64_t>(fp.W, 65535), 64, 0, ctx->stream>>>(fp);
+    k1_finalize<MODE><<<(unsigned)std::min<int64_t>((fp.W + FIN_WPB - 1) / FIN_WPB, 65535), 64 * FIN_WPB, 0, ctx->stream>>>(fp);
     pg_time_end(ctx, ti);
     PG_CUDA(cudaGetLastError());
     return PG_OK;
@@ -2532,9 +2541,8 @@
     }));
 
     PG_TRY(ctx->out_i.ensure((size_t)W * 4 + 128));
-    int* d_cnt = (int*)ctx->out_i.p;
+    int* d_cnt = slot_counter(ctx, L);
     int32_t* d_path = (int32_t*)ctx->out_i.p + 16;
-    PG_CUDA(cudaMemsetAsync(d_cnt, 0, 4, ctx->stream));
     FinParams fp;
     fill_fin(fp, ctx, c, L.slots, Q, Q);
     fp.P = P;
diff --git a/genomics_general_b200/csrc/k2.cu b/genomics_general_b200/csrc/k2.cu
--- a/genomics_general_b200/csrc/k2.cu
+++ b/genomics_general_b200/csrc/k2.cu
@@ -426,7 +426,7 @@
     long long* sh_c = reinterpret_cast<long long*>(epi_sh + (size_t)nblk * 4);
     const int wb = blockIdx.x;
     const int lane = threadIdx.x & 31, warp = threadIdx.x >> 5;
-    const int32_t* D = ep.diff + (size_t)wb * ep.Hk * ep.Hk;
+    const int32_t* D = ep.diff + (size_t)wb * ep.Hm * ep.Hm;
     const int32_t* N = ep.n + (size_t)wb * ep.Hm * ep.Hm;
     int blk = 0;
     for (int X = 0; X < P; ++X) {
@@ -461,10 +461,9 @@
                     }
                 }
                 const int nab = N[(size_t)a * ep.Hm + b];
-                const int2 u = *reinterpret_cast<const int2*>(D + (size_t)(2 * a) * ep.Hk + 2 * b);
-                const int2 v = *reinterpret_cast<const int2*>(D + (size_t)(2 * a + 1) * ep.Hk + 2 * b);
+                const int dab = D[(size_t)a * ep.Hm + b];
                 const bool ok = use && nab != 0 && !(ep.min_sites > 0 && nab < ep.min_sites);
-                const int num = (a == b) ? u.y : (u.x + u.y + v.x + v.y);
+                const int num = (a == b) ? dab / 2 : dab;
                 const double q = (double)num / (double)(ok ? nab : 1);
                 if (ok) {
                     s += q;
@@ -1085,12 +1084,13 @@
 }
 
 int run_pair_batch(pg_ctx* ctx, const PlaneSet& ps, const int64_t* d_lo, const int64_t* d_hi, int nb, int32_t** d_diff,
-                   int32_t** d_n) {
-    const size_t HH = (size_t)ps.Hk * ps.Hk, MM = (size_t)ps.Hm * ps.Hm;
+                   int32_t** d_n, bool by_sample = false) {
+    PG_CHECK(!by_sample || (ps.tensor && ps.Hm * 2 == ps.Hk), "pairwise path: no per-sample rows for the sample-row diff Gram");
+    const size_t HH = by_sample ? (size_t)ps.Hm * ps.Hm : (size_t)ps.Hk * ps.Hk, MM = (size_t)ps.Hm * ps.Hm;
     PG_TRY(ctx->pairs.ensure((size_t)nb * (HH + MM) * 4 + 64));
     *d_diff = (int32_t*)ctx->pairs.p;
     *d_n = *d_diff + (size_t)nb * HH;
-    if (ps.tensor) return pg_k2t_pairs(ctx, ps.t, d_lo, d_hi, nb, *d_diff, *d_n);
+    if (ps.tensor) return pg_k2t_pairs(ctx, ps.t, d_lo, d_hi, nb, *d_diff, *d_n, by_sample);
     PG_TRY(pg_smem_limit<k2_pair<PAIR_DIFF>>(ctx, PairGeom<PAIR_DIFF>::SMEM));
     PG_TRY(pg_smem_limit<k2_pair<PAIR_N>>(ctx, PairGeom<PAIR_N>::SMEM));
     PairParams pp;
@@ -1233,12 +1233,16 @@
     PlaneSet ps;
     PG_TRY(build_planes(ctx, order, lo, hi, ps));
     const size_t per_batch = pair_batch_size(ps.Hk, 0);
+    const int nblk = P * (P + 1) / 2;
+    bool by_pairs = ps.tensor && ps.Hm * 2 == ps.Hk && (size_t)nblk * 64 <= 48 * 1024;
+    for (int X = 0; X <= P; ++X) by_pairs = by_pairs && (pop_start[X] % 2 == 0);
+    ctx->k2_diff_rows = by_pairs ? 2 : 1;
     PG_TRY(ctx->misc.ensure((size_t)(P + 1) * 4 + per_batch * 8 + 128));
     PG_CUDA(cudaMemcpyAsync(ctx->misc.p, pop_start.data(), (size_t)(P + 1) * 4, cudaMemcpyHostToDevice, ctx->stream));
     int64_t* d_widx = reinterpret_cast<int64_t*>((uint8_t*)ctx->misc.p + (((size_t)(P + 1) * 4 + 63) / 64) * 64);
     return for_each_batch(ctx, wins, win_lo, win_hi, per_batch, [&](size_t b0, size_t nb, const int64_t* d_lo, const int64_t* d_hi) {
         int32_t *d_diff = nullptr, *d_n = nullptr;
-        PG_TRY(run_pair_batch(ctx, ps, d_lo, d_hi, (int)nb, &d_diff, &d_n));
+        PG_TRY(run_pair_batch(ctx, ps, d_lo, d_hi, (int)nb, &d_diff, &d_n, by_pairs));
         PG_CUDA(cudaMemcpyAsync(d_widx, wins.data() + b0, nb * 8, cudaMemcpyHostToDevice, ctx->stream));
         PopEpiParams ep;
         ep.diff = d_diff;
@@ -1253,12 +1257,9 @@
         ep.rec = (unsigned long long*)d_rec;
         ep.RC = RC;
         ep.win_idx = d_widx;
-        const int nblk = P * (P + 1) / 2;
         PG_TRY(ctx->misc5.ensure(nb * (size_t)nblk * 16 + 64));
         ep.blk_s = (double*)ctx->misc5.p;
         ep.blk_c = (long long*)(ep.blk_s + nb * (size_t)nblk);
-        bool by_pairs = ps.tensor && ps.Hm * 2 == ps.Hk && (size_t)nblk * 64 <= 48 * 1024;
-        for (int X = 0; X <= P; ++X) by_pairs = by_pairs && (pop_start[X] % 2 == 0);
         const unsigned nsplit = (unsigned)std::max<int64_t>(1, std::min<int64_t>(nblk, (8 * (int64_t)ctx->sm_count + (int64_t)nb - 1) / (int64_t)nb));
         PG_TRY(pg_timed(ctx, by_pairs ? "k2_popgen_epi_pairs" : "k2_popgen_epi_blocks", [&] {
             if (by_pairs) k2_popgen_epi_pairs<<<dim3((unsigned)nb, nsplit), 128, (size_t)nblk * 64, ctx->stream>>>(ep);
@@ -1438,6 +1439,47 @@
     return PG_OK;
 }
 
+extern "C" int pg_debug_sample_gram(pg_ctx* ctx, int64_t window, int64_t cap, int32_t* D, int32_t* n, int32_t* info) {
+    PG_CHECK(ctx && D && n && info, "pg_debug_sample_gram: null argument");
+    PG_CHECK(window >= 0 && window < ctx->W, "pg_debug_sample_gram: window %lld out of range", (long long)window);
+    PG_CHECK(ctx->win_hi[window] > ctx->win_lo[window], "pg_debug_sample_gram: window %lld is empty", (long long)window);
+    PG_CUDA(cudaSetDevice(ctx->device));
+    info[0] = ctx->k2_diff_rows;
+    info[1] = 0;
+    pg_timings_reset(ctx);
+    std::vector<int32_t> order, pop_start;
+    PG_TRY(group_rows(ctx, ctx->hap_pop.data(), ctx->P, nullptr, order, pop_start));
+    std::vector<int64_t> wins;
+    int64_t lo, hi;
+    nonempty_windows(ctx, wins, lo, hi);
+    PlaneSet ps;
+    PG_TRY(build_planes(ctx, order, lo, hi, ps));
+    PG_CHECK(ps.tensor, "pg_debug_sample_gram: the planes are the POPC kernels' (PG_K2_POPC or too wide)");
+    if (ps.Hm * 2 != ps.Hk) return PG_OK;
+    const int Hm = ps.Hm;
+    const size_t MM = (size_t)Hm * Hm;
+    PG_CHECK((int64_t)MM <= cap, "pg_debug_sample_gram: %lld entries do not fit cap %lld", (long long)MM, (long long)cap);
+    PG_TRY(for_each_batch(ctx, wins, ctx->win_lo.data(), ctx->win_hi.data(), pair_batch_size(ps.Hk, 0),
+                          [&](size_t b0, size_t nb, const int64_t* d_lo, const int64_t* d_hi) {
+        int32_t *d_diff = nullptr, *d_n = nullptr;
+        PG_TRY(run_pair_batch(ctx, ps, d_lo, d_hi, (int)nb, &d_diff, &d_n, true));
+        for (size_t k = 0; k < nb; ++k)
+            if (wins[b0 + k] == window) {
+                PG_CUDA(cudaMemcpyAsync(D, d_diff + k * MM, MM * 4, cudaMemcpyDeviceToHost, ctx->stream));
+                PG_CUDA(cudaMemcpyAsync(n, d_n + k * MM, MM * 4, cudaMemcpyDeviceToHost, ctx->stream));
+            }
+        PG_CUDA(cudaStreamSynchronize(ctx->stream));
+        return PG_OK;
+    }));
+    for (int a = 0; a < Hm; ++a)
+        for (int b = 0; b < a; ++b) {
+            D[(size_t)a * Hm + b] = D[(size_t)b * Hm + a];
+            n[(size_t)a * Hm + b] = n[(size_t)b * Hm + a];
+        }
+    info[1] = Hm;
+    return PG_OK;
+}
+
 extern "C" int pg_ind_het(pg_ctx* ctx, int32_t n_ind, const int32_t* hap_ind, int32_t min_sites, double* het) {
     PG_CHECK(ctx && hap_ind && het, "pg_ind_het: null argument");
     PG_CHECK(n_ind >= 1, "pg_ind_het: n_ind must be >= 1");
diff --git a/genomics_general_b200/csrc/k2t.cu b/genomics_general_b200/csrc/k2t.cu
--- a/genomics_general_b200/csrc/k2t.cu
+++ b/genomics_general_b200/csrc/k2t.cu
@@ -378,6 +378,8 @@
     r.w = (((x >> 12) & 0xfu) * 0x00204081u) & 0x01010101u;
     return r;
 }
+
+__device__ __forceinline__ uint4 add4(uint4 a, uint4 b) { return make_uint4(a.x + b.x, a.y + b.y, a.z + b.z, a.w + b.w); }
 
 __device__ __forceinline__ uint64_t gmma_desc(uint32_t saddr) {
     return (uint64_t)((saddr & 0x3ffffu) >> 4) | ((uint64_t)(128u >> 4) << 16) | ((uint64_t)(256u >> 4) << 32);
@@ -523,9 +525,11 @@
     }
 }
 
-template <int NPL, int CH>
+template <int NPL, int CH, bool SAMPLE>
 __global__ void __launch_bounds__(GRAM_THREADS, 1) k2t_gram(const __grid_constant__ GramParams gp) {
     static_assert(CH == 1 || CH == 2 || CH == 4, "chunks per stage");
+    static_assert(!SAMPLE || NPL == 2, "sample rows: the diff Gram only");
+    constexpr int HR = SAMPLE ? 2 : 1;
     constexpr int GRAM_MAX_ITEMS = ((128 + GRAM_BMAX) * NPL + GRAM_CTHREADS - 1) / GRAM_CTHREADS;
     extern __shared__ __align__(128) uint8_t gsm[];
     __shared__ __align__(8) uint64_t raw_full[GRAM_MAX_RAW], raw_empty[GRAM_MAX_RAW];
@@ -533,7 +537,7 @@
     const int NS = gp.nstages, RD = gp.nraw;
     const int AOFF = gp.a_sep ? 128 : 0;
     const int RROWS = AOFF + gp.brows;
-    const int RAW1 = NPL * RROWS * 8;
+    const int RAW1 = NPL * HR * RROWS * 8;
     const int RAW = CH * RAW1;
     const int BLK = RROWS * 32;
     const int STAGE = CH * 2 * NPL * BLK;
@@ -558,8 +562,9 @@
         for (int64_t j = j0; j < j1; ++j) {
             const GramItem im = gram_item<NPL, CH>(gp, j);
             const bool a_in_b = (im.g.a_row0 == im.g.b_row0);
-            const int a_rows = a_in_b ? 0 : min(128, gp.R - im.g.a_row0);
-            const uint32_t bytes_a = (uint32_t)a_rows * 8u, bytes_b = (uint32_t)im.g.nb_rows * 8u;
+            const int a_rows = a_in_b ? 0 : max(0, min(HR * 128, gp.R - HR * im.g.a_row0));
+            const int b_rows = SAMPLE ? max(0, min(HR * im.g.nb_rows, gp.R - HR * im.g.b_row0)) : im.g.nb_rows;
+            const uint32_t bytes_a = (uint32_t)a_rows * 8u, bytes_b = (uint32_t)b_rows * 8u;
             for (int it = 0; it < im.nst; ++it) {
                 if (n_done >= RD) mbar_wait(&raw_empty[rs], rph ^ 1u);
                 if (elect_one()) {
@@ -570,9 +575,9 @@
 #pragma unroll
                         for (int pl = 0; pl < NPL; ++pl) {
                             const uint64_t* src = gp.plane + (chunk * NPL + pl) * gp.R;
-                            uint8_t* dst = raw_base + (size_t)rs * RAW + (size_t)h * RAW1 + (size_t)pl * RROWS * 8;
-                            if (bytes_a) bulk_g2s(dst, src + im.g.a_row0, bytes_a, &raw_full[rs]);
-                            bulk_g2s(dst + AOFF * 8, src + im.g.b_row0, bytes_b, &raw_full[rs]);
+                            uint8_t* dst = raw_base + (size_t)rs * RAW + (size_t)h * RAW1 + (size_t)pl * HR * RROWS * 8;
+                            if (bytes_a) bulk_g2s(dst, src + HR * im.g.a_row0, bytes_a, &raw_full[rs]);
+                            if (!SAMPLE || bytes_b) bulk_g2s(dst + HR * AOFF * 8, src + HR * im.g.b_row0, bytes_b, &raw_full[rs]);
                         }
                     }
                 }
@@ -609,7 +614,8 @@
                 const int rr = item - pl * rows_tot + skip_a;
                 const int x = (rr < 128) ? rr : rr - 128;
                 const int row = (rr < 128) ? x : AOFF + x;
-                r_idx[q] = (rr < 128 && im.g.a_row0 + x >= gp.R) ? -2 : pl * RROWS + row;
+                const int prow = HR * (((rr < 128) ? im.g.a_row0 : im.g.b_row0) + x);
+                r_idx[q] = ((rr < 128 || SAMPLE) && prow >= gp.R) ? -2 : pl * HR * RROWS + HR * row;
                 d_off[q] = pl * BLK + (row >> 3) * 256 + (row & 7) * 16;
             }
         }
@@ -632,11 +638,14 @@
             }
             mbar_wait(&raw_full[rs], rph);
             const uint64_t* rw = reinterpret_cast<const uint64_t*>(raw_base + (size_t)rs * RAW);
-            uint64_t v[GRAM_MAX_ITEMS][CH];
+            uint64_t v[GRAM_MAX_ITEMS][CH], v2[GRAM_MAX_ITEMS][CH];
 #pragma unroll
             for (int q = 0; q < GRAM_MAX_ITEMS; ++q)
 #pragma unroll
-                for (int h = 0; h < CH; ++h) v[q][h] = (r_idx[q] >= 0) ? (rw[h * (RAW1 / 8) + r_idx[q]] & mask[h]) : 0ull;
+                for (int h = 0; h < CH; ++h) {
+                    v[q][h] = (r_idx[q] >= 0) ? (rw[h * (RAW1 / 8) + r_idx[q]] & mask[h]) : 0ull;
+                    v2[q][h] = (SAMPLE && r_idx[q] >= 0) ? (rw[h * (RAW1 / 8) + r_idx[q] + 1] & mask[h]) : 0ull;
+                }
             if (NS == 1) {
                 wgmma_wait_all();
                 consumers_sync();
@@ -650,10 +659,18 @@
                         const uint32_t wlo = (uint32_t)v[q][h], whi = (uint32_t)(v[q][h] >> 32);
                         uint8_t* d0 = sb + (size_t)h * 2 * NPL * BLK + d_off[q];
                         uint8_t* d1 = d0 + NPL * BLK;
-                        *reinterpret_cast<uint4*>(d0) = expand16(wlo & 0xffffu);
-                        *reinterpret_cast<uint4*>(d0 + 128) = expand16(wlo >> 16);
-                        *reinterpret_cast<uint4*>(d1) = expand16(whi & 0xffffu);
-                        *reinterpret_cast<uint4*>(d1 + 128) = expand16(whi >> 16);
+                        if (SAMPLE) {
+                            const uint32_t ulo = (uint32_t)v2[q][h], uhi = (uint32_t)(v2[q][h] >> 32);
+                            *reinterpret_cast<uint4*>(d0) = add4(expand16(wlo & 0xffffu), expand16(ulo & 0xffffu));
+                            *reinterpret_cast<uint4*>(d0 + 128) = add4(expand16(wlo >> 16), expand16(ulo >> 16));
+                            *reinterpret_cast<uint4*>(d1) = add4(expand16(whi & 0xffffu), expand16(uhi & 0xffffu));
+                            *reinterpret_cast<uint4*>(d1 + 128) = add4(expand16(whi >> 16), expand16(uhi >> 16));
+                        } else {
+                            *reinterpret_cast<uint4*>(d0) = expand16(wlo & 0xffffu);
+                            *reinterpret_cast<uint4*>(d0 + 128) = expand16(wlo >> 16);
+                            *reinterpret_cast<uint4*>(d1) = expand16(whi & 0xffffu);
+                            *reinterpret_cast<uint4*>(d1 + 128) = expand16(whi >> 16);
+                        }
                     }
                 }
             }
@@ -898,12 +915,14 @@
 }
 
 int pg_k2t_pairs(pg_ctx* ctx, const K2TPlanes& ps, const int64_t* d_lo, const int64_t* d_hi, int nb, int32_t* d_diff,
-                 int32_t* d_n) {
+                 int32_t* d_n, bool by_sample) {
+    PG_CHECK(!by_sample || ps.vpair, "pairwise path: the sample-row diff Gram needs per-sample co-valid rows");
     const int budget = 227 * 1024 - 1024;
-    PG_TRY((pg_smem_limit<k2t_gram<1, 1>>(ctx, budget)));
-    PG_TRY((pg_smem_limit<k2t_gram<1, 2>>(ctx, budget)));
-    PG_TRY((pg_smem_limit<k2t_gram<1, 4>>(ctx, budget)));
-    PG_TRY((pg_smem_limit<k2t_gram<2, 1>>(ctx, budget)));
+    PG_TRY((pg_smem_limit<k2t_gram<1, 1, false>>(ctx, budget)));
+    PG_TRY((pg_smem_limit<k2t_gram<1, 2, false>>(ctx, budget)));
+    PG_TRY((pg_smem_limit<k2t_gram<1, 4, false>>(ctx, budget)));
+    PG_TRY((pg_smem_limit<k2t_gram<2, 1, false>>(ctx, budget)));
+    PG_TRY((pg_smem_limit<k2t_gram<2, 1, true>>(ctx, budget)));
     const int Rn = ps.vpair ? ps.R2 : ps.R;
     std::vector<GramGroup> gn, gd;
     int brows_n, asep_n, brows_d, asep_d;
@@ -919,9 +938,9 @@
     gp.win_lo = d_lo;
     gp.win_hi = d_hi;
     gp.nb = nb;
-    auto geometry = [&](int npl, int brows, int a_sep, int ch, int& nstages, int& nraw) {
+    auto geometry = [&](int npl, int hr, int brows, int a_sep, int ch, int& nstages, int& nraw) {
         const int rrows = (a_sep ? 128 : 0) + brows;
-        const int stage = ch * 2 * npl * rrows * 32, raw = ch * npl * rrows * 8;
+        const int stage = ch * 2 * npl * rrows * 32, raw = ch * npl * hr * rrows * 8;
         nstages = 2;
         if (const char* e = getenv("PG_K2T_NSTAGES")) nstages = std::max(1, std::min(nstages, atoi(e)));
         nraw = std::min(GRAM_MAX_RAW, (budget - nstages * stage) / raw);
@@ -938,10 +957,10 @@
         gp.a_sep = asep_n;
         int ch_n = 4;
         if (const char* e = getenv("PG_K2T_CH")) ch_n = std::min(ch_n, std::max(1, atoi(e)));
-        size_t smem = geometry(1, brows_n, asep_n, ch_n, gp.nstages, gp.nraw);
+        size_t smem = geometry(1, 1, brows_n, asep_n, ch_n, gp.nstages, gp.nraw);
         while (ch_n > 1 && (smem > (size_t)budget || gp.nraw < 2)) {
             ch_n /= 2;
-            smem = geometry(1, brows_n, asep_n, ch_n, gp.nstages, gp.nraw);
+            smem = geometry(1, 1, brows_n, asep_n, ch_n, gp.nstages, gp.nraw);
         }
         PG_CHECK(smem <= (size_t)budget, "pairwise path: %d mask rows do not fit the Gram kernel's shared memory", Rn);
         gp.plane = ps.vpair ? ps.vpair : ps.vplane;
@@ -950,26 +969,29 @@
         gp.out = d_n;
         const unsigned grid = (unsigned)std::min<int64_t>((int64_t)nb * gp.ngroups, ctx->sm_count);
         PG_TRY(pg_timed(ctx, "k2t_gram_n", [&] {
-            if (ch_n == 4) k2t_gram<1, 4><<<grid, GRAM_THREADS, smem, ctx->stream>>>(gp);
-            else if (ch_n == 2) k2t_gram<1, 2><<<grid, GRAM_THREADS, smem, ctx->stream>>>(gp);
-            else k2t_gram<1, 1><<<grid, GRAM_THREADS, smem, ctx->stream>>>(gp);
+            if (ch_n == 4) k2t_gram<1, 4, false><<<grid, GRAM_THREADS, smem, ctx->stream>>>(gp);
+            else if (ch_n == 2) k2t_gram<1, 2, false><<<grid, GRAM_THREADS, smem, ctx->stream>>>(gp);
+            else k2t_gram<1, 1, false><<<grid, GRAM_THREADS, smem, ctx->stream>>>(gp);
         }));
     }
     {
         gp.R = ps.R;
-        gp.Hk = ps.Hk;
-        gp.groups = d_gd;
-        gp.ngroups = (int)gd.size();
-        gp.brows = brows_d;
-        gp.a_sep = asep_d;
-        const size_t smem = geometry(2, brows_d, asep_d, 1, gp.nstages, gp.nraw);
+        gp.Hk = by_sample ? ps.Hm : ps.Hk;
+        gp.groups = by_sample ? d_gn : d_gd;
+        gp.ngroups = (int)(by_sample ? gn.size() : gd.size());
+        gp.brows = by_sample ? brows_n : brows_d;
+        gp.a_sep = by_sample ? asep_n : asep_d;
+        const size_t smem = geometry(2, by_sample ? 2 : 1, gp.brows, gp.a_sep, 1, gp.nstages, gp.nraw);
         PG_CHECK(smem <= (size_t)budget, "pairwise path: %d haplotype rows do not fit the Gram kernel's shared memory", ps.R);
         gp.plane = ps.pq;
         gp.nchunks = (ps.npseudo + 63) / 64;
         gp.cps = ps.cps;
         gp.out = d_diff;
         const unsigned grid = (unsigned)std::min<int64_t>((int64_t)nb * gp.ngroups, ctx->sm_count);
-        PG_TRY(pg_timed(ctx, "k2t_gram_diff", [&] { k2t_gram<2, 1><<<grid, GRAM_THREADS, smem, ctx->stream>>>(gp); }));
+        PG_TRY(pg_timed(ctx, "k2t_gram_diff", [&] {
+            if (by_sample) k2t_gram<2, 1, true><<<grid, GRAM_THREADS, smem, ctx->stream>>>(gp);
+            else k2t_gram<2, 1, false><<<grid, GRAM_THREADS, smem, ctx->stream>>>(gp);
+        }));
     }
     return PG_OK;
 }
diff --git a/genomics_general_b200/csrc/pgwin_internal.h b/genomics_general_b200/csrc/pgwin_internal.h
--- a/genomics_general_b200/csrc/pgwin_internal.h
+++ b/genomics_general_b200/csrc/pgwin_internal.h
@@ -105,6 +105,7 @@
     std::vector<cudaEvent_t> event_pool;
     size_t events_used = 0;
     int64_t launches = 0;
+    int32_t k2_diff_rows = 0;
     PgBuf tables, part, segmeta, winmeta, out_d, out_i, planes, planes2, pairs, misc, misc2, misc3, misc4, misc5;
     PgBuf text, starts, meta;
     int64_t ingest_sites = -1;
@@ -195,7 +196,7 @@
 inline bool pg_k2t_fits(int pitch, int Hk) { return (size_t)16 * pitch + (size_t)((Hk + 15) / 16 * 16) * 8 <= 96 * 1024; }
 int pg_k2t_build(pg_ctx* ctx, const std::vector<int32_t>& order, int64_t lo, int64_t hi, K2TPlanes& ps);
 int pg_k2t_pairs(pg_ctx* ctx, const K2TPlanes& ps, const int64_t* d_lo, const int64_t* d_hi, int nb, int32_t* d_diff,
-                 int32_t* d_n);
+                 int32_t* d_n, bool by_sample = false);
 int pg_k2t_seq_nonnan(pg_ctx* ctx, const K2TPlanes& ps, const int64_t* d_lo, const int64_t* d_hi, int nb, long long* d_out);
 int pg_k2t_het(pg_ctx* ctx, const K2TPlanes& ps, const int64_t* d_lo, const int64_t* d_hi, int nb, const int32_t* d_ind_start,
                int n_ind, int min_sites, double* d_out);
diff --git a/genomics_general_b200/engine.py b/genomics_general_b200/engine.py
--- a/genomics_general_b200/engine.py
+++ b/genomics_general_b200/engine.py
@@ -886,6 +886,18 @@
               "pg_debug_uniform_tiles")
         return int(geo[0]), int(geo[1]), site_lo, row0
 
+    def sample_gram(self, window: int):
+        cap = max(1, (self.H // 2) ** 2)
+        D = np.empty(cap, dtype=np.int32)
+        n = np.empty(cap, dtype=np.int32)
+        info = (C.c_int32 * 2)()
+        check(self._lib.pg_debug_sample_gram(self._ctx, int(window), cap, _ptr(D), _ptr(n), info), "pg_debug_sample_gram")
+        last = {0: None, 1: "haplotypes", 2: "samples"}[int(info[0])]
+        Hm = int(info[1])
+        if Hm == 0:
+            return None, None, last
+        return D[:Hm * Hm].reshape(Hm, Hm), n[:Hm * Hm].reshape(Hm, Hm), last
+
 
 def k1_plan(S: int, H: int, nw: int = 8, lanes: int = 0, table_bytes: int = 4096):
     v = (C.c_int32 * 9)()
diff --git a/include/pgwin.h b/include/pgwin.h
--- a/include/pgwin.h
+++ b/include/pgwin.h
@@ -219,6 +219,7 @@
 int pg_debug_uniform_launch(pg_ctx* ctx, int32_t* out);
 int pg_debug_uniform_tiles(pg_ctx* ctx, int64_t cap, int64_t* site_lo, int64_t* row0, int64_t* ntiles, int32_t* geometry);
 int pg_debug_uniform_rows(pg_ctx* ctx, int64_t* one_plane_rows, int64_t* words);
+int pg_debug_sample_gram(pg_ctx* ctx, int64_t window, int64_t cap, int32_t* D, int32_t* n, int32_t* info);
 
 
 int pg_seq_index(pg_ctx* ctx, const char* text, size_t len, const char* path, int64_t body_offset, int32_t n_cols,
```

New measurement: 72.95 billion (median of 6 runs). +5.1%, better.
